# LiangZhaoPKUImperial/LinearSFM

Measured on AMD Instinct MI355X. Metric: hierarchical linear map-joining solve wall-clock, NC3500-like stereo (all transforms + joins), lower is better.
Workload: dtype f64

## Files before the change

### linearsfm_amd/csrc/lsfm_chol.hip

```cpp
#include <algorithm>
#include <climits>
#include <cmath>
#include <cstdlib>
#include <numeric>

#include "lsfm_device.hpp"
#include "lsfm_symbolic.hpp"
#include "lsfm_chol.hpp"

namespace lsfm {

#define FX_ONE 0x1p61
#define FX_INV 0x1p-61
__device__ __forceinline__ long long fx_from(double v) { return __double2ll_rn(fmin(fmax(v, -2.0), 2.0) * FX_ONE); }
__device__ __forceinline__ double fx_to(long long a) { return (double)a * FX_INV; }
__device__ __forceinline__ void fx_atomic_sub(double* slot, double t)
{
	__hip_atomic_fetch_add(reinterpret_cast<unsigned long long*>(slot), (unsigned long long)fx_from(-t), __ATOMIC_RELAXED, __HIP_MEMORY_SCOPE_AGENT);
}
__device__ __forceinline__ int scale_exp(double d)
{
	if (!(d > 0) || !(d < 1e300)) return 0;
	return (__builtin_amdgcn_frexp_exp(d) + 1) >> 1;
}
// ... 810 lines not shown
	__shared__ int spos[HB * HB];
	__shared__ int sCol[CHOL_GS];
	const int g = blockIdx.x, c0 = grp_c0[g], s = grp_s[g], nr = grp_nr[g];
	if (nr == 0 || of.skip(c0)) return;
	const int tid = threadIdx.x, nt = blockDim.x, lane = tid & 63, wave = __builtin_amdgcn_readfirstlane(tid >> 6);
	const int n6 = 6 * s, n6r = (n6 + 3) & ~3;
	const int xs = ((6 * smax + 3) & ~3) + 1;
	double* const XA = Ms;
	double* const XBs = Ms + 6 * HB * xs;
	const int nch = (nr + HB - 1) / HB, npairs = nch * (nch + 1) / 2;
	for (int t = tid; t < s; t += nt) sCol[t] = colptr[c0 + t];
	__syncthreads();
	const int rows0 = sCol[s - 1] + 1;
	for (int p = blockIdx.y; p < npairs; p += gridDim.y)
	{
		int ca = (int)((sqrtf(8.0f * p + 1.0f) - 1.0f) * 0.5f);
		while (ca * (ca + 1) / 2 > p) ca--;
		while ((ca + 1) * (ca + 2) / 2 <= p) ca++;
		const int cb = p - ca * (ca + 1) / 2;
		const bool two = ca != cb;
		if (tid < HB * HB)
		{
			const int a = tid / HB, b = tid - a * HB;
			const int ia = ca * HB + a, ib = cb * HB + b;
			int pos = -1;
			if (ia < nr && ib < nr && ia >= ib)
			{
				const int ra = rowidx[rows0 + ia], rb = rowidx[rows0 + ib];
				const int cbk = colptr[rb], nbk = colptr[rb + 1] - cbk;
				pos = cbk + (ia - ib);
				if (!(ia - ib < nbk && rowidx[pos] == ra)) pos = find_row(rowidx, cbk, cbk + nbk, ra);
			}
			spos[tid] = pos;
		}
		const int np2 = (two ? 2 : 1) * HB * s * 18;
		for (int base = 0; base < np2; base += nt * SN_LD)
		{
			double2 v[SN_LD];
#pragma unroll
			for (int i = 0; i < SN_LD; i++)
			{
				const int q = base + i * nt + tid;
				v[i] = make_double2(0.0, 0.0);
				if (q < np2)
				{
					const int blk = q / 18, il = blk / s, t = blk - il * s;
					const int row = (il < HB ? ca * HB + il : cb * HB + (il - HB));
					if (row < nr) v[i] = *reinterpret_cast<const double2*>(Lg + (size_t)(sCol[t] + (s - t) + row) * 36 + 2 * (q - blk * 18));
				}
			}
#pragma unroll
			for (int i = 0; i < SN_LD; i++)
			{
				const int q = base + i * nt + tid;
				if (q < np2)
				{
					const int blk = q / 18, w = 2 * (q - blk * 18), il = blk / s, t = blk - il * s;
					double* d = &Ms[(6 * il + w / 6) * xs + 6 * t + w % 6];
					d[0] = v[i].x; d[1] = v[i].y;
				}
			}
		}
		if (n6r > n6)
			for (int q = tid; q < (two ? 2 : 1) * 6 * HB * (n6r - n6); q += nt) Ms[(q / (n6r - n6)) * xs + n6 + q % (n6r - n6)] = 0.0;
		__syncthreads();
		const double* XB = two ? XBs : XA;
		sn_v4d acc[TPW];
#pragma unroll
		for (int i = 0; i < TPW; i++)
		{
			acc[i] = (sn_v4d){ 0.0, 0.0, 0.0, 0.0 };
			const int q = wave + (SN_THREADS / 64) * i;
			if (q < NTL * NTL)
			{
				const int ti = q / NTL, tj = q - ti * NTL;
				const double* pa = &XA[(16 * ti + (lane & 15)) * xs + (lane >> 4)];
				const double* pb = &XB[(16 * tj + (lane & 15)) * xs + (lane >> 4)];
				for (int ks = 0; ks < n6r; ks += 4) acc[i] = __builtin_amdgcn_mfma_f64_16x16x4f64(pa[ks], pb[ks], acc[i], 0, 0, 0);
			}
		}
		__syncthreads();
		double* sT = Ms;
#pragma unroll
		for (int i = 0; i < TPW; i++)
		{
			const int q = wave + (SN_THREADS / 64) * i;
			if (q < NTL * NTL)
			{
				const int ti = q / NTL, tj = q - ti * NTL;
#pragma unroll
				for (int e = 0; e < 4; e++) sT[(16 * ti + (lane >> 4) + 4 * e) * TS + 16 * tj + (lane & 15)] = acc[i][e];
			}
		}
		__syncthreads();
		for (int idx = tid; idx < HB * HB * 36; idx += nt)
		{
			const int pp = idx / 36, q = idx - pp * 36, ps = spos[pp];
			if (ps >= 0) fx_atomic_sub(L + (size_t)ps * 36 + q, sT[(6 * (pp / HB) + q / 6) * TS + 6 * (pp % HB) + q % 6]);
		}
		__syncthreads();
	}
}
static size_t sn_syrk_lds(int smax)
{
	const size_t xs = ((6 * (size_t)smax + 3) & ~(size_t)3) + 1;
	return std::max((size_t)(6 * SN_RB) * xs, (size_t)(6 * SN_RB / 2) * (6 * SN_RB / 2 + 1)) * sizeof(double);
}
static size_t sn_panel_lds(int smax)
{
	const size_t LD = 6 * (size_t)smax, xs = ((LD + 3) & ~(size_t)3) + 1;
	return std::max((LD + 6 * SN_RB + 1) * xs, (size_t)(6 * SN_RB / 2) * (6 * SN_RB / 2 + 1)) * sizeof(double);
}
__global__ void k_sn_merge(const int* __restrict__ grp_c0, const int* __restrict__ grp_s, const int* __restrict__ colptr, const double* __restrict__ Lg,
                           double* __restrict__ L)
{
	const int g = blockIdx.x, c0 = grp_c0[g], s = grp_s[g];
	const size_t b0 = (size_t)colptr[c0] * 36, b1 = (size_t)colptr[c0 + s] * 36;
	for (size_t q = b0 + threadIdx.x; q < b1; q += blockDim.x) L[q] = Lg[q];
}


template <class FT> struct SnPair;
template <> struct SnPair<double> { typedef double2 T; };
template <> struct SnPair<float> { typedef float2 T; };
template <class FT>
__device__ __forceinline__ void sn_load_diag(int s, int c0, const int* __restrict__ colptr, const FT* __restrict__ L, double* Ls, int* sSrc,
                                             int* sDst, int* sCol)
{
	const int tid = threadIdx.x, nt = blockDim.x, nb = s * (s + 1) / 2;
	for (int t = tid; t < s; t += nt) sCol[t] = colptr[c0 + t];
	__syncthreads();
	for (int e = tid; e < nb; e += nt)
	{
		int t = 0;
		while (sn_idx(s, s - 1, t) < e) t++;
		const int u = t + (e - sn_idx(s, t, t));
		sSrc[e] = (sCol[t] + (u - t)) * 36;
		sDst[e] = 6 * u * SN_XS + 6 * t;
	}
	__syncthreads();
	const int nd2 = nb * 18;
	for (int base = 0; base < nd2; base += nt * SN_LD)
	{
		typename SnPair<FT>::T v[SN_LD];
#pragma unroll
		for (int i = 0; i < SN_LD; i++)
		{
			const int q = base + i * nt + tid;
			if (q < nd2) { const int e = q / 18; v[i] = *reinterpret_cast<const typename SnPair<FT>::T*>(L + (size_t)sSrc[e] + 2 * (q - e * 18)); }
		}
#pragma unroll
		for (int i = 0; i < SN_LD; i++)
		{
			const int q = base + i * nt + tid;
			if (q < nd2) { const int e = q / 18, w = 2 * (q - e * 18); double* d = &Ls[sDst[e] + (w / 6) * SN_XS + w % 6]; d[0] = (double)v[i].x; d[1] = (double)v[i].y; }
		}
	}
	__syncthreads();
}

template <class FT>
__global__ void __launch_bounds__(SN_THREADS) k_sn_fwd(const int* __restrict__ grp_c0, const int* __restrict__ grp_s, const int* __restrict__ grp_nr,
                                                        const int* __restrict__ colptr, const int* __restrict__ rowidx, const FT* __restrict__ L,
                                                        const FT* __restrict__ Dinv, double* __restrict__ v, double* __restrict__ w, OwnFilter of)
{
	__shared__ double Ls[6 * CHOL_GS * SN_XS];
	__shared__ double sDi[CHOL_GS * 36];
	__shared__ double sA[6], sY[6 * CHOL_GS];
	__shared__ int sSrc[CHOL_GS * (CHOL_GS + 1) / 2], sDst[CHOL_GS * (CHOL_GS + 1) / 2], sCol[CHOL_GS];
	const int g = blockIdx.x, c0 = grp_c0[g], s = grp_s[g], nr = grp_nr[g];
	if (of.skip(c0)) return;
	const int tid = threadIdx.x, n6 = 6 * s;
	for (int q = tid; q < s * 36; q += SN_THREADS) sDi[q] = (double)Dinv[(size_t)c0 * 36 + q];
	double acc = tid < n6 ? v[(size_t)c0 * 6 + tid] : 0.0;
	sn_load_diag(s, c0, colptr, L, Ls, sSrc, sDst, sCol);
	for (int t = 0; t < s; t++)
	{
		const int k0 = 6 * t;
		if (tid >= k0 && tid < k0 + 6) sA[tid - k0] = acc;
		__syncthreads();
		if (tid >= k0 && tid < k0 + 6)
		{
			const int c = tid - k0;
			double y = 0.0;
			for (int k = 0; k <= c; k++) y = fma(sDi[t * 36 + c * 6 + k], sA[k], y);
			sY[tid] = y;
		}
		__syncthreads();
		if (tid >= k0 + 6 && tid < n6)
		{
			const double* lr = &Ls[tid * SN_XS + k0];
#pragma unroll
			for (int k = 0; k < 6; k++) acc = fma(-lr[k], sY[k0 + k], acc);
		}
	}
	if (tid < n6) w[(size_t)c0 * 6 + tid] = sY[tid];
	const int rows0 = colptr[c0 + s - 1] + 1;
	const int sub = tid & 3;
	for (int i = tid >> 2; i < nr; i += SN_THREADS / 4)
	{
		double o[6] = { 0, 0, 0, 0, 0, 0 };
		for (int t = sub; t < s; t += 4)
		{
			const FT* blk = L + ((size_t)sCol[t] + (s - t) + i) * 36;
			double b[36];
			ld<36>(b, blk);
#pragma unroll
			for (int r = 0; r < 6; r++)
#pragma unroll
				for (int k = 0; k < 6; k++) o[r] = fma(b[r * 6 + k], sY[6 * t + k], o[r]);
		}
#pragma unroll
		for (int r = 0; r < 6; r++)
		{
			o[r] += __shfl_xor(o[r], 1, LSFM_WAVE);
			o[r] += __shfl_xor(o[r], 2, LSFM_WAVE);
		}
		if (sub == 0)
		{
			double* dst = v + (size_t)rowidx[rows0 + i] * 6;
#pragma unroll
			for (int r = 0; r < 6; r++) atomic_add_f64(dst + r, -o[r]);
		}
	}
}

template <class FT>
__global__ void __launch_bounds__(SN_THREADS) k_sn_bwd(const int* __restrict__ grp_c0, const int* __restrict__ grp_s, const int* __restrict__ grp_nr,
                                                        const int* __restrict__ colptr, const int* __restrict__ rowidx, const FT* __restrict__ L,
                                                        const FT* __restrict__ Dinv, double* __restrict__ v, const double* __restrict__ w, OwnFilter of)
{
	__shared__ double Ls[6 * CHOL_GS * SN_XS];
	__shared__ double sDi[CHOL_GS * 36];
	__shared__ double sA[6], sZ[6 * CHOL_GS], sX[6 * CHOL_GS];
	__shared__ int sSrc[CHOL_GS * (CHOL_GS + 1) / 2], sDst[CHOL_GS * (CHOL_GS + 1) / 2], sCol[CHOL_GS];
	const int g = blockIdx.x, c0 = grp_c0[g], s = grp_s[g], nr = grp_nr[g];
	if (of.skip(c0)) return;
	const int tid = threadIdx.x, n6 = 6 * s;
	for (int q = tid; q < s * 36; q += SN_THREADS) sDi[q] = (double)Dinv[(size_t)c0 * 36 + q];
	if (tid < n6) sZ[tid] = w[(size_t)c0 * 6 + tid];
	sn_load_diag(s, c0, colptr, L, Ls, sSrc, sDst, sCol);
	const int rows0 = colptr[c0 + s - 1] + 1;
	const int sub = tid & 3;
	for (int i = tid >> 2; i < nr; i += SN_THREADS / 4)
	{
		const double* xr = v + (size_t)rowidx[rows0 + i] * 6;
		double x6[6];
		ld<6>(x6, xr);
		for (int t = sub; t < s; t += 4)
		{
			const FT* blk = L + ((size_t)sCol[t] + (s - t) + i) * 36;
			double b[36];
			ld<36>(b, blk);
#pragma unroll
			for (int c = 0; c < 6; c++)
			{
				double o = 0.0;
#pragma unroll
				for (int r = 0; r < 6; r++) o = fma(b[r * 6 + c], x6[r], o);
				lds_add_f64(&sZ[6 * t + c], -o);
			}
		}
	}
	__syncthreads();
	double acc = tid < n6 ? sZ[tid] : 0.0;
	for (int t = s - 1; t >= 0; t--)
	{
		const int k0 = 6 * t;
		if (tid >= k0 && tid < k0 + 6) sA[tid - k0] = acc;
		__syncthreads();
		if (tid >= k0 && tid < k0 + 6)
		{
			const int c = tid - k0;
			double x = 0.0;
			for (int k = c; k < 6; k++) x = fma(sDi[t * 36 + k * 6 + c], sA[k], x);
			sX[tid] = x;
		}
		__syncthreads();
		if (tid < k0)
		{
#pragma unroll
			for (int k = 0; k < 6; k++) acc = fma(-Ls[(k0 + k) * SN_XS + tid], sX[k0 + k], acc);
		}
	}
	if (tid < n6) v[(size_t)c0 * 6 + tid] = sX[tid];
}

__global__ void k_to_float(size_t n, const double* __restrict__ a, float* __restrict__ b)
{
	size_t i = (size_t)blockIdx.x * blockDim.x + threadIdx.x;
	if (i < n) b[i] = (float)a[i];
}

__global__ void k_perm_in(int M, const int* __restrict__ perm, const double* __restrict__ r, const unsigned char* __restrict__ fixed,
                          const double* __restrict__ dscale, double* __restrict__ v, int zero_from)
{
	size_t i = (size_t)blockIdx.x * blockDim.x + threadIdx.x;
	if (i >= (size_t)M * 6) return;
	const size_t src = (size_t)perm[i / 6] * 6 + i % 6;
	v[i] = ((fixed && fixed[src]) || (long)(i / 6) >= (long)zero_from) ? 0.0 : r[src] * dscale[i];
}
__global__ void k_perm_out_dot(int M, const int* __restrict__ pinv, const double* __restrict__ v, const double* __restrict__ r,
                               const unsigned char* __restrict__ fixed, const double* __restrict__ dscale, const int* __restrict__ pose_seg,
                               double* __restrict__ z, double* dot, int dot_stride, const int* __restrict__ col_owner, int rank)
{
	int row = blockIdx.x * blockDim.x + threadIdx.x;
	const bool ok = row < M;
	double acc = 0;
	int sg = 0;
	if (ok)
	{
		sg = pose_seg[row];
		const double* src = v + (size_t)pinv[row] * 6;
		const double* sc = dscale + (size_t)pinv[row] * 6;
		for (int i = 0; i < 6; i++)
		{
			double zz = src[i] * sc[i];
			if (fixed && fixed[(size_t)row * 6 + i]) zz = 0.0;
			if (col_owner) { const int ow = col_owner[pinv[row]]; if (!(ow == rank || (ow < 0 && rank == 0))) zz = 0.0; }
			z[(size_t)row * 6 + i] = zz;
			acc = fma(zz, r[(size_t)row * 6 + i], acc);
		}
	}
	if (dot) wave_scatter_add<1>(dot + (size_t)sg * dot_stride, &acc, ok);
}
__global__ void k_rz_dot(int M, const double* __restrict__ z, const double* __restrict__ r, const int* __restrict__ pose_seg, double* dot, int dot_stride)
{
	int row = blockIdx.x * blockDim.x + threadIdx.x;
	const bool ok = row < M;
	double acc = 0;
	int sg = 0;
	if (ok)
	{
		sg = pose_seg[row];
		for (int i = 0; i < 6; i++) acc = fma(z[(size_t)row * 6 + i], r[(size_t)row * 6 + i], acc);
	}
	wave_scatter_add<1>(dot + (size_t)sg * dot_stride, &acc, ok);
}

void chol_fetch(lsfm_context* ctx, const SchurSystem& sy, const int* d_origin, CholHostIn& in)
{
	const int M = sy.M, nnzb = sy.nnzb;
	in.keys.resize(nnzb);
	in.origin.resize(M);
	if (d_origin) LSFM_CHECK_HIP(hipMemcpyAsync(in.origin.data(), d_origin, (size_t)M * sizeof(int), hipMemcpyDeviceToHost, ctx->stream));
	else std::iota(in.origin.begin(), in.origin.end(), 0);
	d2h(ctx, in.keys.data(), sy.upper_keys, (size_t)nnzb * sizeof(unsigned long long));
}

void chol_alloc_values(lsfm_context* ctx, CholDev& ch)
{
	Arena& sc = ctx->scratch;
	ch.L = sc.alloc<double>((size_t)ch.nnzL * 36); ch.Dinv = sc.alloc<double>((size_t)ch.M * 36);
	ch.wv = sc.alloc<double>((size_t)ch.M * 6);
	ch.diag0 = sc.alloc<double>((size_t)ch.M * 6);
	ch.dscale = sc.alloc<double>((size_t)ch.M * 6);
	ch.Lg = ch.ngroups ? sc.alloc<double>((size_t)ch.nnzL * 36) : nullptr;
	dev_zero(ctx, ch.L, (size_t)ch.nnzL * 36 * sizeof(double));
	static const bool digest = getenv("LSFM_FACTOR_DIGEST") != nullptr;
	if (digest && ch.Lg) dev_zero(ctx, ch.Lg, (size_t)ch.nnzL * 36 * sizeof(double));
	ch.d_err = sc.alloc<int>(1);
	dev_zero(ctx, ch.d_err, sizeof(int));
}

static size_t chol_task_lds(const CholDev& ch) { return (size_t)ch.task0_maxsize * CHOL_TASK_LDS_PER_COL + 8; }
void chol_upload_index(lsfm_context* ctx, const CholSymbolic& sym, CholDev& ch)
{
	Arena& sc = ctx->scratch;
	ch.M = sym.M; ch.nnzL = sym.nnzL; ch.nlevels = sym.nlevels; ch.tail_begin = sym.tail_begin;
	ch.level_ptr = sym.level_ptr;
	if (!sym.tlevel_ptr.empty())
	{
		ch.ntask0 = sym.tlevel_ptr[1]; ch.ncol0 = sym.tlevel_col0[1];
		ch.task0_maxsize = sym.tlevel_maxsize[0]; ch.task0_lds = sym.tlevel_small_lds[0]; ch.task0_outer = sym.tlevel_outer[0];
		if (sym.tlevel_nsmall[0] != ch.ntask0 || chol_task_lds(ch) > CHOL_SOLVE_LDS)
			LSFM_FAIL(LSFM_ERR_INTERNAL, "a leaf task of the factorisation does not fit LDS (" + std::to_string(sym.tlevel_nsmall[0]) + " of " + std::to_string(ch.ntask0) +
			                                 " fit, " + std::to_string(ch.task0_maxsize) + " columns at most)");
	}
	ch.ngroups = sym.ngroups; ch.glevel_ptr = sym.glevel_ptr; ch.glevel_maxnr = sym.glevel_maxnr; ch.glevel_maxs = sym.glevel_maxs;
	ch.work_total = sym.work_total; ch.work_shared = sym.work_shared;
	ch.first_shared = sym.first_shared; ch.shared_blk0 = sym.colptr[sym.first_shared]; ch.glevel_owned = sym.glevel_owned; ch.glevel_shared = sym.glevel_shared;
	const struct { int** dst; const std::vector<int>* v; } parts[] = {
		{ &ch.grp_c0, &sym.grp_c0 }, { &ch.grp_s, &sym.grp_s }, { &ch.grp_nr, &sym.grp_nr }, { &ch.col_nin, &sym.col_nin }, { &ch.col_task, &sym.col_task },
		{ &ch.col_lpos, &sym.col_lpos }, { &ch.task_cols, &sym.task_cols }, { &ch.task_ptr, &sym.task_ptr }, { &ch.colptr, &sym.colptr },
		{ &ch.rowidx, &sym.rowidx }, { &ch.perm, &sym.perm }, { &ch.pinv, &sym.pinv }, { &ch.order, &sym.order }, { &ch.col_owner, &sym.col_owner } };
	size_t total = 0;
	for (const auto& pt : parts) total += pt.v->size();
	static thread_local std::vector<int> blob;
	blob.resize(total);
	int* d_blob = sc.alloc<int>(total);
	size_t off = 0;
	for (const auto& pt : parts)
	{
		if (!pt.v->empty()) memcpy(blob.data() + off, pt.v->data(), pt.v->size() * sizeof(int));
		*pt.dst = pt.v->empty() ? nullptr : d_blob + off;
		off += pt.v->size();
	}
	h2d(ctx, d_blob, blob.data(), total * sizeof(int));
	ch.blob = d_blob; ch.blob_ints = total;
}
void chol_upload_symbolic(lsfm_context* ctx, const CholSymbolic& sym, CholDev& ch)
{
	chol_upload_index(ctx, sym, ch);
	chol_alloc_values(ctx, ch);
	if (getenv("LSFM_DEBUG") && sym.ngroups > 50)
	{
		int hist[CHOL_GS + 1] = { 0 };
		for (int g = 0; g < sym.ngroups; g++) hist[sym.grp_s[g]]++;
		fprintf(stderr, "[lsfm] groups %d, group levels %d, sizes:", sym.ngroups, (int)sym.glevel_ptr.size() - 1);
		for (int q = 1; q <= CHOL_GS; q++) fprintf(stderr, " %d", hist[q]);
		fprintf(stderr, " | groups per level:");
		for (size_t l = 0; l + 1 < sym.glevel_ptr.size(); l++) fprintf(stderr, " %d", sym.glevel_ptr[l + 1] - sym.glevel_ptr[l]);
		fprintf(stderr, "\n");
	}
}
void chol_analyse(lsfm_context* ctx, const SchurSystem& sy, const CholHostIn& in, CholDev& ch)
{
	static thread_local CholSymbolic sym;
	chol_symbolic(in.keys.data(), sy.nnzb, in.origin.data(), sy.M, sym, ctx->comm ? ctx->comm->block_maps : 0);
	chol_upload_symbolic(ctx, sym, ch);
}

bool chol_distributed(const lsfm_context* ctx, const CholDev& ch)
{
	return ctx->comm && ctx->comm->world > 1 && ch.col_owner && ch.first_shared < ch.M;
}
static void comm_sum(lsfm_context* ctx, void* p, size_t count, int dtype)
{
	if (!count) return;
	Comm& cm = *ctx->comm;
	const size_t mk = cm.off;
	void* b = cm.alloc_bytes(count * 8);
	LSFM_CHECK_HIP(hipMemcpyAsync(b, p, count * 8, hipMemcpyDeviceToDevice, ctx->stream));
	cm.allreduce(ctx->stream, b, count, dtype);
	LSFM_CHECK_HIP(hipMemcpyAsync(p, b, count * 8, hipMemcpyDeviceToDevice, ctx->stream));
	cm.off = mk;
}
void comm_sum_host(lsfm_context* ctx, long long* h, int n)
{
	hipStream_t s = ctx->stream;
	Comm& cm = *ctx->comm;
	const size_t mk = cm.off;
	long long* d = cm.alloc<long long>(n);
	LSFM_CHECK_HIP(hipMemcpyAsync(d, h, n * sizeof(long long), hipMemcpyHostToDevice, s));
	LSFM_CHECK_HIP(hipStreamSynchronize(s));
	cm.allreduce(s, d, n, LSFM_DTYPE_I64);
	LSFM_CHECK_HIP(hipMemcpyAsync(h, d, n * sizeof(long long), hipMemcpyDeviceToHost, s));
	LSFM_CHECK_HIP(hipStreamSynchronize(s));
	cm.off = mk;
}

void chol_scatter(lsfm_context* ctx, const SchurSystem& sy, const unsigned char* fixed, CholDev& ch)
{
	const bool dist = chol_distributed(ctx, ch);
	if (sy.nnzb)
		hipLaunchKernelGGL(k_chol_scatter, dim3((sy.nnzb + 127) / 128), dim3(128), 0, ctx->stream, sy.nnzb, sy.upper_keys, sy.S, sy.rowptr, ch.pinv, ch.colptr, ch.rowidx,
		                   fixed, ch.col_task, ch.ntask0, ch.L, ch.diag0, ch.dscale, dist ? ch.col_owner : (const int*)nullptr, dist ? ctx->comm->rank : 0);
}
void chol_factor(lsfm_context* ctx, const SchurSystem& sy, const unsigned char* fixed, CholDev& ch, double* fwd_v)
{
	hipStream_t s = ctx->stream;
	const bool dist = chol_distributed(ctx, ch);
	const OwnFilter mine{ dist ? ch.col_owner : nullptr, dist ? ctx->comm->rank : 0 }, shared{ dist ? ch.col_owner : nullptr, -1 };
	ch.sn_fused_levels = ch.sn_split_levels = 0;
	if (ch.ntask0)
	{
		hipLaunchKernelGGL(k_chol_factor_level, dim3(ch.ntask0), dim3(128), (size_t)ch.task0_lds, s, ch.task_ptr, ch.task_cols, ch.col_nin, ch.colptr, ch.rowidx,
		                   ch.L, ch.Dinv, ch.d_err, mine);
		if (ch.task0_outer > 0)
		{
			const dim3 grid(ch.ncol0, std::min((ch.task0_outer + CHOL_OUT_THREADS - 1) / CHOL_OUT_THREADS, 64));
			hipLaunchKernelGGL(k_chol_update_outer, grid, dim3(CHOL_OUT_THREADS), 0, s, ch.task_cols, ch.col_nin, ch.colptr, ch.rowidx, ch.L, mine);
		}
		if (fwd_v)
			hipLaunchKernelGGL(k_chol_fwd_tasks<double>, dim3(ch.ntask0), dim3(128), chol_task_lds(ch), s, ch.task_ptr, ch.task_cols, ch.col_task, ch.col_lpos, 0, ch.colptr,
			                   ch.rowidx, (const double*)ch.L, (const double*)ch.Dinv, fwd_v, mine);
	}
	static const int fuse_max = getenv("LSFM_SN_FUSE_MAX") ? atoi(getenv("LSFM_SN_FUSE_MAX")) : 96;
	static const double piv_floor = getenv("LSFM_PIVOT_FLOOR") ? atof(getenv("LSFM_PIVOT_FLOOR")) : 1e-13;
	static const bool lds_set = []() {
		(void)hipFuncSetAttribute(reinterpret_cast<const void*>(&k_sn_panel<true>), hipFuncAttributeMaxDynamicSharedMemorySize, (int)sn_panel_lds(CHOL_GS));
		(void)hipFuncSetAttribute(reinterpret_cast<const void*>(&k_sn_panel<false>), hipFuncAttributeMaxDynamicSharedMemorySize, (int)sn_panel_lds(CHOL_GS));
		(void)hipFuncSetAttribute(reinterpret_cast<const void*>(&k_sn_syrk), hipFuncAttributeMaxDynamicSharedMemorySize, (int)sn_syrk_lds(CHOL_GS));
		return true;
	}();
	(void)lds_set;
	for (int phase = 0; phase < (dist ? 2 : 1); phase++)
	{
		const OwnFilter of = phase == 0 ? mine : shared;
		if (phase == 1)
		{
			comm_sum(ctx, ch.L + (size_t)ch.shared_blk0 * 36, ((size_t)ch.nnzL - ch.shared_blk0) * 36, LSFM_DTYPE_I64);
			if (fwd_v) comm_sum(ctx, fwd_v + (size_t)ch.first_shared * 6, ((size_t)ch.M - ch.first_shared) * 6, LSFM_DTYPE_F64);
		}
		for (size_t l = 0; l + 1 < ch.glevel_ptr.size(); l++)
		{
			const int g0 = ch.glevel_ptr[l], ng = ch.glevel_ptr[l + 1] - g0, mnr = ch.glevel_maxnr[l];
			if (!ng) continue;
			if (dist && !(phase == 0 ? ch.glevel_owned[l] : ch.glevel_shared[l])) continue;
			const int smax = l < ch.glevel_maxs.size() ? ch.glevel_maxs[l] : CHOL_GS;
			if (mnr <= fuse_max)
			{
				const int nch = (mnr + SN_RB / 2 - 1) / (SN_RB / 2);
				hipLaunchKernelGGL(k_sn_panel<true>, dim3(ng, std::max(1, nch * (nch + 1) / 2)), dim3(SN_PT), sn_panel_lds(smax), s, ch.grp_c0 + g0, ch.grp_s + g0, ch.grp_nr + g0,
				                   ch.colptr, ch.L, ch.Lg, ch.Dinv, ch.d_err, ch.rowidx, fwd_v, ch.wv, smax, ch.diag0, piv_floor, ctx->d_run ? &ctx->d_run->floored : nullptr, of);
				ch.sn_fused_levels++;
				continue;
			}
			hipLaunchKernelGGL(k_sn_panel<false>, dim3(ng, std::max(1, (mnr + SN_RB - 1) / SN_RB)), dim3(SN_PT), sn_panel_lds(smax), s, ch.grp_c0 + g0, ch.grp_s + g0, ch.grp_nr + g0,
			                   ch.colptr, ch.L, ch.Lg, ch.Dinv, ch.d_err, ch.rowidx, fwd_v, ch.wv, smax, ch.diag0, piv_floor, ctx->d_run ? &ctx->d_run->floored : nullptr, of);
			const long nch = (mnr + SN_RB / 2 - 1) / (SN_RB / 2), npair = nch * (nch + 1) / 2;
			hipLaunchKernelGGL(k_sn_syrk, dim3(ng, (unsigned)std::max<long>(1, std::min<long>(npair, 8192))), dim3(SN_THREADS), sn_syrk_lds(smax), s,
			                   ch.grp_c0 + g0, ch.grp_s + g0, ch.grp_nr + g0, ch.colptr, ch.rowidx, ch.L, ch.Lg, smax, of);
			ch.sn_split_levels++;
		}
	}
}

void chol_merge_groups(lsfm_context* ctx, const CholDev& ch)
{
	if (ch.ngroups)
		hipLaunchKernelGGL(k_sn_merge, dim3(ch.ngroups), dim3(256), 0, ctx->stream, ch.grp_c0, ch.grp_s, ch.colptr, ch.Lg, ch.L);
}
void chol_round_to_float(lsfm_context* ctx, CholDev& ch)
{
	hipStream_t s = ctx->stream;
	Arena& sc = ctx->scratch;
	const size_t nl = (size_t)ch.nnzL * 36, nd = (size_t)ch.M * 36;
	ch.Lf = sc.alloc<float>(nl); ch.Dinvf = sc.alloc<float>(nd);
	hipLaunchKernelGGL(k_to_float, dim3((unsigned)((nl + 255) / 256)), dim3(256), 0, s, nl, ch.L, ch.Lf);
	if (ch.Lg)
	{
		ch.Lgf = sc.alloc<float>(nl);
		hipLaunchKernelGGL(k_to_float, dim3((unsigned)((nl + 255) / 256)), dim3(256), 0, s, nl, ch.Lg, ch.Lgf);
	}
	hipLaunchKernelGGL(k_to_float, dim3((unsigned)((nd + 255) / 256)), dim3(256), 0, s, nd, ch.Dinv, ch.Dinvf);
}

void chol_perm_in(lsfm_context* ctx, const CholDev& ch, const double* r, const unsigned char* fixed, double* v)
{
	const size_t ns = (size_t)ch.M * 6;
	const int zero_from = (chol_distributed(ctx, ch) && ctx->comm->rank != 0) ? ch.first_shared : INT_MAX;
	hipLaunchKernelGGL(k_perm_in, dim3((unsigned)((ns + 255) / 256)), dim3(256), 0, ctx->stream, ch.M, ch.perm, r, fixed, ch.dscale, v, zero_from);
}

void chol_apply(lsfm_context* ctx, const CholDev& ch, const double* r, double* v, double* z, const unsigned char* fixed, const int* pose_seg,
                double* dot, int dot_stride, bool fwd_done)
{
	hipStream_t s = ctx->stream;
	if (!fwd_done) chol_perm_in(ctx, ch, r, fixed, v);
	const int ngl = (int)ch.glevel_ptr.size() - 1;
	const bool dist = chol_distributed(ctx, ch);
	const OwnFilter mine{ dist ? ch.col_owner : nullptr, dist ? ctx->comm->rank : 0 }, shared{ dist ? ch.col_owner : nullptr, -1 };
	auto sweep = [&](auto tag, const auto* Lx, const auto* Gx, const auto* Dx) {
		typedef decltype(tag) FT;
		if (!fwd_done)
		{
			if (ch.ntask0) hipLaunchKernelGGL(k_chol_fwd_tasks<FT>, dim3(ch.ntask0), dim3(128), chol_task_lds(ch), s, ch.task_ptr, ch.task_cols, ch.col_task, ch.col_lpos, 0, ch.colptr, ch.rowidx, Lx, Dx, v, mine);
			for (int phase = 0; phase < (dist ? 2 : 1); phase++)
			{
				if (phase == 1) comm_sum(ctx, v + (size_t)ch.first_shared * 6, ((size_t)ch.M - ch.first_shared) * 6, LSFM_DTYPE_F64);
				for (int l = 0; l < ngl; l++)
				{
					const int g0 = ch.glevel_ptr[l], ng = ch.glevel_ptr[l + 1] - g0;
					if (!ng || (dist && !(phase == 0 ? ch.glevel_owned[l] : ch.glevel_shared[l]))) continue;
					hipLaunchKernelGGL(k_sn_fwd<FT>, dim3(ng), dim3(SN_THREADS), 0, s, ch.grp_c0 + g0, ch.grp_s + g0, ch.grp_nr + g0, ch.colptr, ch.rowidx, Gx, Dx, v, ch.wv, phase == 0 ? mine : shared);
				}
			}
		}
		for (int phase = (dist ? 1 : 0); phase >= 0; phase--)
			for (int l = ngl - 1; l >= 0; l--)
			{
				const int g0 = ch.glevel_ptr[l], ng = ch.glevel_ptr[l + 1] - g0;
				if (!ng || (dist && !(phase == 0 ? ch.glevel_owned[l] : ch.glevel_shared[l]))) continue;
				hipLaunchKernelGGL(k_sn_bwd<FT>, dim3(ng), dim3(SN_THREADS), 0, s, ch.grp_c0 + g0, ch.grp_s + g0, ch.grp_nr + g0, ch.colptr, ch.rowidx, Gx, Dx, v, ch.wv, (dist && phase == 1) ? shared : mine);
			}
		if (ch.ntask0) hipLaunchKernelGGL(k_chol_bwd_tasks<FT>, dim3(ch.ntask0), dim3(128), chol_task_lds(ch), s, ch.task_ptr, ch.task_cols, ch.col_task, ch.col_lpos, 0, ch.colptr, ch.rowidx, Lx, Dx, v, mine);
	};
	if (ch.Lf) sweep(float(), (const float*)ch.Lf, (const float*)ch.Lgf, (const float*)ch.Dinvf);
	else sweep(double(), (const double*)ch.L, (const double*)ch.Lg, (const double*)ch.Dinv);
	if (dist)
	{
		hipLaunchKernelGGL(k_perm_out_dot, dim3((ch.M + 127) / 128), dim3(128), 0, s, ch.M, ch.pinv, v, r, fixed, ch.dscale, pose_seg, z, (double*)nullptr, dot_stride,
		                   ch.col_owner, ctx->comm->rank);
		ctx->comm->allreduce(s, z, (size_t)ch.M * 6, LSFM_DTYPE_F64);
		hipLaunchKernelGGL(k_rz_dot, dim3((ch.M + 127) / 128), dim3(128), 0, s, ch.M, z, r, pose_seg, dot, dot_stride);
	}
	else
		hipLaunchKernelGGL(k_perm_out_dot, dim3((ch.M + 127) / 128), dim3(128), 0, s, ch.M, ch.pinv, v, r, fixed, ch.dscale, pose_seg, z, dot, dot_stride, (const int*)nullptr, 0);
}

int chol_selftest(lsfm_context* ctx, int m, const int* rowptr, const int* colidx, const double* val, const int* origin, const unsigned char* fixed,
                  const int* pose_seg, int nseg, const double* r, int nrhs, int mode, double* z, double* dot, int* perm, int* colptr, int* rowidx,
                  double* L, double* Dinv, double* dscale, int cap_blocks, int* info)
{
	const int nnzb = rowptr[m];
	const size_t ns = (size_t)m * 6;
	CholHostIn hin;
	hin.keys.resize(nnzb);
	hin.origin.resize(m);
	for (int p = 0; p < m; p++)
	{
		hin.origin[p] = origin ? origin[p] : p;
		for (int k = rowptr[p]; k < rowptr[p + 1]; k++) hin.keys[k] = ((unsigned long long)(unsigned)p << 32) | (unsigned)colidx[k];
	}
	{
		CholSymbolic sym;
		chol_symbolic(hin.keys.data(), nnzb, hin.origin.data(), m, sym);
		info[0] = sym.nnzL;
		if (cap_blocks < sym.nnzL) LSFM_FAIL(LSFM_ERR_ARG, "rowidx / L too small for the factor (" + std::to_string(sym.nnzL) + " blocks)");
		ctx->ensure_arenas((size_t)sym.nnzL * 36 * 32 + (size_t)nnzb * 320 + ns * 8 * (16 + 2 * (size_t)nrhs) + ((size_t)64 << 20));
	}
	ctx->scratch.reset();
	Arena& sc = ctx->scratch;
	SchurSystem sy;
	sy.M = m; sy.nnzb = nnzb;
	unsigned long long* dk = sc.alloc<unsigned long long>(nnzb + 1);
	sy.S = sc.alloc<double>((size_t)nnzb * 36);
	sy.rowptr = sc.alloc<int>(m + 1);
	h2d(ctx, dk, hin.keys.data(), (size_t)nnzb * sizeof(unsigned long long));
	h2d(ctx, sy.S, val, (size_t)nnzb * 36 * sizeof(double));
	h2d(ctx, sy.rowptr, rowptr, (size_t)(m + 1) * sizeof(int));
	sy.upper_keys = dk;
	unsigned char* dfx = nullptr;
	if (fixed) { dfx = sc.alloc<unsigned char>(ns); h2d(ctx, dfx, fixed, ns); }
	int* dseg = sc.alloc<int>(m);
	h2d(ctx, dseg, pose_seg, (size_t)m * sizeof(int));
	double* dr = sc.alloc<double>(ns * nrhs);
	double* dz = sc.alloc<double>(ns * nrhs);
	double* ddot = sc.alloc<double>((size_t)nseg * nrhs);
	double* dv = sc.alloc<double>(ns);
	h2d(ctx, dr, r, ns * nrhs * sizeof(double));
	dev_zero(ctx, ddot, (size_t)nseg * nrhs * sizeof(double));
	CholDev ch;
	chol_analyse(ctx, sy, hin, ch);
	RunStatsDev* d_run = sc.alloc<RunStatsDev>(1);
	dev_zero(ctx, d_run, sizeof(RunStatsDev));
	const bool fused = (mode & 1) != 0;
	{
		struct Swap { lsfm_context* c; RunStatsDev* keep; ~Swap() { c->d_run = keep; } } swap{ ctx, ctx->d_run };
		ctx->d_run = d_run;
		chol_scatter(ctx, sy, dfx, ch);
		if (fused) chol_perm_in(ctx, ch, dr, dfx, dv);
		chol_factor(ctx, sy, dfx, ch, fused ? dv : nullptr);
	}
	if (mode & 2) chol_round_to_float(ctx, ch);
	for (int k = 0; k < nrhs; k++) chol_apply(ctx, ch, dr + ns * k, dv, dz + ns * k, dfx, dseg, ddot + (size_t)nseg * k, 1, fused && k == 0);
	chol_merge_groups(ctx, ch);
	LSFM_CHECK_HIP(hipGetLastError());
	RunStatsDev rs;
	d2h(ctx, &rs, d_run, sizeof rs);
	const int chol_err = d2h_int(ctx, ch.d_err);
	const int ngl = (int)ch.glevel_ptr.size() - 1;
	info[1] = ch.ntask0; info[2] = ch.ncol0; info[3] = ch.task0_outer; info[4] = ch.ngroups; info[5] = std::max(ngl, 0);
	info[6] = ch.sn_fused_levels; info[7] = ch.sn_split_levels;
	info[8] = ch.glevel_maxnr.empty() ? 0 : *std::max_element(ch.glevel_maxnr.begin(), ch.glevel_maxnr.end());
	info[9] = chol_err; info[10] = rs.floored;
	d2h(ctx, z, dz, ns * nrhs * sizeof(double));
	d2h(ctx, dot, ddot, (size_t)nseg * nrhs * sizeof(double));
	if (perm) d2h(ctx, perm, ch.perm, (size_t)m * sizeof(int));
	if (colptr) d2h(ctx, colptr, ch.colptr, (size_t)(m + 1) * sizeof(int));
	if (rowidx) d2h(ctx, rowidx, ch.rowidx, (size_t)ch.nnzL * sizeof(int));
	if (L) d2h(ctx, L, ch.L, (size_t)ch.nnzL * 36 * sizeof(double));
	if (Dinv) d2h(ctx, Dinv, ch.Dinv, (size_t)m * 36 * sizeof(double));
	if (dscale) d2h(ctx, dscale, ch.dscale, ns * sizeof(double));
	if (chol_err) LSFM_FAIL(LSFM_ERR_NOT_SPD, "the matrix is not positive definite (block column " + std::to_string(chol_err - 1) + " of the factor)");
	return LSFM_OK;
}

}
```

### linearsfm_amd/csrc/lsfm_chol.hpp

```cpp
#pragma once
#include <vector>

#include "lsfm_internal.hpp"
#include "lsfm_solve.hpp"

namespace lsfm {

struct CholDev {
	int M = 0, nnzL = 0, nlevels = 0, tail_begin = 0;
	int* colptr = nullptr;
	int* rowidx = nullptr;
	int* perm = nullptr;
	int* pinv = nullptr;
	int* order = nullptr;
	std::vector<int> level_ptr;
	int* task_cols = nullptr;
	int* task_ptr = nullptr;
	int* col_task = nullptr;
	int* col_lpos = nullptr;
	int* col_nin = nullptr;
	int ntask0 = 0, ncol0 = 0;
	int task0_maxsize = 0;
	int task0_lds = 0;
	int task0_outer = 0;
	int ngroups = 0;
	int *grp_c0 = nullptr, *grp_s = nullptr, *grp_nr = nullptr;
	std::vector<int> glevel_ptr;
	std::vector<int> glevel_maxnr;
	std::vector<int> glevel_maxs;
	int sn_fused_levels = 0, sn_split_levels = 0;
	int* col_owner = nullptr;
	int first_shared = 0, shared_blk0 = 0;
	double work_total = 0, work_shared = 0;
	std::vector<char> glevel_owned, glevel_shared;
	int* blob = nullptr;
	size_t blob_ints = 0;
	float *Lf = nullptr, *Dinvf = nullptr;
	double* wv = nullptr;
	double* Lg = nullptr;
	float* Lgf = nullptr;
	double* L = nullptr;
	double* Dinv = nullptr;
	double* diag0 = nullptr;
	double* dscale = nullptr;
	int* d_err = nullptr;
};

struct OwnFilter {
	const int* col_owner = nullptr;
	int want = 0;
	__device__ __forceinline__ bool skip(int col) const { return col_owner && col_owner[col] != want; }
};
__device__ __forceinline__ int find_row(const int* __restrict__ rowidx, int lo, int hi, int target)
{
	while (lo < hi) { int mid = (lo + hi) >> 1; if (rowidx[mid] < target) lo = mid + 1; else hi = mid; }
	return lo;
}


struct CholSymbolic;
struct CholHostIn {
	std::vector<unsigned long long> keys;
	std::vector<int> origin;
};

void chol_fetch(lsfm_context* ctx, const SchurSystem& sy, const int* d_origin, CholHostIn& in);
void chol_analyse(lsfm_context* ctx, const SchurSystem& sy, const CholHostIn& in, CholDev& ch);
void chol_upload_index(lsfm_context* ctx, const CholSymbolic& sym, CholDev& ch);
void chol_upload_symbolic(lsfm_context* ctx, const CholSymbolic& sym, CholDev& ch);
void chol_alloc_values(lsfm_context* ctx, CholDev& ch);
void chol_scatter(lsfm_context* ctx, const SchurSystem& sy, const unsigned char* fixed, CholDev& ch);
void chol_factor(lsfm_context* ctx, const SchurSystem& sy, const unsigned char* fixed, CholDev& ch, double* fwd_v = nullptr);
void chol_merge_groups(lsfm_context* ctx, const CholDev& ch);
void chol_round_to_float(lsfm_context* ctx, CholDev& ch);
void chol_perm_in(lsfm_context* ctx, const CholDev& ch, const double* r, const unsigned char* fixed, double* v);
void chol_apply(lsfm_context* ctx, const CholDev& ch, const double* r, double* v, double* z, const unsigned char* fixed, const int* pose_seg, double* dot, int dot_stride, bool fwd_done = false);
bool chol_distributed(const lsfm_context* ctx, const CholDev& ch);
void comm_sum_host(lsfm_context* ctx, long long* h, int n);

}
```

### linearsfm_amd/csrc/lsfm_internal.hpp

```cpp
#pragma once
#include <hip/hip_runtime.h>

#include <cstdint>
#include <cstdio>
#include <condition_variable>
#include <cstring>
#include <exception>
#include <functional>
#include <memory>
#include <mutex>
#include <thread>
#include <string>
#include <vector>

#include "../../include/lsfm.h"

namespace lsfm {

struct Error { int code; std::string msg; };
struct DevBatch;
struct IndexHold;
struct SolvePlan;
struct PreLevel;
struct EarlyPattern;

#define LSFM_CHECK_HIP(expr)                                                                                   \
	do {                                                                                                        \
		hipError_t e__ = (expr);                                                                                \
		if (e__ != hipSuccess)                                                                                  \
			throw ::lsfm::Error{ LSFM_ERR_HIP, std::string(#expr) + ": " + hipGetErrorString(e__) + " at " + __FILE__ + ":" + std::to_string(__LINE__) }; \
	} while (0)
#define LSFM_FAIL(code, m) throw ::lsfm::Error{ (code), std::string(m) + " at " + __FILE__ + ":" + std::to_string(__LINE__) }

struct Arena {
	char* base = nullptr;
	size_t cap = 0, off = 0, high = 0;
	void init(size_t bytes);
	void destroy();
	void* alloc_bytes(size_t bytes);
	template <class T> T* alloc(size_t n) { return static_cast<T*>(alloc_bytes(n * sizeof(T))); }
	void reset() { off = 0; }
	size_t mark() const { return off; }
	void release(size_t m) { off = m; }
};

struct ZeroSpan {
	Arena& ar;
	size_t from;
	explicit ZeroSpan(Arena& a) : ar(a), from((a.off + 255) & ~size_t(255)) {}
	void zero(hipStream_t s) const;
};

struct DevBatch {
	int B = 0, M = 0, NF = 0, NU = 0, NW = 0;
	std::vector<int> pose_off, feat_off, u_off, w_off;
	std::vector<int> Ref, FRef, ScaP, Fix, Sign, FScaP, FFix;
	int *d_pose_off = nullptr, *d_feat_off = nullptr;
	double* pose = nullptr;
	int* pose_id = nullptr;
	int* pose_map = nullptr;
	int* pose_origin = nullptr;
	double* feat = nullptr;
	int* feat_id = nullptr;
	int* feat_map = nullptr;
	double* U = nullptr; int *Ui = nullptr, *Uj = nullptr;
	double* W = nullptr; int *photo = nullptr, *feature = nullptr;
	int* fptr = nullptr;
	double* V = nullptr;
	const double* W_alias = nullptr;
	const int* d_alias = nullptr;
	const unsigned long long* s_keys = nullptr;
	int s_nnzb = 0;
};

struct PcgOptions { double rel_tol = 1e-12; int max_steps = 50; bool mixed = false; int spmv_variant = 0; };

struct LevelIndex {
	int NU = -1, NW = -1, NF = -1;
	const int *KU = nullptr, *KW = nullptr;
	const int *match = nullptr, *R = nullptr;
	std::shared_ptr<IndexHold> own;
};
const int* level_index_keep(lsfm_context* ctx, LevelIndex& li, const int* src, size_t n);

struct LevelPlan {
	bool valid = false;
	LevelIndex idx;
	std::vector<int> tr_cnt;
	std::vector<int> tr_sign;
	std::vector<int> join_rb;
	std::vector<int> join_uo, join_wo;
	std::shared_ptr<SolvePlan> solve;
};

struct RunStatsDev {
	int chol_err;
	int not_converged;
	int tr_err;
	int plan_stale;
	int undone;
	int floored;
	double max_rel_residual;
	unsigned long long s_digest, factor_digest;
	int refactor_mismatch;
	int s_rebuild_mismatch;
	unsigned long long k2;
};

struct Comm {
	int rank = 0, world = 1;
	lsfm_allreduce_fn fn = nullptr;
	void* user = nullptr;
	char* buf = nullptr;
	size_t cap = 0, off = 256;
	int block_maps = 0;
	enum { HDR_BYTES = 256, KIND_DATA = 0, KIND_FINAL = 1 };
	bool broken = false;
	void restart() { off = HDR_BYTES; }
	void* alloc_bytes(size_t bytes)
	{
		const size_t a = (off + 255) & ~size_t(255);
		if (a + bytes > cap)
			throw Error{ LSFM_ERR_ARG, "the buffer handed to lsfm_tree_set_comm is too small (" + std::to_string(a + bytes) + " bytes needed, " + std::to_string(cap) + " given)" };
		off = a + bytes;
		return buf + a;
	}
	template <class T> T* alloc(size_t n) { return static_cast<T*>(alloc_bytes(n * sizeof(T))); }
	void allreduce(hipStream_t s, void* p, size_t count, int dtype, int kind = KIND_DATA);
	void call(hipStream_t s, size_t offset, size_t count, int dtype)
	{
		const int rc = fn(user, offset, count, dtype, (void*)s);
		if (rc) { broken = true; throw Error{ LSFM_ERR_INTERNAL, "the caller's all-reduce failed with code " + std::to_string(rc) }; }
	}
	bool follow(hipStream_t s);
};

struct HostWorker {
	std::thread th;
	std::mutex m;
	std::condition_variable cv;
	std::function<void()> job;
	std::exception_ptr err;
	bool busy = false, quit = false;
	~HostWorker()
	{
		{ std::lock_guard<std::mutex> l(m); quit = true; }
		cv.notify_all();
		if (th.joinable()) th.join();
	}
	void run(std::function<void()> f)
	{
		std::unique_lock<std::mutex> l(m);
		cv.wait(l, [&] { return !busy; });
		job = std::move(f); busy = true; err = nullptr;
		if (!th.joinable())
			th = std::thread([this] {
				std::unique_lock<std::mutex> lk(m);
				for (;;)
				{
					cv.wait(lk, [&] { return quit || (busy && job); });
					if (quit) return;
					std::function<void()> j = std::move(job);
					job = nullptr;
					lk.unlock();
					std::exception_ptr e;
					try { j(); } catch (...) { e = std::current_exception(); }
					lk.lock();
					err = e; busy = false;
					cv.notify_all();
				}
			});
		cv.notify_all();
	}
	void wait()
	{
		std::unique_lock<std::mutex> l(m);
		cv.wait(l, [&] { return !busy; });
		if (err) { std::exception_ptr e = err; err = nullptr; std::rethrow_exception(e); }
	}
};

}

namespace lsfm {
struct Roctx {
	int (*push)(const char*) = nullptr;
	int (*pop)() = nullptr;
	void (*mark)(const char*) = nullptr;
	Roctx();
};
Roctx& roctx();
struct Range {
	bool on;
	explicit Range(const char* name) : on(roctx().push != nullptr) { if (on) roctx().push(name); }
	~Range() { if (on) roctx().pop(); }
	Range(const Range&) = delete;
	Range& operator=(const Range&) = delete;
};
}

namespace lsfm {
enum Ord {
	evA,
	evB,
	evC_pairs,
	evC_runs,
	evY,
	evP,
	evU,
	evG,
	evT,
	evK9_fork,
	evK9_done,
	evR_fork,
	evR_done,
	ORD_COUNT
};
}

struct lsfm_context {
	int device = 0;
	hipStream_t stream = nullptr;
	lsfm::Arena arena[3];
	lsfm::Arena scratch;
	int cur = 0;
	size_t arena_bytes = 0, arena_req = 0;
	lsfm::PcgOptions pcg;
	int covcols_panel = 0;
	int small_max = 5;
	std::string last_error;
	int* h_pinned = nullptr;
	char* h_stage = nullptr;
	char* d_stage = nullptr;
	size_t stage_size = 0, stage_off = 0;
	hipEvent_t ev_half[2] = { nullptr, nullptr };
	unsigned long long generation = 0;
	hipStream_t stream2 = nullptr;
	hipEvent_t ord[lsfm::ORD_COUNT] = {};
	void quiesce_side_streams();
	std::shared_ptr<lsfm::EarlyPattern> early;
	hipStream_t stream3 = nullptr;
	lsfm::Arena sarena[2];
	std::shared_ptr<lsfm::PreLevel> pre;
	lsfm::LevelPlan pre_plan;
	int pre_plan_level = -1;
	std::unique_ptr<lsfm::HostWorker> worker;
	void drop_prepared() { pre.reset(); pre_plan = lsfm::LevelPlan(); pre_plan_level = -1; }
	double dbg_gap_ms = 0.0;
	std::vector<std::pair<const char*, double>> timeline;
	bool timeline_on = false;
	void mark(const char* what);
	bool in_tree_run = false;
	lsfm_stats* stats = nullptr;
	lsfm::LevelPlan* plan = nullptr;
	bool warm() const { return plan && plan->valid; }
	lsfm::RunStatsDev* d_run = nullptr;
	lsfm::Comm* comm = nullptr;
	std::vector<hipEvent_t> ev_pool;
	size_t ev_next = 0;
	struct Timed { hipEvent_t a, b; double* sink; };
	std::vector<Timed> timed;
	hipEvent_t pool_event();
	void defer_time(hipEvent_t a, hipEvent_t b, double* sink) { timed.push_back(Timed{ a, b, sink }); }
	void flush_times();
	void ensure_arenas(size_t bytes_each, bool start_small = false);
	bool grow_arenas();
	bool arena_small = false;
	size_t arena_bound = 0;
};

namespace lsfm {

struct OnStream {
	lsfm_context* c; hipStream_t& s; Arena* a;
	OnStream(lsfm_context* ctx, hipStream_t& other, Arena* arena = nullptr) : c(ctx), s(other), a(arena) { std::swap(c->stream, s); if (a) std::swap(c->scratch, *a); }
	~OnStream() { if (a) std::swap(c->scratch, *a); std::swap(c->stream, s); }
	OnStream(const OnStream&) = delete;
	OnStream& operator=(const OnStream&) = delete;
};
inline void wait_for(lsfm_context* ctx, hipStream_t s, Ord e) { LSFM_CHECK_HIP(hipStreamWaitEvent(s, ctx->ord[e], 0)); }
struct Fork {
	lsfm_context* c; hipStream_t main; OnStream on;
	Fork(lsfm_context* ctx, hipStream_t& side, Arena* arena = nullptr) : c(ctx), main(ctx->stream), on(ctx, side, arena) {}
	Fork(lsfm_context* ctx, hipStream_t& side, Ord start, bool record = true, Arena* arena = nullptr) : Fork(ctx, side, arena)
	{
		if (record) LSFM_CHECK_HIP(hipEventRecord(c->ord[start], main));
		wait_for(c, c->stream, start);
	}
	void done(Ord e) { LSFM_CHECK_HIP(hipEventRecord(c->ord[e], c->stream)); }
	void join(Ord e) { done(e); wait_for(c, main, e); }
};

void dev_exclusive_scan(lsfm_context* ctx, const int* in, int* out, size_t n);
void dev_sort_pairs_u64(lsfm_context* ctx, unsigned long long* keys, int* vals, size_t n, int end_bit, int begin_bit = 0);
void dev_sort_keys_u64(lsfm_context* ctx, const unsigned long long* keys, unsigned long long* sorted, size_t n, int begin_bit, int end_bit);
int d2h_int(lsfm_context* ctx, const int* dptr);
void d2h_ints(lsfm_context* ctx, const int* dptr, int* h, size_t n);
void h2d(lsfm_context* ctx, void* d, const void* h, size_t bytes);
struct HostPiece { const void* p; size_t bytes; };
void h2d_gather(lsfm_context* ctx, void* d, const std::vector<HostPiece>& pieces);
struct CopyBatch {
	lsfm_context* ctx;
	struct Item { void* dst; const void* src; size_t bytes; bool host; };
	std::vector<Item> items;
	explicit CopyBatch(lsfm_context* c) : ctx(c) {}
	void h2d(void* d, const void* h, size_t bytes) { if (bytes) items.push_back(Item{ d, h, bytes, true }); }
	void d2d(void* d, const void* s, size_t bytes) { if (bytes) items.push_back(Item{ d, s, bytes, false }); }
	void flush();
};
void d2h(lsfm_context* ctx, void* h, const void* d, size_t bytes);
void dev_zero(lsfm_context* ctx, void* d, size_t bytes);
void fill_async(hipStream_t s, void* d, int byte, size_t bytes);

void batch_upload(lsfm_context* ctx, Arena& ar, const lsfm_map* maps, int N, bool mono, DevBatch& out);
void batch_download_map(lsfm_context* ctx, const DevBatch& b, int k, bool mono, lsfm_map* out);
template <class T> inline T* host_alloc(size_t n) { return static_cast<T*>(malloc((n ? n : 1) * sizeof(T))); }
struct CopyBatch;
void batch_set_offsets(lsfm_context* ctx, Arena& ar, DevBatch& b, CopyBatch* cb = nullptr);
void batch_fill_maps(lsfm_context* ctx, DevBatch& b);
struct PackHeader {
	int magic, version, mono, m, n, nU, nW, Ref, FRef, ScaP, Fix, Sign, FScaP, FFix, pad0, pad1;
	unsigned long long total;
	unsigned long long off[12];
	unsigned long long pad[11];
};
static_assert(sizeof(PackHeader) == 256, "the header is the first 256 bytes of a pack");
#define LSFM_PACK_MAGIC 0x4d46534c
size_t pack_layout(PackHeader& h);
void batch_pack_map(lsfm_context* ctx, const DevBatch& b, int k, bool mono, void* dst, size_t cap);
void batch_slice_counts(lsfm_context* ctx, const DevBatch& b, int nslices, std::vector<int>& nf, std::vector<int>& nw);
void batch_pack_slice(lsfm_context* ctx, const DevBatch& b, bool mono, int nslices, int slice, int nf, int nw, void* dst, size_t cap);
void batch_unpack_maps(lsfm_context* ctx, Arena& ar, const void* const* packed, const PackHeader* hdr, int N, bool mono, DevBatch& out);
unsigned long long batch_structure_digest(lsfm_context* ctx, const DevBatch& b);

inline bool map_in_frame(const DevBatch& X, int b, int tref, int tscap, bool mono) { return X.Ref[b] == tref && (!mono || X.ScaP[b] == tscap); }
int level_targets(const DevBatch& X, bool mono, std::vector<int>& tref, std::vector<int>& tscap, std::vector<int>& tfix);
struct TrRedirect {
	const int* wbase = nullptr;
	const int* newf = nullptr;
	double* W = nullptr;
	int *photo = nullptr, *feature = nullptr, *srcf = nullptr;
};
using TrHook = std::function<TrRedirect(DevBatch& mid, const int* hub)>;
void transform_batch(lsfm_context* ctx, Arena& ar, const DevBatch& in, const std::vector<int>& target_ref,
                     const std::vector<int>& target_scap, const std::vector<int>& target_fix, bool mono, DevBatch& out,
                     bool alias_passthrough = false, const TrHook* hook = nullptr);

struct JoinWork;
struct SolveIO {
	int M = 0, NF = 0, NU = 0, NW = 0, nseg = 0;
	const int* d_pose_seg = nullptr;
	const int* d_feat_seg = nullptr;
	const unsigned char* d_seg_active = nullptr;
	const double* U = nullptr; const int *Ui = nullptr, *Uj = nullptr;
	const double* W = nullptr; const int *photo = nullptr, *fptr = nullptr;
	const double* V = nullptr;
	const double* ea = nullptr;
	const double* eb = nullptr;
	const double* x0 = nullptr;
	const unsigned char* d_fixed = nullptr;
	const int* d_pose_origin = nullptr;
	double* x_pose = nullptr;
	double* x_feat = nullptr;
	std::vector<int> seg_rows;
	const int *d_pose_off = nullptr, *d_feat_off = nullptr, *d_u_off = nullptr;
	const struct RhsFused* rhs = nullptr;
	const struct PatternSeed* seed = nullptr;
	bool index_arrays_at_evA = false;
	int step_hint = 0;
	bool caller_syncs = false;
};
struct SolveOutcome {
	int not_converged = 0;
	int steps_used = 0;
	const unsigned long long* keys = nullptr;
	int nnzb = 0;
	hipEvent_t end = nullptr;
};
int small_level_strips(const lsfm_context* ctx, int most_rows);
inline int most_rows(const std::vector<int>& seg_rows) { int most = 0; for (int r : seg_rows) most = r > most ? r : most; return most; }
inline int small_level_strips(const lsfm_context* ctx, const std::vector<int>& seg_rows) { return small_level_strips(ctx, most_rows(seg_rows)); }
void small_level_offsets(lsfm_context* ctx, const DevBatch& out, SolveIO& io);
void small_solve_launch(lsfm_context* ctx, const SolveIO& io, int strips, int* status, double* max_rel);
struct HostSystem;
int small_selftest(lsfm_context* ctx, int G, const int* pose_off, const int* feat_off, const int* u_off, const unsigned char* active, const HostSystem& h,
                   const unsigned char* fixed, int strips, double* x_pose, double* x_feat, int* status, double* max_rel);
SolveOutcome solve_batch(lsfm_context* ctx, const SolveIO& io);
SolveOutcome join_batch_stereo(lsfm_context* ctx, Arena& ar, const DevBatch& in, DevBatch& out, double* eP_out, double* eF_out, int step_hint = 0);
SolveOutcome join_batch_mono(lsfm_context* ctx, Arena& ar, const DevBatch& in, DevBatch& out, double* eP_out, double* eF_out, int step_hint = 0);
int gn_polish(lsfm_context* ctx, const lsfm_map* maps, int N, bool mono, lsfm_map* x, int iters, int kind, double c, double* obj, double* gnorm,
              int* halvings, double* chi2, double* weight, bool feat = false);
int map_feature_chi2(lsfm_context* ctx, const lsfm_map* maps, int N, bool mono, const lsfm_map* x, double* fchi2, double* pose_chi2);
int gn_polish_features(lsfm_context* ctx, const lsfm_map* maps, int N, bool mono, lsfm_map* x, int iters, int kind, double c, double* obj, double* gnorm,
                       int* halvings, double* fchi2, double* fweight);
int map_chi2(lsfm_context* ctx, const lsfm_map* maps, int N, bool mono, const lsfm_map* x, double* chi2, int* dof);
int gn_linearise(lsfm_context* ctx, const lsfm_map* maps, int N, bool mono, const lsfm_map* x, const double* weight, lsfm_map* out, double* obj,
                 double* b, double* times, int* counts);
int map_covariance(lsfm_context* ctx, const lsfm_map* map, bool mono, double* pose_cov, double* feat_cov, double* pair_cov, int cap_blocks, int* nnzb,
                   double* times);
int map_covariance_columns(lsfm_context* ctx, const lsfm_map* map, bool mono, const int* poses, int k, double* pose_cols, double* feat_cols, double* joint,
                           int* steps, double* last_corr, double* times);
int inverse_v(lsfm_context* ctx, double* V, int n);
int solve_features(lsfm_context* ctx, const double* W, const double* IV, const double* eb, const double* dpa, double* dpb, int m, int n, const int* mapCor,
                   const int* photo);
bool no_timing_events();
#define LSFM_REC_T(e, s) do { if (!lsfm::no_timing_events()) LSFM_CHECK_HIP(hipEventRecord(e, s)); } while (0)
unsigned timing_event_flags();
unsigned order_event_flags();
void prefetch_next_level(lsfm_context* ctx, const DevBatch& Y, const std::vector<int>& target_ref, int next_level, int step_hint,
                         const unsigned long long* level_keys, int level_nnzb);
int spmv_external(lsfm_context* ctx, int m, const int* rowptr, const int* colidx, const double* val, const double* x, double* y, int reps,
                  double* avg_ms, double* bytes);
int chol_selftest(lsfm_context* ctx, int m, const int* rowptr, const int* colidx, const double* val, const int* origin, const unsigned char* fixed,
                  const int* pose_seg, int nseg, const double* r, int nrhs, int mode, double* z, double* dot, int* perm, int* colptr, int* rowidx,
                  double* L, double* Dinv, double* dscale, int cap_blocks, int* info);

int wstream_bench(lsfm_context* ctx, long long nblocks, int mode, int reps, double* avg_ms);
int prims_selftest(lsfm_context* ctx, int cases, unsigned seed);
}
```

### linearsfm_amd/csrc/lsfm_level.hip

```cpp
#include <algorithm>
#include <chrono>
#include <cmath>
#include <cstdlib>

#include "lsfm_device.hpp"
#include "lsfm_symbolic.hpp"
#include "lsfm_pcg.hpp"

namespace lsfm {

struct SolvePlan {
	SchurSystem sy;
	CholDev ch;
	int its = 1;
	bool mixed = false;
	double rel_tol = 0;
	bool small = false;
	char* mem = nullptr;
	~SolvePlan() { if (mem) (void)hipFree(mem); }
};
static std::shared_ptr<SolvePlan> solve_plan_store(lsfm_context* ctx, const SchurSystem& sy, const CholDev& ch, int its)
{
	auto sp = std::make_shared<SolvePlan>();
	const size_t M = sy.M, nnzb = sy.nnzb, cap = (size_t)sy.mask + 1;
	if (getenv("LSFM_DEBUG") && sy.k9.ns && sy.k9_tiles > 0)
	{
		std::vector<int> h(sy.k9_tiles);
		d2h(ctx, h.data(), sy.k9.ns, sizeof(int) * h.size());
		int b16 = 0, b32 = 0, b48 = 0, b64 = 0, b96 = 0, more = 0;
		for (int v : h) { const int n = v < 0 ? -v : v; (n <= 16 ? b16 : n <= 32 ? b32 : n <= 48 ? b48 : n <= 64 ? b64 : n <= 96 ? b96 : more)++; }
		fprintf(stderr, "[lsfm] Schur tiles by poses: <=16 %d, <=32 %d, <=48 %d, <=64 %d, <=96 %d, more (or > 64 distinct: hash full) %d\n", b16, b32, b48, b64, b96, more);
	}
	struct Item { const void* src; size_t bytes; void** dst; };
	SolvePlan& P = *sp;
	P.sy = sy; P.ch = ch; P.its = its; P.mixed = ch.Lf != nullptr; P.rel_tol = ctx->pcg.rel_tol;
	P.sy.S = nullptr; P.sy.E = nullptr; P.sy.IV = nullptr;
	P.ch.L = nullptr; P.ch.Dinv = nullptr; P.ch.diag0 = nullptr; P.ch.dscale = nullptr; P.ch.Lg = nullptr; P.ch.Lgf = nullptr; P.ch.d_err = nullptr; P.ch.wv = nullptr; P.ch.Lf = nullptr; P.ch.Dinvf = nullptr;
	std::vector<Item> items = {
		{ sy.rowptr, (M + 1) * 4, (void**)&P.sy.rowptr }, { sy.colidx, (nnzb + 1) * 4, (void**)&P.sy.colidx },
		{ sy.upper_keys, nnzb * 8, (void**)&P.sy.upper_keys }, { sy.longrows, (M + 1) * 4, (void**)&P.sy.longrows },
		{ sy.d_nlong, 4, (void**)&P.sy.d_nlong }, { sy.tab, cap * 8, (void**)&P.sy.tab }, { sy.hval, cap * 4, (void**)&P.sy.hval },
		{ ch.blob, ch.blob_ints * 4, (void**)&P.ch.blob },
		{ sy.gent, sy.gent ? nnzb * 16 : 0, (void**)&P.sy.gent }, { sy.goth, sy.goth ? nnzb * 8 : 0, (void**)&P.sy.goth },
		{ sy.k9.ns, sy.k9.ns ? (size_t)sy.k9_tiles * 4 : 0, (void**)&P.sy.k9.ns }, { sy.k9.pose, sy.k9.pose ? (size_t)sy.k9_tiles * 64 * 4 : 0, (void**)&P.sy.k9.pose },
		{ sy.k9.eslot, sy.k9.eslot ? (size_t)sy.k9_NW : 0, (void**)&P.sy.k9.eslot },
		{ sy.k9.wlist, sy.k9.wlist ? (size_t)sy.k9_tiles * 3 * 4 : 0, (void**)&P.sy.k9.wlist }, { sy.k9.wcnt, sy.k9.wcnt ? (size_t)32 : (size_t)0, (void**)&P.sy.k9.wcnt },
	};
	size_t total = 0;
	for (const Item& it : items) total += (it.bytes + 255) & ~(size_t)255;
	LSFM_CHECK_HIP(hipMalloc((void**)&P.mem, total + 256));
	size_t off = 0;
	for (const Item& it : items)
	{
		if (it.bytes) LSFM_CHECK_HIP(hipMemcpyAsync(P.mem + off, it.src, it.bytes, hipMemcpyDeviceToDevice, ctx->stream));
		*it.dst = it.src ? P.mem + off : nullptr;
		off += (it.bytes + 255) & ~(size_t)255;
	}
	const ptrdiff_t shift = (char*)P.ch.blob - (char*)ch.blob;
	auto rebase = [&](int*& p) { if (p) p = (int*)((char*)p + shift); };
	rebase(P.ch.colptr); rebase(P.ch.rowidx); rebase(P.ch.perm); rebase(P.ch.pinv); rebase(P.ch.order); rebase(P.ch.task_cols);
	rebase(P.ch.task_ptr); rebase(P.ch.col_task); rebase(P.ch.col_lpos); rebase(P.ch.col_nin); rebase(P.ch.grp_c0); rebase(P.ch.grp_s);
	rebase(P.ch.grp_nr); rebase(P.ch.col_owner);
	LSFM_CHECK_HIP(hipStreamSynchronize(ctx->stream));
	return sp;
}

struct PreLevel {
	SchurSystem sy;
	CholSymbolic sym;
	CholHostIn hin;
	int M = 0;
	HostWorker* worker = nullptr;
	bool whole = false;
	int level = -1, its = 0;
	void wait()
	{
		HostWorker* w = worker;
		worker = nullptr;
		if (w) w->wait();
	}
	~PreLevel() { try { wait(); } catch (...) {} }
};
void prefetch_next_level(lsfm_context* ctx, const DevBatch& Y, const std::vector<int>& target_ref, int next_level, int step_hint,
                         const unsigned long long* level_keys, int level_nnzb)
{
	ctx->drop_prepared();
	if (!Y.M || Y.B < 2) return;
	int most_next = 0;
	for (int b = 0; b < Y.B; b += 2) most_next = std::max(most_next, Y.pose_off[std::min(b + 2, Y.B)] - Y.pose_off[b]);
	const bool next_small = small_level_strips(ctx, most_next) > 0;
	const bool whole = step_hint > 0 && !getenv("LSFM_CHECK_EARLY_PATTERN");
	if (next_small && !whole) return;
	ctx->mark("pre_start");
	auto pl = std::make_shared<PreLevel>();
	pl->M = Y.M;
	Arena& sa = ctx->sarena[next_level & 1];
	sa.reset();
	std::vector<int> counts;
	LevelIndex kept;
	bool ok = false;
	{
		Fork side(ctx, ctx->stream3, evY, false, &sa);
		if (ctx->timeline_on) { (void)hipEventSynchronize(ctx->ord[evY]); ctx->mark("pre_evY"); }
		int* d_tref = ctx->scratch.alloc<int>(Y.B);
		h2d(ctx, d_tref, target_ref.data(), sizeof(int) * (size_t)Y.B);
		ok = schur_pattern_prefetch(ctx, Y, d_tref, level_keys, level_nnzb, pl->sy, whole ? &counts : nullptr, !next_small, whole ? &kept : nullptr);
		if (ok)
		{
			if (!next_small) chol_fetch(ctx, pl->sy, Y.pose_origin, pl->hin);
			side.done(evP);
		}
	}
	ctx->mark("pre_pat");
	if (!ok) return;
	if (!next_small)
	{
		if (!ctx->worker) ctx->worker.reset(new HostWorker());
		PreLevel* raw = pl.get();
		ctx->worker->run([raw]() { chol_symbolic(raw->hin.keys.data(), raw->sy.nnzb, raw->hin.origin.data(), raw->sy.M, raw->sym); });
		pl->worker = ctx->worker.get();
		ctx->mark("pre_sym");
		pl->whole = whole; pl->level = next_level; pl->its = step_hint;
		ctx->pre = pl;
	}
	if (!whole) return;
	const int B = Y.B;
	ctx->pre_plan.tr_cnt.assign(counts.begin(), counts.begin() + 2 * (B + 1));
	ctx->pre_plan.join_rb.assign(counts.begin() + 2 * (B + 1), counts.end());
	ctx->pre_plan.solve.reset();
	ctx->pre_plan.idx = kept;
	ctx->pre_plan.valid = true;
	ctx->pre_plan_level = next_level;
	ctx->mark("pre_plan");
}
static std::shared_ptr<SolvePlan> pre_plan_complete(lsfm_context* ctx, PreLevel& pl)
{
	pl.wait();
	auto sp = std::make_shared<SolvePlan>();
	sp->sy = pl.sy;
	sp->its = pl.its; sp->mixed = ctx->pcg.mixed; sp->rel_tol = ctx->pcg.rel_tol;
	{
		Fork side(ctx, ctx->stream3, &ctx->sarena[pl.level & 1]);
		chol_upload_index(ctx, pl.sym, sp->ch);
		side.join(evP);
	}
	return sp;
}

__global__ void k_dbg_absstats(size_t n, const double* __restrict__ a, double* __restrict__ out)
{
	double s = 0.0, m = 0.0;
	for (size_t i = (size_t)blockIdx.x * blockDim.x + threadIdx.x; i < n; i += (size_t)gridDim.x * blockDim.x)
	{
		const double v = fabs(a[i]);
		s += v; if (v > m || !(v == v)) m = v == v ? v : 1e300;
	}
	atomic_add_f64(out, s);
	atomicMax(reinterpret_cast<unsigned long long*>(out + 1), (unsigned long long)__double_as_longlong(m));
}
__global__ void k_dbg_dinv(int M, const double* __restrict__ Dinv, const double* __restrict__ diag0, const int* __restrict__ colptr, int first_group_col)
{
	int j = blockIdx.x * blockDim.x + threadIdx.x;
	if (j >= M) return;
	double m = 0.0;
	for (int q = 0; q < 36; q++) m = fmax(m, fabs(Dinv[(size_t)j * 36 + q]));
	if (m > 1e3 || !(m == m))
		printf("[lsfm conv] column %d (%s, %d blocks): max |Dinv| %.3e, Dinv diag %.3e %.3e %.3e %.3e %.3e %.3e, diag0 %.3e %.3e %.3e %.3e %.3e %.3e\n", j,
		       j >= first_group_col ? "group" : "leaf", colptr[j + 1] - colptr[j], m, Dinv[(size_t)j * 36], Dinv[(size_t)j * 36 + 7], Dinv[(size_t)j * 36 + 14],
		       Dinv[(size_t)j * 36 + 21], Dinv[(size_t)j * 36 + 28], Dinv[(size_t)j * 36 + 35], diag0[j * 6], diag0[j * 6 + 1], diag0[j * 6 + 2], diag0[j * 6 + 3],
		       diag0[j * 6 + 4], diag0[j * 6 + 5]);
}
__global__ void k_digest(size_t n, const unsigned long long* __restrict__ a, unsigned long long* out)
{
	unsigned long long h = 0;
	for (size_t i = (size_t)blockIdx.x * blockDim.x + threadIdx.x; i < n; i += (size_t)gridDim.x * blockDim.x)
	{
		unsigned long long b = a[i];
		if (b == 0x8000000000000000ull) b = 0;
		b ^= b >> 31; b *= 0x9E3779B97F4A7C15ull * (2 * (unsigned long long)i + 1); b ^= b >> 29;
		h += b;
	}
	atomicAdd(out, h);
}
__global__ void k_digest_compare(const unsigned long long* d, int* mismatch)
{
	if (d[0] != d[1]) atomicAdd(mismatch, 1);
}
__global__ void k_chol_err_to_run(const int* err, RunStatsDev* run)
{
	if (*err && !run->chol_err) run->chol_err = *err;
}

struct LevelStructure {
	SchurSystem sy;
	CholDev ch;
	SolvePlan* sp = nullptr;
	double tw0 = 0, tw1 = 0;
};
static double wall_ms() { return std::chrono::duration<double, std::milli>(std::chrono::steady_clock::now().time_since_epoch()).count(); }
static LevelStructure level_structure(lsfm_context* ctx, const SolveIO& io, SolvePlan* sp, PreLevel* pre, bool pending, hipEvent_t eb)
{
	hipStream_t s = ctx->stream;
	LevelStructure ls;
	SchurSystem& sy = ls.sy;
	CholDev& ch = ls.ch;
	auto assemble = [&]() {
		build_schur_values(ctx, io, sy);
		LSFM_REC_T(eb, s); if (roctx().mark) roctx().mark("lsfm factor + refine: begin");
	};
	if (sp || pending)
	{
		sy = pending ? pre->sy : sp->sy;
		schur_vinv(ctx, io, sy);
		assemble();
		if (pending)
		{
			ctx->mark("k9_enq");
			ctx->plan->solve = pre_plan_complete(ctx, *pre);
			sp = ctx->plan->solve.get();
			ctx->mark("sym_wait");
		}
		ls.sp = sp;
		ch = sp->ch;
		chol_alloc_values(ctx, ch);
		return ls;
	}
	schur_vinv(ctx, io, sy);
	CholHostIn hin;
	bool have = false;
	if (pre && !(pre->M == io.M && !ctx->comm)) pre = nullptr;
	if (pre)
	{
		schur_pattern_early_drop(ctx);
		SchurSystem prepared = pre->sy;
		prepared.IV = sy.IV; prepared.LY = sy.LY; prepared.ymax = sy.ymax; prepared.uu = sy.uu;
		sy = prepared;
		have = true;
		wait_for(ctx, s, evP);
		if (getenv("LSFM_CHECK_EARLY_PATTERN")) schur_pattern_check(ctx, io, sy, "prefetched");
	}
	else if (ctx->early && !ctx->comm)
	{
		{
			Fork side(ctx, ctx->stream3, evC_runs, false);
			ctx->mark("sv_start");
			have = schur_pattern_early_finish(ctx, io, sy);
			ctx->mark("pat_fin");
			if (have)
			{
				if (getenv("LSFM_CHECK_EARLY_PATTERN")) schur_pattern_check(ctx, io, sy, "early");
				chol_fetch(ctx, sy, io.d_pose_origin, hin);
				ctx->mark("fetch");
				schur_pattern_early_extras(ctx, sy);
				side.join(evB);
			}
		}
	}
	else if (io.index_arrays_at_evA && !ctx->comm)
	{
		Fork side(ctx, ctx->stream2, evA, false);
		build_schur_pattern(ctx, io, sy);
		chol_fetch(ctx, sy, io.d_pose_origin, hin);
		side.join(evB);
		have = true;
	}
	if (!have)
	{
		build_schur_pattern(ctx, io, sy);
		chol_fetch(ctx, sy, io.d_pose_origin, hin);
	}
	assemble();
	ls.tw0 = wall_ms();
	ctx->mark("k9_enq");
	if (pre) { pre->wait(); chol_upload_symbolic(ctx, pre->sym, ch); }
	else chol_analyse(ctx, sy, hin, ch);
	ctx->mark("analyse");
	ls.tw1 = wall_ms();
	return ls;
}

static SolveOutcome solve_level_dense(lsfm_context* ctx, const SolveIO& io, int strips, bool warm, hipEvent_t eb, hipEvent_t ec, hipEvent_t ed)
{
	hipStream_t s = ctx->stream;
	LevelPlan* lp = ctx->plan;
	if (!warm) schur_pattern_early_drop(ctx);
	int* d_small = nullptr;
	auto enqueue = [&]() {
		d_small = ctx->scratch.alloc<int>(4);
		dev_zero(ctx, d_small, 4 * sizeof(int));
		hipEvent_t esm0 = nullptr, esm1 = nullptr;
		if (ctx->stats) { esm0 = ctx->pool_event(); esm1 = ctx->pool_event(); LSFM_REC_T(esm0, s); }
		small_solve_launch(ctx, io, strips, d_small, reinterpret_cast<double*>(d_small + 2));
		if (ctx->stats) { LSFM_REC_T(esm1, s); ctx->defer_time(esm0, esm1, &ctx->stats->t_small_ms); ctx->stats->small_levels++; }
	};
	if (!warm) enqueue();
	LSFM_REC_T(eb, s); if (warm && roctx().mark) roctx().mark("lsfm factor + refine: begin");
	if (warm) enqueue();
	LSFM_REC_T(ec, s);
	LSFM_REC_T(ed, s); if (roctx().mark) roctx().mark("lsfm solve: end");
	SolveOutcome oc;
	oc.end = ed;
	oc.steps_used = 1;
	if (ctx->stats) ctx->stats->pcg_iterations += 1;
	const bool deferred = ctx->in_tree_run && ctx->d_run && (warm || !lp || lp == &ctx->pre_plan);
	if (deferred) return oc;
	int hs[4];
	d2h_ints(ctx, d_small, hs, 4);
	if (hs[1]) LSFM_FAIL(LSFM_ERR_NOT_SPD, "Schur system is not positive definite (system " + std::to_string(hs[1] - 1) + " of the level)");
	double mr;
	memcpy(&mr, hs + 2, sizeof mr);
	if (ctx->stats) ctx->stats->max_rel_residual = std::max(ctx->stats->max_rel_residual, mr);
	if (lp && !lp->solve && hs[0] == 0)
	{
		auto small_plan = std::make_shared<SolvePlan>();
		small_plan->its = 1; small_plan->mixed = false; small_plan->rel_tol = ctx->pcg.rel_tol; small_plan->small = true;
		lp->solve = small_plan;
	}
	oc.not_converged = hs[0];
	return oc;
}

static void factor_digest_check(lsfm_context* ctx, const SolveIO& io, const SchurSystem& sy, CholDev& ch)
{
	static const bool digest = getenv("LSFM_FACTOR_DIGEST") != nullptr;
	if (!digest || !ctx->d_run) return;
	hipStream_t s = ctx->stream;
	Arena& sc = ctx->scratch;
	const int M = io.M;
	auto dg = [&](const double* a, size_t n, unsigned long long* out) {
		if (a && n) hipLaunchKernelGGL(k_digest, dim3(256), dim3(256), 0, s, n, reinterpret_cast<const unsigned long long*>(a), out);
	};
	dg(sy.S, (size_t)sy.nnzb * 36, &ctx->d_run->s_digest);
	if (!ctx->comm)
	{
		SchurSystem sy2 = sy;
		build_schur_values(ctx, io, sy2);
		unsigned long long* d = sc.alloc<unsigned long long>(2);
		dev_zero(ctx, d, 2 * sizeof(unsigned long long));
		dg(sy.S, (size_t)sy.nnzb * 36, d); dg(sy.E, (size_t)M * 6, d);
		dg(sy2.S, (size_t)sy.nnzb * 36, d + 1); dg(sy2.E, (size_t)M * 6, d + 1);
		hipLaunchKernelGGL(k_digest_compare, dim3(1), dim3(1), 0, s, d, &ctx->d_run->s_rebuild_mismatch);
	}
	auto factor_digest = [&](unsigned long long* out) {
		dg(ch.Dinv, (size_t)ch.M * 36, out);
		dg(ch.L, (size_t)ch.nnzL * 36, out);
		if (ch.Lg) dg(ch.Lg, (size_t)ch.nnzL * 36, out);
	};
	factor_digest(&ctx->d_run->factor_digest);
	if (!ctx->comm)
	{
		unsigned long long* d = sc.alloc<unsigned long long>(2);
		dev_zero(ctx, d, 2 * sizeof(unsigned long long));
		factor_digest(d);
		dev_zero(ctx, ch.L, (size_t)ch.nnzL * 36 * sizeof(double));
		if (ch.Lg) dev_zero(ctx, ch.Lg, (size_t)ch.nnzL * 36 * sizeof(double));
		chol_scatter(ctx, sy, io.d_fixed, ch);
		chol_factor(ctx, sy, io.d_fixed, ch, nullptr);
		factor_digest(d + 1);
		hipLaunchKernelGGL(k_digest_compare, dim3(1), dim3(1), 0, s, d, &ctx->d_run->refactor_mismatch);
	}
}

static void debug_conv(lsfm_context* ctx, const SolveIO& io, const SchurSystem& sy, const CholDev& ch, const PcgSeg* seg)
{
	hipStream_t s = ctx->stream;
	const int M = io.M;
	hipLaunchKernelGGL(k_pcg_debug, dim3((io.nseg + 127) / 128), dim3(128), 0, s, io.nseg, M, seg);
	if (!(M > 10000 && io.nseg == 1)) return;
	double* d = ctx->scratch.alloc<double>(12);
	dev_zero(ctx, d, 12 * sizeof(double));
	auto st = [&](const double* a, size_t n, int k) { if (a && n) hipLaunchKernelGGL(k_dbg_absstats, dim3(512), dim3(256), 0, s, n, a, d + 2 * k); };
	st(sy.S, (size_t)sy.nnzb * 36, 0); st(sy.E, (size_t)M * 6, 1); st(ch.L, (size_t)ch.nnzL * 36, 2); st(ch.Lg, (size_t)ch.nnzL * 36, 3);
	st(ch.Dinv, (size_t)ch.M * 36, 4); st(io.x_pose, (size_t)M * 6, 5);
	hipLaunchKernelGGL(k_dbg_dinv, dim3((ch.M + 255) / 256), dim3(256), 0, s, ch.M, ch.Dinv, ch.diag0, ch.colptr, 0);
	double h[12];
	d2h(ctx, h, d, sizeof h);
	fprintf(stderr, "[lsfm conv] root M=%d: |S| sum %.15e max %.6e  |E| sum %.15e  |L| sum %.12e max %.3e  |Lg| sum %.12e max %.3e  |Dinv| sum %.6e max %.3e  |x| sum %.12e max %.3e\n",
	        M, h[0], h[1], h[2], h[4], h[5], h[6], h[7], h[8], h[9], h[10], h[11]);
}

SolveOutcome solve_batch(lsfm_context* ctx, const SolveIO& io)
{
	hipStream_t s = ctx->stream;
	const int M = io.M;
	LevelPlan* lp = ctx->plan;
	const int strips = (io.d_pose_off && io.d_feat_off && io.d_u_off) ? small_level_strips(ctx, io.seg_rows) : 0;
	SolvePlan* sp = lp ? lp->solve.get() : nullptr;
	if (sp && sp->small != (strips > 0)) { lp->solve.reset(); sp = nullptr; }
	std::shared_ptr<PreLevel> pre = std::move(ctx->pre);
	const bool pending = !strips && !sp && pre && pre->whole && lp == &ctx->pre_plan;
	if (pre && !pending && (strips || sp || pre->whole || pre->M != M || ctx->comm)) pre.reset();
	const bool warm = sp != nullptr || pending;
	hipEvent_t ea = ctx->pool_event(), eb = ctx->pool_event(), ec = ctx->pool_event(), ed = ctx->pool_event();
	LSFM_REC_T(ea, s); if (roctx().mark) roctx().mark("lsfm schur: begin");
	if (strips) return solve_level_dense(ctx, io, strips, warm, eb, ec, ed);
	LevelStructure ls = level_structure(ctx, io, sp, pre.get(), pending, eb);
	pre.reset();
	const SchurSystem& sy = ls.sy;
	CholDev& ch = ls.ch;
	sp = ls.sp;
	const bool dbg = getenv("LSFM_DEBUG") != nullptr;
	PcgWork w = pcg_begin(ctx, io, sy, ch);
	if (ctx->stats && chol_distributed(ctx, ch)) { ctx->stats->dist_solves++; ctx->stats->dist_work_total += ch.work_total; ctx->stats->dist_work_shared += ch.work_shared; }
	chol_scatter(ctx, sy, io.d_fixed, ch);
	if (w.fused_fwd) chol_perm_in(ctx, ch, w.r, io.d_fixed, w.v);
	chol_factor(ctx, sy, io.d_fixed, ch, w.fused_fwd ? w.v : nullptr);
	if (ctx->pcg.mixed) chol_round_to_float(ctx, ch);
	factor_digest_check(ctx, io, sy, ch);
	if (dbg) { LSFM_CHECK_HIP(hipStreamSynchronize(s)); }
	const double tw2 = wall_ms();
	const bool deferred = warm || (ctx->in_tree_run && ctx->d_run && !lp);
	const PcgSteps steps{ warm, deferred, sp ? sp->its : 0, sp ? sp->mixed : false, sp ? sp->rel_tol : 0.0 };
	const PcgResult res = pcg_run(ctx, io, sy, ch, w, steps);
	if (dbg)
	{
		LSFM_CHECK_HIP(hipStreamSynchronize(s));
		fprintf(stderr, "[lsfm] solve M=%d nseg=%d nnzb=%d nnzL=%d etree levels=%d tail=%d leaf tasks=%d group levels=%d %s| analyse %.2f ms, factor %.2f ms, cg(%d its) %.2f ms\n", M, io.nseg,
		        sy.nnzb, ch.nnzL, ch.nlevels, ch.M - ch.tail_begin, ch.ntask0, (int)ch.glevel_ptr.size() - 1, warm ? "(plan) " : "", ls.tw1 - ls.tw0, tw2 - ls.tw1, res.its, wall_ms() - tw2);
	}
	if (ctx->comm)
	{
		Comm& cm = *ctx->comm;
		const size_t nscal = (size_t)M * 6;
		double *x = io.x_pose, *xb = cm.alloc<double>(nscal);
		if (cm.rank == 0) LSFM_CHECK_HIP(hipMemcpyAsync(xb, x, nscal * sizeof(double), hipMemcpyDeviceToDevice, s));
		else fill_async(s, xb, 0, nscal * sizeof(double));
		cm.allreduce(s, xb, nscal, LSFM_DTYPE_F64);
		LSFM_CHECK_HIP(hipMemcpyAsync(x, xb, nscal * sizeof(double), hipMemcpyDeviceToDevice, s));
	}
	pcg_final_residual(ctx, io, sy, w);
	LSFM_REC_T(ec, s); if (roctx().mark) roctx().mark("lsfm back-substitution: begin");
	launch_backsub(ctx, io, sy, io.x_pose);
	LSFM_CHECK_HIP(hipGetLastError());
	LSFM_REC_T(ed, s); if (roctx().mark) roctx().mark("lsfm solve: end");
	SolveOutcome oc;
	oc.keys = sy.upper_keys; oc.nnzb = sy.nnzb;
	oc.end = ed;
	if (ctx->stats)
	{
		lsfm_stats* st = ctx->stats;
		ctx->defer_time(ea, eb, &st->t_schur_ms);
		ctx->defer_time(eb, ec, &st->t_pcg_ms);
		ctx->defer_time(ec, ed, &st->t_backsub_ms);
		ctx->defer_time(w.es0, w.es1, &st->spmv_ms);
		st->pcg_iterations += res.its;
		st->spmv_launches += 1;
		st->spmv_bytes += spmv_bytes(sy);
		st->spmv_nnzb_upper_last = sy.nnzb; st->spmv_rows_last = M;
	}
	oc.steps_used = res.planned ? 0 : std::max(res.its, 1);
	if (deferred)
	{
		if (warm && !res.planned) { sp->its = std::max(res.its, 1); sp->mixed = ctx->pcg.mixed; sp->rel_tol = ctx->pcg.rel_tol; }
		static const bool dbg_conv = getenv("LSFM_DEBUG_CONV") != nullptr;
		if (dbg_conv) debug_conv(ctx, io, sy, ch, w.seg);
		hipLaunchKernelGGL(k_pcg_run_stats, dim3((io.nseg + 127) / 128), dim3(128), 0, s, io.nseg, w.seg, ctx->d_run);
		return oc;
	}
	double maxrel = 0;
	int notconv = pcg_read_verdict(ctx, io, w, &maxrel);
	if (ctx->stats) ctx->stats->max_rel_residual = std::max(ctx->stats->max_rel_residual, maxrel);
	if (ctx->comm)
	{
		long long hv[2] = { notconv, 0 };
		comm_sum_host(ctx, hv, 2);
		notconv = (int)((hv[0] + ctx->comm->world - 1) / ctx->comm->world);
	}
	if (lp && !lp->solve && notconv == 0) lp->solve = solve_plan_store(ctx, sy, ch, std::max(res.its, 1));
	oc.not_converged = notconv;
	return oc;
}

}
```

### linearsfm_amd/csrc/lsfm_pcg.hip

```cpp
#include <algorithm>
#include <cmath>
#include <cstdlib>

#include "lsfm_device.hpp"
#include "lsfm_pcg.hpp"

namespace lsfm {

struct PcgSeg {
	double rz[2];
	double pAp;
	double rr, ee, thresh, rr_prev;
	int done, its, row0, active;
	int slow, pad;
};
static_assert(sizeof(PcgSeg) % sizeof(double) == 0, "PcgSeg is strided in doubles by the fused dot products");
#define SEG_STRIDE ((int)(sizeof(PcgSeg) / sizeof(double)))

__global__ void k_x_init(int M, const double* __restrict__ x0, const unsigned char* __restrict__ fixed, double* __restrict__ x, double* __restrict__ y, int* __restrict__ misc)
{
	size_t i = (size_t)blockIdx.x * blockDim.x + threadIdx.x;
	if (i < 4) misc[i] = 0;
	if (i >= (size_t)M * 6) return;
	y[i] = 0.0;
	double v = x0 ? x0[i] : 0.0;
	if (fixed && fixed[i]) v = 0.0;
	x[i] = v;
}

__global__ void k_pcg_resid(int M, const double* __restrict__ E, double* __restrict__ y, const int* __restrict__ pose_seg,
                            const unsigned char* __restrict__ fixed, double* __restrict__ r, PcgSeg* seg, int with_ee)
{
	int row = blockIdx.x * blockDim.x + threadIdx.x;
	bool v = row < M;
	double a[2] = { 0, 0 };
	int sg = 0;
	if (v)
	{
		sg = pose_seg[row];
		for (int i = 0; i < 6; i++)
		{
			const size_t o = (size_t)row * 6 + i;
			double e = E[o], d = e - y[o];
			y[o] = 0.0;
			if (fixed && fixed[o]) { e = 0; d = 0; }
			if (r) r[o] = d;
			a[0] += d * d; a[1] += e * e;
		}
		if (seg[sg].done) v = false;
	}
	if (!with_ee) a[1] = 0.0;
	wave_scatter_add<2>(&seg[sg].rr, a, v);
}

__global__ void k_pcg_start(int nseg, PcgSeg* seg, const unsigned char* __restrict__ active, double rel_tol, int* ndone, const int* __restrict__ err, RunStatsDev* run)
{
	int s = blockIdx.x * blockDim.x + threadIdx.x;
	if (s == 0 && run && *err && !run->chol_err) run->chol_err = *err;
	if (s >= nseg) return;
	PcgSeg& g = seg[s];
	g.thresh = rel_tol * rel_tol * g.ee;
	g.pAp = 0; g.rz[1] = 0; g.its = 0;
	g.active = active ? active[s] : 1;
	g.done = (!g.active || !(g.rr > g.thresh)) ? 1 : 0;
	g.rr_prev = g.rr;
	seg[nseg + s].rr = g.rr; seg[nseg + s].ee = g.ee;
	g.rr = 0;
	if (g.done) atomicAdd(ndone, 1);
}
__global__ void k_copy(size_t n, const double* __restrict__ a, double* __restrict__ b)
{
	size_t i = (size_t)blockIdx.x * blockDim.x + threadIdx.x;
	if (i < n) b[i] = a[i];
}

__global__ void k_pcg_update1(int M, int cur, const int* __restrict__ pose_seg, double* __restrict__ x, const double* __restrict__ p,
                              double* __restrict__ y, const PcgSeg* __restrict__ seg)
{
	int row = blockIdx.x * blockDim.x + threadIdx.x;
	if (row >= M) return;
	const PcgSeg& g = seg[pose_seg[row]];
	for (int i = 0; i < 6; i++) y[(size_t)row * 6 + i] = 0.0;
	if (g.done) return;
	const double alpha = g.rz[cur] / g.pAp;
	for (int i = 0; i < 6; i++) { const size_t o = (size_t)row * 6 + i; x[o] += alpha * p[o]; }
}

__global__ void k_pcg_update2(int M, int cur, const double* __restrict__ z, const int* __restrict__ pose_seg, double* __restrict__ p,
                              double* __restrict__ Ap, PcgSeg* seg, int* ndone)
{
	int row = blockIdx.x * blockDim.x + threadIdx.x;
	if (row >= M) return;
	const int sg = pose_seg[row];
	PcgSeg& g = seg[sg];
	const bool done = g.done;
	const double rzn = g.rz[cur ^ 1], rzc = g.rz[cur];
	for (int i = 0; i < 6; i++) Ap[(size_t)row * 6 + i] = 0.0;
	if (!done)
	{
		const double beta = rzn / rzc;
		for (int i = 0; i < 6; i++) { const size_t o = (size_t)row * 6 + i; p[o] = z[o] + beta * p[o]; }
	}
}
__global__ void k_pcg_check(int nseg, PcgSeg* seg, int* ndone)
{
	int s = blockIdx.x * blockDim.x + threadIdx.x;
	if (s >= nseg) return;
	PcgSeg& g = seg[s];
	if (g.done) return;
	const double rr = g.rr;
	g.its++;
	seg[nseg + s].rr = rr;
	const bool slow = !(rr < 0.25 * g.rr_prev);
	g.slow = slow ? g.slow + 1 : 0;
	if (!(rr > g.thresh) || !(rr == rr) || (slow && (!(rr > 1e-16 * g.ee) || g.slow >= 10))) { g.done = (rr == rr) ? 1 : 2; atomicAdd(ndone, 1); }
	g.rr_prev = rr;
}
__global__ void k_pcg_reset(int nseg, int cur, PcgSeg* seg)
{
	int s = blockIdx.x * blockDim.x + threadIdx.x;
	if (s >= nseg) return;
	PcgSeg& g = seg[s];
	if (g.done) return;
	g.pAp = 0; g.rr = 0; g.rz[cur] = 0;
}

__global__ void k_pcg_final_zero(int nseg, PcgSeg* fin)
{
	int s = blockIdx.x * blockDim.x + threadIdx.x;
	if (s < nseg) { fin[s].rr = 0.0; fin[s].ee = 0.0; }
}
__global__ void k_pcg_run_stats(int nseg, const PcgSeg* __restrict__ seg, RunStatsDev* run)
{
	int g = blockIdx.x * blockDim.x + threadIdx.x;
	if (g >= nseg || !seg[g].active) return;
	const PcgSeg& fin = seg[nseg + g];
	const double rel = fin.ee > 0 ? sqrt(fin.rr / fin.ee) : 0.0;
	if (!(rel < 1e-8) || (seg[g].done != 1 && !(rel < 1e-9))) atomicAdd(&run->not_converged, 1);
	if (seg[g].done == 0 && !(rel < 1e-10)) atomicAdd(&run->undone, 1);
	atomicMax(reinterpret_cast<unsigned long long*>(&run->max_rel_residual), (unsigned long long)__double_as_longlong(rel == rel ? rel : 1e300));
}
__global__ void k_pcg_debug(int nseg, int M, const PcgSeg* __restrict__ seg)
{
	int g = blockIdx.x * blockDim.x + threadIdx.x;
	if (g >= nseg || !seg[g].active) return;
	const PcgSeg& fin = seg[nseg + g];
	const double rel = fin.ee > 0 ? sqrt(fin.rr / fin.ee) : 0.0;
	if (!(rel < 1e-9))
		printf("[lsfm conv] M=%d nseg=%d system %d: rel %.3e its %d done %d slow %d rr_prev/ee %.3e thresh/ee %.3e ee %.3e pAp %.3e rz %.3e %.3e\n", M, nseg, g, rel, seg[g].its,
		       seg[g].done, seg[g].slow, seg[g].rr_prev / fin.ee, seg[g].thresh / fin.ee, fin.ee, seg[g].pAp, seg[g].rz[0], seg[g].rz[1]);
}

PcgWork pcg_begin(lsfm_context* ctx, const SolveIO& io, const SchurSystem& sy, const CholDev& ch)
{
	hipStream_t s = ctx->stream;
	Arena& sc = ctx->scratch;
	const int M = io.M, nseg = io.nseg;
	PcgWork w;
	w.d_misc = sc.alloc<int>(4);
	std::vector<PcgSeg> hseg(2 * (size_t)nseg);
	memset(hseg.data(), 0, sizeof(PcgSeg) * hseg.size());
	for (int g = 0, row = 0; g < nseg; g++) { hseg[g].row0 = hseg[nseg + g].row0 = row; row += io.seg_rows[g]; }
	w.seg = sc.alloc<PcgSeg>(hseg.size());
	h2d(ctx, w.seg, hseg.data(), sizeof(PcgSeg) * hseg.size());
	const size_t nscal = (size_t)M * 6;
	w.r = sc.alloc<double>(nscal); w.z = ctx->comm ? ctx->comm->alloc<double>(nscal) : sc.alloc<double>(nscal); w.p = sc.alloc<double>(nscal);
	w.Ap = sc.alloc<double>(nscal); w.v = sc.alloc<double>(nscal);
	const unsigned nbe = (unsigned)((nscal + 255) / 256);
	hipLaunchKernelGGL(k_x_init, dim3(std::max(1u, nbe)), dim3(256), 0, s, M, io.x0, io.d_fixed, io.x_pose, w.Ap, w.d_misc);
	launch_spmv(ctx, sy, io.x_pose, w.Ap, io.d_fixed, nullptr, nullptr, nullptr, 1);
	hipLaunchKernelGGL(k_pcg_resid, dim3((M + 127) / 128), dim3(128), 0, s, M, sy.E, w.Ap, io.d_pose_seg, io.d_fixed, w.r, w.seg, 1);
	static const bool no_fused_fwd = getenv("LSFM_NO_FUSED_FWD") != nullptr;
	w.fused_fwd = !ctx->pcg.mixed && !no_fused_fwd && ch.M > 0;
	return w;
}

PcgResult pcg_run(lsfm_context* ctx, const SolveIO& io, const SchurSystem& sy, const CholDev& ch, PcgWork& w, const PcgSteps& steps)
{
	hipStream_t s = ctx->stream;
	const int M = io.M, nseg = io.nseg;
	const size_t nscal = (size_t)M * 6;
	const int nbr = (M + 127) / 128, nbs = (nseg + 127) / 128;
	const unsigned nbe = (unsigned)((nscal + 255) / 256);
	double *x = io.x_pose, *r = w.r, *z = w.z, *p = w.p, *Ap = w.Ap, *v = w.v;
	PcgSeg* seg = w.seg;
	int* d_misc = w.d_misc;
	const bool mixed = ctx->pcg.mixed;
	chol_apply(ctx, ch, r, v, z, io.d_fixed, io.d_pose_seg, &seg[0].rz[0], SEG_STRIDE, w.fused_fwd);
	hipLaunchKernelGGL(k_copy, dim3(nbe), dim3(256), 0, s, nscal, z, p);
	const bool err_to_run = steps.deferred || (ctx->comm && ctx->d_run);
	hipLaunchKernelGGL(k_pcg_start, dim3(nbs), dim3(128), 0, s, nseg, seg, io.d_seg_active, ctx->pcg.rel_tol, d_misc + 1, ch.d_err, err_to_run ? ctx->d_run : (RunStatsDev*)nullptr);

	const int maxit = std::max(1, std::min(50, ctx->pcg.max_steps));
	const bool hinted = !steps.warm && steps.deferred && io.step_hint > 0 && io.step_hint <= maxit;
	const bool planned_run = hinted || (steps.warm && steps.mixed == mixed && steps.rel_tol == ctx->pcg.rel_tol && steps.its <= maxit);
	int its = 0, ndone = 0;
	w.es0 = ctx->pool_event(); w.es1 = ctx->pool_event();
	const bool ask_after = hinted && io.caller_syncs && !ctx->comm;
	const int base_steps = hinted ? io.step_hint : (planned_run ? steps.its : maxit);
	const int planned = (planned_run && !ask_after && base_steps >= (mixed ? 3 : 2)) ? std::min(base_steps + 1, maxit) : base_steps;
	bool counting = planned_run;
	int cap = maxit;
	while ((counting ? its < planned : (ndone < nseg && its < cap)))
	{
		const int cur = its & 1;
		launch_spmv(ctx, sy, p, Ap, io.d_fixed, p, io.d_pose_seg, &seg[0].pAp, SEG_STRIDE);
		hipLaunchKernelGGL(k_pcg_update1, dim3(nbr), dim3(128), 0, s, M, cur, io.d_pose_seg, x, p, Ap, seg);
		if (!w.es_done) LSFM_REC_T(w.es0, s);
		launch_spmv(ctx, sy, x, Ap, io.d_fixed, nullptr, nullptr, nullptr, 1);
		if (!w.es_done) { LSFM_REC_T(w.es1, s); w.es_done = true; }
		hipLaunchKernelGGL(k_pcg_resid, dim3(nbr), dim3(128), 0, s, M, sy.E, Ap, io.d_pose_seg, io.d_fixed, r, seg, 0);
		hipLaunchKernelGGL(k_pcg_check, dim3(nbs), dim3(128), 0, s, nseg, seg, d_misc + 1);
		its++;
		if (counting)
		{
			if (its >= planned)
			{
				if (!ask_after) break;
				ndone = d2h_int(ctx, d_misc + 1);
				if (ndone >= nseg || its >= maxit) break;
				counting = false;
				cap = std::min(maxit, planned + 3);
			}
		}
		else
		{
			ctx->mark("cg_enq");
			ndone = d2h_int(ctx, d_misc + 1);
			ctx->mark("cg_sync");
			const int cerr = (its == 1 && !err_to_run) ? d2h_int(ctx, ch.d_err) : 0;
			if (cerr) LSFM_FAIL(LSFM_ERR_NOT_SPD, "Schur system is not positive definite (block column " + std::to_string(cerr - 1) + " of the factor)");
			if (ctx->comm && ctx->comm->world > 1)
			{
				long long more = ndone >= nseg ? 0 : 1;
				comm_sum_host(ctx, &more, 1);
				if (!more) break;
				ndone = std::min(ndone, nseg - 1);
			}
			else if (ndone >= nseg) break;
		}
		chol_apply(ctx, ch, r, v, z, io.d_fixed, io.d_pose_seg, &seg[0].rz[cur ^ 1], SEG_STRIDE);
		hipLaunchKernelGGL(k_pcg_update2, dim3(nbr), dim3(128), 0, s, M, cur, z, io.d_pose_seg, p, Ap, seg, d_misc + 1);
		hipLaunchKernelGGL(k_pcg_reset, dim3(nbs), dim3(128), 0, s, nseg, cur, seg);
	}
	return PcgResult{ its, planned_run };
}

void pcg_final_residual(lsfm_context* ctx, const SolveIO& io, const SchurSystem& sy, PcgWork& w)
{
	if (!ctx->comm && w.es_done) return;
	hipStream_t s = ctx->stream;
	const int M = io.M, nseg = io.nseg, nbr = (M + 127) / 128, nbs = (nseg + 127) / 128;
	PcgSeg* seg2 = w.seg + nseg;
	if (!w.es_done) LSFM_REC_T(w.es0, s);
	launch_spmv(ctx, sy, io.x_pose, w.Ap, io.d_fixed, nullptr, nullptr, nullptr, 1);
	if (!w.es_done) { LSFM_REC_T(w.es1, s); w.es_done = true; }
	hipLaunchKernelGGL(k_pcg_final_zero, dim3(nbs), dim3(128), 0, s, nseg, seg2);
	hipLaunchKernelGGL(k_pcg_resid, dim3(nbr), dim3(128), 0, s, M, sy.E, w.Ap, io.d_pose_seg, io.d_fixed, (double*)nullptr, seg2, 1);
}

int pcg_read_verdict(lsfm_context* ctx, const SolveIO& io, const PcgWork& w, double* maxrel)
{
	const int nseg = io.nseg;
	std::vector<PcgSeg> hs2(2 * (size_t)nseg);
	d2h(ctx, hs2.data(), w.seg, sizeof(PcgSeg) * 2 * nseg);
	int notconv = 0;
	*maxrel = 0;
	for (int g = 0; g < nseg; g++)
	{
		if (!hs2[g].active) continue;
		const PcgSeg& fin = hs2[nseg + g];
		const double rel = fin.ee > 0 ? sqrt(fin.rr / fin.ee) : 0.0;
		*maxrel = std::max(*maxrel, rel);
		if (!(rel < 1e-8) || (hs2[g].done != 1 && !(rel < 1e-9))) notconv++;
	}
	return notconv;
}

}
```

### linearsfm_amd/csrc/lsfm_pcg.hpp

```cpp
#pragma once
#include "lsfm_chol.hpp"

namespace lsfm {

struct PcgSeg;

struct PcgWork {
	double *r = nullptr, *z = nullptr, *p = nullptr, *Ap = nullptr, *v = nullptr;
	PcgSeg* seg = nullptr;
	int* d_misc = nullptr;
	bool fused_fwd = false;
	hipEvent_t es0 = nullptr, es1 = nullptr;
	bool es_done = false;
};
struct PcgSteps { bool warm, deferred; int its; bool mixed; double rel_tol; };
struct PcgResult { int its; bool planned; };

PcgWork pcg_begin(lsfm_context* ctx, const SolveIO& io, const SchurSystem& sy, const CholDev& ch);
PcgResult pcg_run(lsfm_context* ctx, const SolveIO& io, const SchurSystem& sy, const CholDev& ch, PcgWork& w, const PcgSteps& steps);
void pcg_final_residual(lsfm_context* ctx, const SolveIO& io, const SchurSystem& sy, PcgWork& w);
__global__ void k_pcg_run_stats(int nseg, const PcgSeg* __restrict__ seg, RunStatsDev* run);
__global__ void k_pcg_debug(int nseg, int M, const PcgSeg* __restrict__ seg);
int pcg_read_verdict(lsfm_context* ctx, const SolveIO& io, const PcgWork& w, double* maxrel);

}
```

### linearsfm_amd/csrc/lsfm_solve.hip

```cpp
#include <algorithm>
#include <cmath>

#include "lsfm_device.hpp"
#include "lsfm_internal.hpp"
#include "lsfm_solve.hpp"

namespace lsfm {

__global__ void __launch_bounds__(256) k_vinv(int NF, const double* __restrict__ V, const double* __restrict__ eb, double* __restrict__ IV, double* __restrict__ LY,
                                               double* __restrict__ ymax, RhsFused rhs, double* __restrict__ uu)
{
	__shared__ double wmax[4];
	int f = blockIdx.x * blockDim.x + threadIdx.x;
	double y2 = 0.0;
	if (f < NF)
	{
	double a[9], o[9];
	ld<9>(a, V + (size_t)f * 9);
	inv3_sym(a, o);
	st<9>(IV + (size_t)f * 9, o);
	const double* e = eb + (size_t)f * 3;
	double l[9];
	const double d0 = o[0];
	l[0] = sqrt(d0);
	l[1] = o[3] / l[0];
	l[3] = o[6] / l[0];
	const double d1 = o[4] - l[1] * l[1];
	l[2] = sqrt(d1);
	l[4] = (o[7] - l[3] * l[1]) / l[2];
	const double d2 = o[8] - l[3] * l[3] - l[4] * l[4];
	l[5] = sqrt(d2);
	l[6] = l[0] * e[0] + l[1] * e[1] + l[3] * e[2];
	l[7] = l[2] * e[1] + l[4] * e[2];
	l[8] = l[5] * e[2];
	if (!(d0 > 0.0) || !(d1 > 0.0) || !(d2 > 0.0)) l[0] = __builtin_nan("");
	st<9>(LY + (size_t)f * 9, l);
	y2 = l[6] * l[6] + l[7] * l[7] + l[8] * l[8];
	if (uu)
	{
#pragma unroll
		for (int sd = 0; sd < 2; sd++)
		{
			const int fs = sd ? rhs.srcC[f] : rhs.srcE[f];
			double u0 = 0.0, u1 = 0.0, u2 = 0.0;
			if (fs >= 0)
			{
				const double* x = rhs.feat_src + (size_t)fs * 3;
				u0 = x[0] / l[0];
				u1 = (x[1] - l[1] * u0) / l[2];
				u2 = (x[2] - l[3] * u0 - l[4] * u1) / l[5];
			}
			uu[(size_t)f * 6 + 3 * sd] = u0; uu[(size_t)f * 6 + 3 * sd + 1] = u1; uu[(size_t)f * 6 + 3 * sd + 2] = u2;
			y2 = fmax(y2, u0 * u0 + u1 * u1 + u2 * u2);
		}
	}
	if (!(y2 == y2)) y2 = 0.0;
	}
	if (!ymax) return;
#pragma unroll
	for (int off = 32; off > 0; off >>= 1) y2 = fmax(y2, __shfl_xor(y2, off, LSFM_WAVE));
	if ((threadIdx.x & (LSFM_WAVE - 1)) == 0) wmax[threadIdx.x >> 6] = y2;
	__syncthreads();
	if (threadIdx.x == 0) ymax[blockIdx.x] = fmax(fmax(wmax[0], wmax[1]), fmax(wmax[2], wmax[3]));
}

__device__ __forceinline__ int half_exponent(double d)
{
	if (!(d > 0.0) || !(d < 1e300)) return 0;
	int k;
	(void)frexp(d, &k);
	return ((k + 1) >> 1) + 1;
}
__global__ void __launch_bounds__(256) k_schur_scale(int M, const int* __restrict__ rowptr, const double* __restrict__ S, int NF, int nymax,
                                                      const double* __restrict__ ymax, const unsigned char* __restrict__ fixed, int* __restrict__ sexp,
                                                      const double* __restrict__ ea, double* __restrict__ E)
{
	const int i = blockIdx.x * blockDim.x + threadIdx.x;
	if (i < 6 * M)
	{
		E[i] = ea[i];
		const int p = i / 6, r = i - 6 * p;
		sexp[i] = (fixed && fixed[i]) ? 400 : half_exponent(S[(size_t)rowptr[p] * 36 + 7 * r]);
	}
	if (blockIdx.x == 0)
	{
		__shared__ double wmax[4];
		double m = 0.0;
		for (int b = threadIdx.x; b < nymax; b += 256) m = fmax(m, ymax[b]);
#pragma unroll
		for (int off = 32; off > 0; off >>= 1) m = fmax(m, __shfl_xor(m, off, LSFM_WAVE));
		if ((threadIdx.x & (LSFM_WAVE - 1)) == 0) wmax[threadIdx.x >> 6] = m;
		__syncthreads();
		if (threadIdx.x == 0) sexp[6 * (size_t)M] = half_exponent((double)NF * fmax(fmax(wmax[0], wmax[1]), fmax(wmax[2], wmax[3]))) + 20;
	}
}
__global__ void k_schur_finish(int nnzb, int M, const unsigned long long* __restrict__ keys, const long long* __restrict__ acc, const int* __restrict__ sexp,
                               double* __restrict__ S, double* __restrict__ E)
{
	const size_t i = (size_t)blockIdx.x * blockDim.x + threadIdx.x;
	const size_t ns = (size_t)nnzb * 36, ne = (size_t)M * 6;
	const bool poison = acc[0] != 0;
	acc += 1;
	if (i < ns)
	{
		const unsigned long long key = keys[i / 36];
		const int p = (int)(key >> 32), q = (int)(key & 0xffffffffull), rc = (int)(i % 36);
		const double v = ldexp((double)acc[i], sexp[6 * (size_t)p + rc / 6] + sexp[6 * (size_t)q + rc % 6] - 60);
		S[i] = poison ? __builtin_nan("") : S[i] - v;
	}
	else if (i < ns + ne)
	{
		const size_t k = i - ns;
		const int e = sexp[k] + sexp[ne] - 62;
		const double v = ldexp((double)acc[ns + k], e) + ldexp((double)acc[ns + ne + k], e - 40);
		E[k] = poison ? __builtin_nan("") : E[k] + v;
	}
}

__global__ void __launch_bounds__(256) k_sum_run_squares(int NF, const int* __restrict__ fptr, unsigned long long* out)
{
	__shared__ unsigned long long part[4];
	unsigned long long v = 0;
	for (int f = blockIdx.x * blockDim.x + threadIdx.x; f < NF; f += gridDim.x * blockDim.x)
	{
		const unsigned long long k = (unsigned long long)(fptr[f + 1] - fptr[f]);
		v += k * k;
	}
#pragma unroll
	for (int off = 32; off > 0; off >>= 1) v += __shfl_xor(v, off, LSFM_WAVE);
	if ((threadIdx.x & (LSFM_WAVE - 1)) == 0) part[threadIdx.x >> 6] = v;
	__syncthreads();
	if (threadIdx.x == 0) { v = part[0] + part[1] + part[2] + part[3]; if (v) atomicAdd(out, v); }
}

#define SCHUR_U_BLOCKS 256
__global__ void __launch_bounds__(SCHUR_U_BLOCKS) k_schur_u(int NU, const double* __restrict__ U, const int* __restrict__ Ui, const int* __restrict__ Uj,
                                                          const unsigned long long* __restrict__ tab, const int* __restrict__ val, unsigned long long mask,
                                                          double* __restrict__ S)
{
	__shared__ int s_slot[SCHUR_U_BLOCKS];
	const int i0 = blockIdx.x * SCHUR_U_BLOCKS, nb = min(SCHUR_U_BLOCKS, NU - i0);
	if ((int)threadIdx.x < nb)
	{
		const int a = Ui[i0 + threadIdx.x], b = Uj[i0 + threadIdx.x];
		const int slot = hash_find(tab, val, mask, pair_key(a, b));
		s_slot[threadIdx.x] = slot < 0 ? -1 : (slot | (a <= b ? 0 : (1 << 30)));
	}
	__syncthreads();
	const double* u = U + (size_t)i0 * 36;
	for (int p = threadIdx.x; p < nb * 36; p += SCHUR_U_BLOCKS)
	{
		const int blk = p / 36, q = p - 36 * blk, sl = s_slot[blk];
		if (sl < 0) continue;
		const int slot = sl & ((1 << 30) - 1);
		const int qq = (sl >> 30) ? (q % 6) * 6 + q / 6 : q;
		atomic_add_f64(S + (size_t)slot * 36 + qq, u[p]);
	}
}

#define SCHUR_TILE 128
#define SCHUR_CAP 256
#define SCHUR_ECAP 64

__global__ void __launch_bounds__(SCHUR_TILE)
k_schur_w(int NF, const int* __restrict__ fptr, const int* __restrict__ photo, const double* __restrict__ W, const double* __restrict__ IV,
          const double* __restrict__ eb, const unsigned long long* __restrict__ tab, const int* __restrict__ val, unsigned long long mask,
          K9Out o, const unsigned char* __restrict__ only, const double* __restrict__ LY)
{
	if (only && !only[blockIdx.x / (LSFM_PM_TILE / SCHUR_TILE)]) return;
	__shared__ int skey[SCHUR_CAP];
	__shared__ int ekey[SCHUR_ECAP];
	__shared__ long long sval[SCHUR_CAP * 36];
	__shared__ long long evalv[SCHUR_ECAP * 12];
	const int tid = threadIdx.x;
	for (int i = tid; i < SCHUR_CAP; i += SCHUR_TILE) skey[i] = -1;
	for (int i = tid; i < SCHUR_ECAP; i += SCHUR_TILE) ekey[i] = -1;
	for (int i = tid; i < SCHUR_CAP * 36; i += SCHUR_TILE) sval[i] = 0;
	for (int i = tid; i < SCHUR_ECAP * 12; i += SCHUR_TILE) evalv[i] = 0;
	__syncthreads();
	const int f = blockIdx.x * SCHUR_TILE + tid;
	bool bad = false;
	const int ey = *o.ey;
	if (f < NF)
	{
		const int j0 = fptr[f], len = fptr[f + 1] - j0;
		double iv[9];
		ld<9>(iv, IV + (size_t)f * 9);
		double eb0 = eb[(size_t)f * 3], eb1 = eb[(size_t)f * 3 + 1], eb2 = eb[(size_t)f * 3 + 2];
		double xfs[2][3] = { { 0.0, 0.0, 0.0 }, { 0.0, 0.0, 0.0 } };
		if (o.xpose)
		{
			for (int a = 0; a < len; a++)
			{
				const double* wa = W + (size_t)(j0 + a) * 18;
				const double* xp = o.xpose + (size_t)photo[j0 + a] * 6;
#pragma unroll
				for (int r = 0; r < 6; r++) { eb0 = fma(wa[3 * r], xp[r], eb0); eb1 = fma(wa[3 * r + 1], xp[r], eb1); eb2 = fma(wa[3 * r + 2], xp[r], eb2); }
			}
			const double* l = LY + (size_t)f * 9;
			if (!(l[0] == l[0])) bad = true;
#pragma unroll
			for (int sd = 0; sd < 2; sd++)
			{
				const double* u = o.uu + (size_t)f * 6 + 3 * sd;
				xfs[sd][0] = l[0] * u[0]; xfs[sd][1] = l[1] * u[0] + l[2] * u[1]; xfs[sd][2] = l[3] * u[0] + l[4] * u[1] + l[5] * u[2];
			}
		}
		for (int a = 0; a < len; a++)
		{
			double WV[18], Wa[18];
			const int pa = photo[j0 + a];
			ld<18>(Wa, W + (size_t)(j0 + a) * 18);
			mm<6, 3, 3, false>(Wa, iv, WV);
			int ea6[6];
#pragma unroll
			for (int r = 0; r < 6; r++) ea6[r] = o.sexp[(size_t)pa * 6 + r];
			{
				const int es = lds_slot(ekey, SCHUR_ECAP, pa);
#pragma unroll
				for (int r = 0; r < 6; r++)
				{
					double e = -(WV[3 * r] * eb0 + WV[3 * r + 1] * eb1 + WV[3 * r + 2] * eb2);
					if (o.xpose) { const double* xf = xfs[o.pside[pa] & 1]; e += Wa[3 * r] * xf[0] + Wa[3 * r + 1] * xf[1] + Wa[3 * r + 2] * xf[2]; }
					long long hi, lo;
					to_fixed2(e, 62 - ea6[r] - ey, hi, lo, bad);
					if (es >= 0) { lds_add_i64(&evalv[es * 6 + r], hi); lds_add_i64(&evalv[SCHUR_ECAP * 6 + es * 6 + r], lo); }
					else { atomic_add_i64(o.Ehi + (size_t)pa * 6 + r, hi); atomic_add_i64(o.Elo + (size_t)pa * 6 + r, lo); }
				}
			}
			for (int b = a; b < len; b++)
			{
				double Wb[18], T[36];
				const int pb = photo[j0 + b];
				ld<18>(Wb, W + (size_t)(j0 + b) * 18);
				mmt<6, 3, 6, false>(WV, Wb, T);
				const int slot = hash_find(tab, val, mask, pair_key(pa, pb));
				const int ls = lds_slot(skey, SCHUR_CAP, slot);
				long long* dl = ls >= 0 ? &sval[ls * 36] : nullptr;
				long long* dg = o.S + (size_t)slot * 36;
				int eb6[6];
#pragma unroll
				for (int c = 0; c < 6; c++) eb6[c] = o.sexp[(size_t)pb * 6 + c];
				const bool same = (pa == pb), tr = pa > pb, twice = same && a != b;
#pragma unroll
				for (int r = 0; r < 6; r++)
#pragma unroll
					for (int c = 0; c < 6; c++)
					{
						double x = T[r * 6 + c];
						if (twice) x += T[c * 6 + r];
						const int at = tr ? c * 6 + r : r * 6 + c;
						const long long q = to_fixed(x, 60 - ea6[r] - eb6[c], bad);
						if (dl) lds_add_i64(dl + at, q); else atomic_add_i64(dg + at, q);
					}
			}
		}
	}
	if (bad) atomic_add_i64(o.poison, 1);
	__syncthreads();
	for (int i = tid; i < SCHUR_CAP * 36; i += SCHUR_TILE)
	{
		const int k = skey[i / 36];
		if (k >= 0 && sval[i]) atomic_add_i64(o.S + (size_t)k * 36 + i % 36, sval[i]);
	}
	for (int i = tid; i < SCHUR_ECAP * 6; i += SCHUR_TILE)
	{
		const int k = ekey[i / 6];
		if (k >= 0)
		{
			if (evalv[i]) atomic_add_i64(o.Ehi + (size_t)k * 6 + i % 6, evalv[i]);
			if (evalv[SCHUR_ECAP * 6 + i]) atomic_add_i64(o.Elo + (size_t)k * 6 + i % 6, evalv[SCHUR_ECAP * 6 + i]);
		}
	}
}

#define SPT 16
#define SPW 64
#define SP_LONG 256
#define SP_FAR 64
#define SPMV_CACHED_BYTES ((size_t)96 << 20)
__global__ void k_spmv_long_rows(int M, const int* __restrict__ rowptr, int* __restrict__ nlong, int* __restrict__ longrows)
{
	int r = blockIdx.x * blockDim.x + threadIdx.x;
	if (r < M && rowptr[r + 1] - rowptr[r] > SP_LONG) longrows[atomicAdd(nlong, 1)] = r;
}
__global__ void __launch_bounds__(256)
k_spmv(int M, const int* __restrict__ rowptr, const int* __restrict__ colidx, const int* __restrict__ nlong_p, const int* __restrict__ longrows,
       const double* __restrict__ S, const double* __restrict__ x, double* __restrict__ y, const unsigned char* __restrict__ fixed,
       const double* __restrict__ dotw, const int* __restrict__ pose_seg, double* __restrict__ dot, int dot_stride)
{
	__shared__ int pre[SPT + 1];
	__shared__ int rp[SPT + 1];
	__shared__ double ywin[(SPT + SPW) * 6];
	__shared__ int fkeys[SP_FAR];
	__shared__ double fvals[SP_FAR * 6];
	const int tid = threadIdx.x, g = tid >> 3, r = tid & 7, ng = blockDim.x >> 3;
	const int r0 = blockIdx.x * SPT, r1 = min(r0 + SPT, M), nr = r1 - r0;
	for (int i = tid; i < (SPT + SPW) * 6; i += blockDim.x) ywin[i] = 0.0;
	for (int i = tid; i < SP_FAR; i += blockDim.x) fkeys[i] = -1;
	for (int i = tid; i < SP_FAR * 6; i += blockDim.x) fvals[i] = 0.0;
	for (int i = tid; i <= nr; i += blockDim.x) rp[i] = rowptr[r0 + i];
	__syncthreads();
	if (tid == 0)
	{
		int acc = 0;
		for (int i = 0; i < nr; i++) { pre[i] = acc; const int len = rp[i + 1] - rp[i]; acc += len > SP_LONG ? 0 : len; }
		pre[nr] = acc;
	}
	__syncthreads();
	auto add = [&](int t, double v) {
		const int w = t - r0;
		if (w >= 0 && w < SPT + SPW) { lds_add_f64(&ywin[w * 6 + r], v); return; }
		const int sl = lds_slot(fkeys, SP_FAR, t);
		if (sl >= 0) { lds_add_f64(&fvals[sl * 6 + r], v); return; }
		if (fixed && fixed[(size_t)t * 6 + r]) return;
		atomic_add_f64(y + (size_t)t * 6 + r, v);
		if (dotw) atomic_add_f64(dot + (size_t)pose_seg[t] * dot_stride, dotw[(size_t)t * 6 + r] * v);
	};
	auto block = [&](int k, int p) {
		const int q = colidx[k];
		const double* blk = S + (size_t)k * 36;
		const double* xq = x + (size_t)q * 6;
		double sum = 0.0;
#pragma unroll
		for (int j = 0; j < 6; j++) sum = fma(blk[r * 6 + j], xq[j], sum);
		add(p, sum);
		if (q != p)
		{
			const double* xp = x + (size_t)p * 6;
			double t = 0.0;
#pragma unroll
			for (int j = 0; j < 6; j++) t = fma(blk[j * 6 + r], xp[j], t);
			add(q, t);
		}
	};
	const int nb = pre[nr];
	if (r < 6)
		for (int i = g; i < nb; i += ng)
		{
			int lo = 0, hi = nr - 1;
			while (lo < hi) { const int mid = (lo + hi + 1) >> 1; if (pre[mid] <= i) lo = mid; else hi = mid - 1; }
			block(rp[lo] + (i - pre[lo]), r0 + lo);
		}
	__shared__ int lstart[SP_FAR];
	const int nlong = *nlong_p;
	for (int l0 = 0; l0 < nlong; l0 += SP_FAR)
	{
		const int nl = min(SP_FAR, nlong - l0);
		__syncthreads();
		if (tid < nl)
		{
			const int h = longrows[l0 + tid];
			int lo = rowptr[h], hi = rowptr[h + 1];
			const int guess = lo + max(r0 - h, 0);
			if (guess < hi && colidx[guess] >= r0 && (guess == lo || colidx[guess - 1] < r0)) lo = guess;
			else
				while (lo < hi) { const int mid = (lo + hi) >> 1; if (colidx[mid] < r0) lo = mid + 1; else hi = mid; }
			lstart[tid] = lo;
		}
		__syncthreads();
		if (r < 6)
			for (int li = 0; li < nl; li++)
			{
				const int h = longrows[l0 + li], he = rowptr[h + 1];
				for (int k = lstart[li] + g; k < he && colidx[k] < r1; k += ng) block(k, h);
			}
	}
	__syncthreads();
	double w = 0.0;
	int seg = 0;
	bool any = false;
	for (int i = tid; i < (SPT + SPW) * 6; i += blockDim.x)
	{
		const int t = r0 + i / 6;
		const double v = ywin[i];
		if (t < M && v != 0.0 && !(fixed && fixed[(size_t)t * 6 + i % 6]))
		{
			atomic_add_f64(y + (size_t)t * 6 + i % 6, v);
			if (dotw)
			{
				const int sg = pose_seg[t];
				if (any && sg != seg) { atomic_add_f64(dot + (size_t)seg * dot_stride, w); w = 0.0; }
				seg = sg; any = true;
				w = fma(dotw[(size_t)t * 6 + i % 6], v, w);
			}
		}
	}
	for (int i = tid; i < SP_FAR * 6; i += blockDim.x)
	{
		const int t = fkeys[i / 6];
		const double v = fvals[i];
		if (t >= 0 && v != 0.0 && !(fixed && fixed[(size_t)t * 6 + i % 6]))
		{
			atomic_add_f64(y + (size_t)t * 6 + i % 6, v);
			if (dotw)
			{
				const int sg = pose_seg[t];
				if (any && sg != seg) { atomic_add_f64(dot + (size_t)seg * dot_stride, w); w = 0.0; }
				seg = sg; any = true;
				w = fma(dotw[(size_t)t * 6 + i % 6], v, w);
			}
		}
	}
	if (dotw) wave_scatter_add<1>(dot + (size_t)seg * dot_stride, &w, any);
}

#define SPG_EPG 8
#define SPG_ENT (32 * SPG_EPG)
__global__ void k_spmv_gather_keys(int nnzb, const unsigned long long* __restrict__ upper_keys, unsigned long long* __restrict__ ent,
                                   int* __restrict__ oth)
{
	const int k = blockIdx.x * blockDim.x + threadIdx.x;
	if (k >= nnzb) return;
	const unsigned long long key = upper_keys[k];
	const unsigned p = (unsigned)(key >> 32), q = (unsigned)(key & 0xffffffffull);
	ent[k] = ((unsigned long long)p << 32) | ((unsigned)k << 1);
	oth[k] = (int)q;
	ent[(size_t)nnzb + k] = p != q ? (((unsigned long long)q << 32) | ((unsigned)k << 1) | 1u) : ~0ull;
	oth[(size_t)nnzb + k] = (int)p;
}
__global__ void __launch_bounds__(256)
k_spmv_gather(int M, int nent, const unsigned long long* __restrict__ ent, const int* __restrict__ oth, const double* __restrict__ S,
              const double* __restrict__ x, double* __restrict__ y, const unsigned char* __restrict__ fixed, const double* __restrict__ dotw,
              const int* __restrict__ pose_seg, double* __restrict__ dot, int dot_stride)
{
	__shared__ double ywin[SPG_ENT * 6];
	const int tid = threadIdx.x, g = tid >> 3, r = tid & 7;
	const int eb = blockIdx.x * SPG_ENT;
	const int row0 = (int)(ent[eb] >> 32);
	for (int i = tid; i < SPG_ENT * 6; i += 256) ywin[i] = 0.0;
	__syncthreads();
	const int e0 = eb + g * SPG_EPG;
	if (r < 6 && e0 < nent && row0 >= 0)
	{
		unsigned long long key[SPG_EPG];
		int ot[SPG_EPG];
#pragma unroll
		for (int i = 0; i < SPG_EPG; i++)
		{
			const bool in = e0 + i < nent;
			key[i] = in ? ent[e0 + i] : ~0ull;
			ot[i] = in ? oth[e0 + i] : 0;
		}
		double sum[SPG_EPG];
#pragma unroll
		for (int i = 0; i < SPG_EPG; i++)
		{
			sum[i] = 0.0;
			if (key[i] == ~0ull) continue;
			const unsigned kk = (unsigned)(key[i] & 0xffffffffull);
			const double* blk = S + (size_t)(kk >> 1) * 36;
			const double* xo = x + (size_t)ot[i] * 6;
			double s = 0.0;
			if (kk & 1u)
			{
#pragma unroll
				for (int j = 0; j < 6; j++) s = fma(blk[j * 6 + r], xo[j], s);
			}
			else
			{
#pragma unroll
				for (int j = 0; j < 6; j++) s = fma(blk[r * 6 + j], xo[j], s);
			}
			sum[i] = s;
		}
		auto put = [&](int row, double v) {
			if (row - row0 < SPG_ENT) { lds_add_f64(&ywin[(row - row0) * 6 + r], v); return; }
			if (fixed && fixed[(size_t)row * 6 + r]) return;
			atomic_add_f64(y + (size_t)row * 6 + r, v);
			if (dotw) atomic_add_f64(dot + (size_t)pose_seg[row] * dot_stride, dotw[(size_t)row * 6 + r] * v);
		};
		int cur = -1;
		double acc = 0.0;
#pragma unroll
		for (int i = 0; i < SPG_EPG; i++)
		{
			if (key[i] == ~0ull) continue;
			const int row = (int)(key[i] >> 32);
			if (row != cur)
			{
				if (cur >= 0) put(cur, acc);
				cur = row; acc = 0.0;
			}
			acc += sum[i];
		}
		if (cur >= 0) put(cur, acc);
	}
	__syncthreads();
	double w = 0.0;
	int seg = 0;
	bool any = false;
	if (row0 >= 0)
		for (int i = tid; i < SPG_ENT * 6; i += 256)
		{
			const int t = row0 + i / 6;
			const double v = ywin[i];
			if (t < M && v != 0.0 && !(fixed && fixed[(size_t)t * 6 + i % 6]))
			{
				atomic_add_f64(y + (size_t)t * 6 + i % 6, v);
				if (dotw)
				{
					const int sg = pose_seg[t];
					if (any && sg != seg) { atomic_add_f64(dot + (size_t)seg * dot_stride, w); w = 0.0; }
					seg = sg; any = true;
					w = fma(dotw[(size_t)t * 6 + i % 6], v, w);
				}
			}
		}
	if (dotw) wave_scatter_add<1>(dot + (size_t)seg * dot_stride, &w, any);
}

#define BSUB_TILE 128
__global__ void __launch_bounds__(256)
k_backsub(int NF, const int* __restrict__ fptr, const int* __restrict__ photo, const double* __restrict__ W,
          const double* __restrict__ IV, const double* __restrict__ eb, const double* __restrict__ xp,
          const int* __restrict__ feat_seg, const unsigned char* __restrict__ active, double* __restrict__ xf,
          const double* __restrict__ LY, const double* __restrict__ xhat)
{
	__shared__ int sFp[BSUB_TILE + 1];
	__shared__ double sT[256 * 3];
	__shared__ double sS[BSUB_TILE * 3];
	const int f0 = blockIdx.x * BSUB_TILE, nft = min(BSUB_TILE, NF - f0);
	for (int i = threadIdx.x; i <= nft; i += blockDim.x) sFp[i] = fptr[f0 + i];
	for (int i = threadIdx.x; i < nft * 3; i += blockDim.x) sS[i] = 0.0;
	__syncthreads();
	tile_runs<3>(nft, sFp, sT,
		[&](int j, int, double* out) {
			double w[18];
			ld<18>(w, W + (size_t)j * 18);
			const double* a = xp + (size_t)photo[j] * 6;
			double a6[6];
			ld<6>(a6, a);
			if (xhat)
			{
				const double* h = xhat + (size_t)photo[j] * 6;
#pragma unroll
				for (int r = 0; r < 6; r++) a6[r] -= h[r];
			}
#pragma unroll
			for (int c = 0; c < 3; c++)
			{
				double sacc = 0.0;
#pragma unroll
				for (int r = 0; r < 6; r++) sacc = fma(w[3 * r + c], a6[r], sacc);
				out[c] = sacc;
			}
		},
		[&](int fl, int q, double sum, bool) { sS[fl * 3 + q] += sum; });
	for (int fl = threadIdx.x; fl < nft; fl += blockDim.x)
	{
		const int f = f0 + fl;
		if (active && !active[feat_seg[f]]) continue;
		if (xhat)
		{
			const double* l = LY + (size_t)f * 9;
			const double s0 = sS[fl * 3], s1 = sS[fl * 3 + 1], s2 = sS[fl * 3 + 2];
			const double d0 = l[6] - (l[0] * s0 + l[1] * s1 + l[3] * s2), d1 = l[7] - (l[2] * s1 + l[4] * s2),
			             d2 = l[8] - l[5] * s2;
			xf[(size_t)f * 3] = l[0] * d0; xf[(size_t)f * 3 + 1] = l[1] * d0 + l[2] * d1; xf[(size_t)f * 3 + 2] = l[3] * d0 + l[4] * d1 + l[5] * d2;
			continue;
		}
		const double* iv = IV + (size_t)f * 9;
		const double d[3] = { eb[(size_t)f * 3] - sS[fl * 3], eb[(size_t)f * 3 + 1] - sS[fl * 3 + 1], eb[(size_t)f * 3 + 2] - sS[fl * 3 + 2] };
		for (int r = 0; r < 3; r++) xf[(size_t)f * 3 + r] = iv[3 * r] * d[0] + iv[3 * r + 1] * d[1] + iv[3 * r + 2] * d[2];
	}
}

__global__ void k_low_words(int n, const unsigned long long* __restrict__ keys, int* __restrict__ out)
{
	int i = blockIdx.x * blockDim.x + threadIdx.x;
	if (i < n) out[i] = (int)(keys[i] & 0xffffffffull);
}

void build_spmv_index(lsfm_context* ctx, SchurSystem& sy, const unsigned long long* sorted_upper)
{
	hipStream_t s = ctx->stream;
	Arena& sc = ctx->scratch;
	const int M = sy.M, cnt = sy.nnzb;
	if (!sy.rowptr)
	{
		sy.rowptr = sc.alloc<int>(M + 1);
		rowptr_from_keys(ctx, M, cnt, sorted_upper, sy.rowptr);
	}
	if (!sy.colidx)
	{
		sy.colidx = sc.alloc<int>(cnt + 1);
		if (cnt) hipLaunchKernelGGL(k_low_words, dim3((cnt + 255) / 256), dim3(256), 0, s, cnt, sorted_upper, sy.colidx);
	}
	int* nl = sc.alloc<int>(1);
	sy.longrows = sc.alloc<int>(M + 1);
	dev_zero(ctx, nl, sizeof(int));
	if (M) hipLaunchKernelGGL(k_spmv_long_rows, dim3((M + 255) / 256), dim3(256), 0, s, M, sy.rowptr, nl, sy.longrows);
	sy.d_nlong = nl;
	sy.gent = nullptr; sy.goth = nullptr;
	const int variant = ctx->pcg.spmv_variant;
	if (cnt && variant != 1 && (variant == 2 || (size_t)cnt * 288 <= SPMV_CACHED_BYTES))
	{
		unsigned long long* ent = sc.alloc<unsigned long long>((size_t)2 * cnt);
		int* oth = sc.alloc<int>((size_t)2 * cnt);
		hipLaunchKernelGGL(k_spmv_gather_keys, dim3((cnt + 255) / 256), dim3(256), 0, s, cnt, sorted_upper, ent, oth);
		int rb = 1;
		while ((1 << rb) <= M) rb++;
		dev_sort_pairs_u64(ctx, ent, oth, (size_t)2 * cnt, 32 + rb, 32);
		sy.gent = ent; sy.goth = oth;
	}
}

void schur_vinv(lsfm_context* ctx, const SolveIO& io, SchurSystem& sy)
{
	sy.IV = ctx->scratch.alloc<double>((size_t)io.NF * 9);
	sy.LY = ctx->scratch.alloc<double>((size_t)io.NF * 9);
	sy.ymax = ctx->scratch.alloc<double>((size_t)(io.NF + 255) / 256 + 1);
	sy.uu = nullptr;
	if (io.rhs) sy.uu = ctx->scratch.alloc<double>((size_t)io.NF * 6);
	if (io.NF) hipLaunchKernelGGL(k_vinv, dim3((io.NF + 255) / 256), dim3(256), 0, ctx->stream, io.NF, io.V, io.eb, sy.IV, sy.LY, sy.ymax, io.rhs ? *io.rhs : RhsFused(), sy.uu);
}

void build_schur_values(lsfm_context* ctx, const SolveIO& io, SchurSystem& sy)
{
	hipStream_t s = ctx->stream;
	Arena& sc = ctx->scratch;
	const int M = io.M, NF = io.NF, cnt = sy.nnzb;
	const unsigned long long* tab = sy.tab;
	const int* hval = sy.hval;
	const unsigned long long mask = sy.mask;
	const int ntiles = (NF + SCHUR_TILE - 1) / SCHUR_TILE;
	unsigned char* fb;
	const size_t nacc = 1 + (size_t)cnt * 36 + (size_t)M * 12;
	if (ctx->comm)
	{
		ctx->comm->restart();
		sy.acc = ctx->comm->alloc<long long>(nacc);
		sy.E = ctx->comm->alloc<double>((size_t)M * 6);
		fill_async(s, sy.acc, 0, nacc * sizeof(long long));
		ZeroSpan zs(sc);
		sy.S = sc.alloc<double>((size_t)cnt * 36);
		fb = sc.alloc<unsigned char>(ntiles + 1);
		zs.zero(s);
	}
	else
	{
		ZeroSpan zs(sc);
		sy.S = sc.alloc<double>((size_t)cnt * 36);
		fb = sc.alloc<unsigned char>(ntiles + 1);
		sy.acc = sc.alloc<long long>(nacc);
		zs.zero(s);
		sy.E = sc.alloc<double>((size_t)M * 6);
	}
	sy.sexp = sc.alloc<int>((size_t)M * 6 + 1);
	if (io.NU) hipLaunchKernelGGL(k_schur_u, dim3((io.NU + 255) / 256), dim3(256), 0, s, io.NU, io.U, io.Ui, io.Uj, tab, hval, mask, sy.S);
	hipLaunchKernelGGL(k_schur_scale, dim3((6 * M + 255) / 256 + 1), dim3(256), 0, s, M, sy.rowptr, sy.S, NF, NF ? (NF + 255) / 256 : 0, sy.ymax, io.d_fixed, sy.sexp, io.ea, sy.E);
	K9Out ko;
	ko.poison = sy.acc; ko.S = sy.acc + 1; ko.Ehi = ko.S + (size_t)cnt * 36; ko.Elo = ko.Ehi + (size_t)M * 6;
	ko.sexp = sy.sexp; ko.ey = sy.sexp + (size_t)M * 6;
	if (io.rhs) { ko.xpose = io.rhs->pose_src; ko.pside = io.rhs->pose_map_src; ko.uu = sy.uu; }
	if (NF)
	{
		hipEvent_t e2 = nullptr, e3 = nullptr;
		if (ctx->stats) { e2 = ctx->pool_event(); e3 = ctx->pool_event(); LSFM_REC_T(e2, s); }
		static_assert(LSFM_PM_TILE % SCHUR_TILE == 0, "a tile of the panel kernel must be whole tiles of the fallback kernel");
		bool fresh_lists = false;
		if (!sy.k9.ns)
		{
			fresh_lists = true;
			sy.k9.ns = sc.alloc<int>(ntiles + 1);
			sy.k9.pose = sc.alloc<int>((size_t)ntiles * 64 + 1);
			sy.k9.eslot = sc.alloc<unsigned char>((size_t)io.NW + 1);
			sy.k9.wlist = sc.alloc<int>((size_t)3 * ntiles + 1);
			sy.k9.wcnt = sc.alloc<int>(8);
			sy.k9_tiles = ntiles; sy.k9_NW = io.NW;
			launch_schur_slots(ctx, NF, io.fptr, io.photo, fb, sy.k9);
		}
		launch_schur_panel(ctx, NF, io.fptr, io.photo, io.W, sy.LY, tab, hval, mask, ko, fb, most_rows(io.seg_rows), sy.k9, fresh_lists);
		hipLaunchKernelGGL(k_schur_w, dim3(ntiles), dim3(SCHUR_TILE), 0, s, NF, io.fptr, io.photo, io.W, sy.IV, io.eb, tab, hval, mask, ko, fb, sy.LY);
		if (ctx->stats)
		{
			LSFM_REC_T(e3, s);
			ctx->defer_time(e2, e3, &ctx->stats->schur_ms);
			ctx->stats->schur_launches++;
			ctx->stats->schur_bytes += (double)io.NW * (144 + 4) + (double)io.NF * (72 + 24 + 4) + (double)sy.nnzb * 288 + (double)io.M * 48;
			ctx->stats->schur_flops += (double)io.NW * (144.0 + 108.0);
			if (io.rhs) { ctx->stats->schur_flops += (double)io.NW * 72.0; ctx->stats->schur_bytes += (double)io.NF * (48 + 24) + (double)io.M * 48; }
			if (ctx->in_tree_run && ctx->d_run)
			{
				Fork side(ctx, ctx->stream2, evR_fork);
				hipLaunchKernelGGL(k_sum_run_squares, dim3(std::min((NF + 255) / 256, 512)), dim3(256), 0, ctx->stream, NF, io.fptr, &ctx->d_run->k2);
				side.done(evR_done);
			}
		}
	}
	if (ctx->comm) ctx->comm->allreduce(s, sy.acc, 1 + (size_t)cnt * 36, LSFM_DTYPE_I64);
	{
		const size_t n = (size_t)cnt * 36 + (size_t)M * 6;
		hipLaunchKernelGGL(k_schur_finish, dim3((unsigned)((n + 255) / 256)), dim3(256), 0, s, cnt, M, sy.upper_keys, sy.acc, sy.sexp, sy.S, sy.E);
	}
	if (ctx->comm) ctx->comm->allreduce(s, sy.E, (size_t)M * 6, LSFM_DTYPE_F64);
	LSFM_CHECK_HIP(hipGetLastError());
}

void launch_spmv(lsfm_context* ctx, const SchurSystem& sy, const double* x, double* y, const unsigned char* fixed,
                 const double* dotw, const int* pose_seg, double* dot, int dot_stride)
{
	if (!sy.M) return;
	if (sy.gent)
	{
		const int nent = 2 * sy.nnzb;
		hipLaunchKernelGGL(k_spmv_gather, dim3((nent + SPG_ENT - 1) / SPG_ENT), dim3(256), 0, ctx->stream, sy.M, nent, sy.gent, sy.goth, sy.S, x, y, fixed,
		                   dotw, pose_seg, dot, dot_stride);
		return;
	}
	hipLaunchKernelGGL(k_spmv, dim3((sy.M + SPT - 1) / SPT), dim3(256), 0, ctx->stream, sy.M, sy.rowptr, sy.colidx, sy.d_nlong, sy.longrows, sy.S, x, y,
	                   fixed, dotw, pose_seg, dot, dot_stride);
}

double spmv_bytes(const SchurSystem& sy) { return (double)sy.nnzb * (288 + 4) + 4.0 * (sy.M + 1) + 2.0 * 48 * sy.M; }

void launch_backsub(lsfm_context* ctx, const SolveIO& io, const SchurSystem& sy, const double* x)
{
	if (io.NF)
		hipLaunchKernelGGL(k_backsub, dim3((io.NF + BSUB_TILE - 1) / BSUB_TILE), dim3(256), 0, ctx->stream, io.NF, io.fptr, io.photo, io.W, sy.IV, io.eb, x,
		                   io.d_feat_seg, io.d_seg_active, io.x_feat, sy.LY, io.rhs ? io.rhs->pose_src : (const double*)nullptr);
}

int inverse_v(lsfm_context* ctx, double* V, int n)
{
	ctx->ensure_arenas((size_t)n * 400 + ((size_t)64 << 20));
	ctx->arena[0].reset(); ctx->scratch.reset();
	double* dV = ctx->arena[0].alloc<double>((size_t)n * 9);
	double* dIV = ctx->arena[0].alloc<double>((size_t)n * 9);
	h2d(ctx, dV, V, (size_t)n * 9 * sizeof(double));
	if (n)
	{
		double* LY = ctx->scratch.alloc<double>((size_t)n * 9);
		double* eb = ctx->scratch.alloc<double>((size_t)n * 3);
		dev_zero(ctx, eb, (size_t)n * 3 * sizeof(double));
		hipLaunchKernelGGL(k_vinv, dim3((n + 255) / 256), dim3(256), 0, ctx->stream, n, dV, eb, dIV, LY, (double*)nullptr, RhsFused(), (double*)nullptr);
		LSFM_CHECK_HIP(hipStreamSynchronize(ctx->stream));
	}
	d2h(ctx, V, dIV, (size_t)n * 9 * sizeof(double));
	return LSFM_OK;
}
int solve_features(lsfm_context* ctx, const double* W, const double* IV, const double* eb, const double* dpa, double* dpb, int m, int n, const int* mapCor,
                   const int* photo)
{
	std::vector<int> fptr((size_t)n + 1, 0);
	for (int f = 0; f < n; f++)
	{
		if (mapCor[f] < 0) LSFM_FAIL(LSFM_ERR_ARG, "negative block count of a feature");
		fptr[f + 1] = fptr[f] + mapCor[f];
	}
	const int nW = fptr[n];
	for (int j = 0; j < nW; j++) if (photo[j] < 0 || photo[j] >= m) LSFM_FAIL(LSFM_ERR_ARG, "photo index out of range");
	ctx->ensure_arenas((size_t)nW * 200 + (size_t)n * 300 + (size_t)m * 100 + ((size_t)64 << 20));
	ctx->arena[0].reset(); ctx->scratch.reset();
	Arena& ar = ctx->arena[0];
	double* dW = ar.alloc<double>((size_t)nW * 18); int* dph = ar.alloc<int>(nW); int* dfp = ar.alloc<int>((size_t)n + 1);
	double* dIV = ar.alloc<double>((size_t)n * 9); double* deb = ar.alloc<double>((size_t)n * 3);
	double* dxp = ar.alloc<double>((size_t)m * 6); double* dxf = ar.alloc<double>((size_t)n * 3);
	h2d(ctx, dW, W, (size_t)nW * 18 * sizeof(double)); h2d(ctx, dph, photo, (size_t)nW * sizeof(int));
	h2d(ctx, dfp, fptr.data(), ((size_t)n + 1) * sizeof(int)); h2d(ctx, dIV, IV, (size_t)n * 9 * sizeof(double));
	h2d(ctx, deb, eb, (size_t)n * 3 * sizeof(double)); h2d(ctx, dxp, dpa, (size_t)m * 6 * sizeof(double));
	if (n)
		hipLaunchKernelGGL(k_backsub, dim3((n + BSUB_TILE - 1) / BSUB_TILE), dim3(256), 0, ctx->stream, n, dfp, dph, dW, dIV, deb, dxp,
		                   (const int*)nullptr, (const unsigned char*)nullptr, dxf, (const double*)nullptr, (const double*)nullptr);
	d2h(ctx, dpb, dxf, (size_t)n * 3 * sizeof(double));
	return LSFM_OK;
}

int spmv_external(lsfm_context* ctx, int m, const int* rowptr, const int* colidx, const double* val, const double* x, double* y, int reps,
                  double* avg_ms, double* bytes)
{
	hipStream_t s = ctx->stream;
	Arena& sc = ctx->scratch;
	size_t mk = sc.mark();
	const int nnzb = rowptr[m];
	SchurSystem sy;
	sy.M = m; sy.nnzb = nnzb;
	std::vector<unsigned long long> keys(nnzb);
	for (int p = 0; p < m; p++)
		for (int k = rowptr[p]; k < rowptr[p + 1]; k++) keys[k] = ((unsigned long long)(unsigned)p << 32) | (unsigned)colidx[k];
	unsigned long long* dk = sc.alloc<unsigned long long>(nnzb + 1);
	sy.S = sc.alloc<double>((size_t)nnzb * 36);
	double* dx = sc.alloc<double>((size_t)m * 6);
	double* dy = sc.alloc<double>((size_t)m * 6);
	h2d(ctx, dk, keys.data(), (size_t)nnzb * sizeof(unsigned long long));
	h2d(ctx, sy.S, val, (size_t)nnzb * 36 * sizeof(double));
	h2d(ctx, dx, x, (size_t)m * 6 * sizeof(double));
	build_spmv_index(ctx, sy, dk);
	float total = 0;
	hipEvent_t e0 = ctx->pool_event(), e1 = ctx->pool_event();
	for (int k = 0; k < reps + 2; k++)
	{
		dev_zero(ctx, dy, (size_t)m * 6 * sizeof(double));
		LSFM_CHECK_HIP(hipEventRecord(e0, s));
		launch_spmv(ctx, sy, dx, dy, nullptr, nullptr, nullptr, nullptr, 1);
		LSFM_CHECK_HIP(hipEventRecord(e1, s));
		LSFM_CHECK_HIP(hipEventSynchronize(e1));
		float t = 0;
		LSFM_CHECK_HIP(hipEventElapsedTime(&t, e0, e1));
		if (k >= 2) total += t;
	}
	d2h(ctx, y, dy, (size_t)m * 6 * sizeof(double));
	if (avg_ms) *avg_ms = reps > 0 ? total / reps : 0;
	if (bytes) *bytes = spmv_bytes(sy);
	sc.release(mk);
	return 0;
}

}
```

### linearsfm_amd/csrc/lsfm_solve.hpp

```cpp
#pragma once
#include "lsfm_device.hpp"
#include "lsfm_internal.hpp"

#ifndef LSFM_PM_TILE
#define LSFM_PM_TILE 128
#endif

namespace lsfm {

struct K9Cache {
	int* ns = nullptr;
	int* pose = nullptr;
	unsigned char* eslot = nullptr;
	int* wlist = nullptr;
	int* wcnt = nullptr;
};

struct SchurSystem {
	int M = 0, nnzb = 0;
	int *rowptr = nullptr, *colidx = nullptr;
	const unsigned long long* upper_keys = nullptr;
	double* S = nullptr;
	double* E = nullptr;
	double* IV = nullptr;
	double* LY = nullptr;
	int* longrows = nullptr;
	const int* d_nlong = nullptr;
	const unsigned long long* gent = nullptr;
	const int* goth = nullptr;
	const unsigned long long* tab = nullptr;
	const int* hval = nullptr;
	unsigned long long mask = 0;
	long long* acc = nullptr;
	int* sexp = nullptr;
	double* uu = nullptr;
	double* ymax = nullptr;
	K9Cache k9;
	int k9_tiles = 0, k9_NW = 0;
	double k9_flops = 0;
};

struct PatternSeed {
	const unsigned long long* prev_keys = nullptr;
	int prev_nnzb = 0;
	const int* pnew = nullptr;
	const unsigned char* dropped = nullptr;
	int NFY = 0;
	const int *srcE = nullptr, *srcC = nullptr;
	const int *fptr_in = nullptr, *photo_in = nullptr;
};
struct EarlyPatternIn {
	int M = 0, NFY = 0, NU = 0;
	const int *Ui = nullptr, *Uj = nullptr, *pose_map = nullptr, *hub = nullptr;
	const int *fptr = nullptr, *photo = nullptr, *feat_map = nullptr, *srcE = nullptr, *srcC = nullptr;
};
void build_schur_pattern(lsfm_context* ctx, const SolveIO& io, SchurSystem& sy);
void schur_pattern_only(lsfm_context* ctx, const SolveIO& io, int* nnzb, const int** rowptr, const int** colidx);
void schur_pattern_early_issue(lsfm_context* ctx, const EarlyPatternIn& in);
void schur_pattern_early_drop(lsfm_context* ctx);
bool schur_pattern_early_finish(lsfm_context* ctx, const SolveIO& io, SchurSystem& sy);
void schur_pattern_early_extras(lsfm_context* ctx, SchurSystem& sy);
bool schur_pattern_prefetch(lsfm_context* ctx, const DevBatch& Y, const int* d_tref, const unsigned long long* prev_keys, int prev_nnzb, SchurSystem& sy,
                            std::vector<int>* counts = nullptr, bool want_pattern = true, LevelIndex* keep = nullptr);
void schur_pattern_check(lsfm_context* ctx, const SolveIO& io, const SchurSystem& sy, const char* what);
void rowptr_from_keys(lsfm_context* ctx, int M, int cnt, const unsigned long long* sorted_upper, int* rowptr);

void build_schur_values(lsfm_context* ctx, const SolveIO& io, SchurSystem& sy);
void schur_vinv(lsfm_context* ctx, const SolveIO& io, SchurSystem& sy);
void build_spmv_index(lsfm_context* ctx, SchurSystem& sy, const unsigned long long* sorted_upper);
void launch_spmv(lsfm_context* ctx, const SchurSystem& sy, const double* x, double* y, const unsigned char* fixed, const double* dotw,
                 const int* pose_seg, double* dot, int dot_stride);
double spmv_bytes(const SchurSystem& sy);
void launch_schur_slots(lsfm_context* ctx, int NF, const int* fptr, const int* photo, unsigned char* fallback, K9Cache kc);
struct K9Out {
	long long* S = nullptr;
	long long *Ehi = nullptr, *Elo = nullptr;
	long long* poison = nullptr;
	const int* sexp = nullptr;
	const int* ey = nullptr;
	const double* xpose = nullptr;
	const int* pside = nullptr;
	const double* uu = nullptr;
};
struct RhsFused {
	const int *srcE = nullptr, *srcC = nullptr;
	const double* feat_src = nullptr;
	const double* pose_src = nullptr;
	const int* pose_map_src = nullptr;
};
void launch_schur_panel(lsfm_context* ctx, int NF, const int* fptr, const int* photo, const double* W, const double* LY,
                        const unsigned long long* tab, const int* val, unsigned long long mask, K9Out out, unsigned char* fallback,
                        int max_poses_per_system, K9Cache kc, bool fresh_lists = false);
void launch_backsub(lsfm_context* ctx, const SolveIO& io, const SchurSystem& sy, const double* x);

static const unsigned long long HEMPTY = ~0ull;
__device__ __forceinline__ unsigned long long mix64(unsigned long long x)
{
	x ^= x >> 33; x *= 0xff51afd7ed558ccdull; x ^= x >> 33; x *= 0xc4ceb9fe1a85ec53ull; x ^= x >> 33;
	return x;
}
__device__ __forceinline__ void hash_insert_mixed(unsigned long long* tab, unsigned long long mask, unsigned long long key, unsigned long long hm, int* overflow)
{
	unsigned long long h = hm & mask;
	for (int probe = 0; probe < 4096; probe++)
	{
		unsigned long long cur = tab[h];
		if (cur == key) return;
		if (cur == HEMPTY)
		{
			unsigned long long old = atomicCAS(&tab[h], HEMPTY, key);
			if (old == HEMPTY || old == key) return;
		}
		h = (h + 1) & mask;
	}
	*overflow = 1;
}
__device__ __forceinline__ void hash_insert(unsigned long long* tab, unsigned long long mask, unsigned long long key, int* overflow)
{
	hash_insert_mixed(tab, mask, key, mix64(key), overflow);
}
constexpr int PAIRSET_SLOTS = 2048;
constexpr int PAIRSET_PROBES = 8;
__device__ __forceinline__ void pairset_clear(unsigned long long* set)
{
	for (int i = threadIdx.x; i < PAIRSET_SLOTS; i += blockDim.x) set[i] = HEMPTY;
}
__device__ __forceinline__ void pairset_insert(unsigned long long* set, unsigned long long* tab, unsigned long long mask, unsigned long long key, int* overflow)
{
	const unsigned long long hm = mix64(key);
	unsigned s = (unsigned)(hm >> 40) & (PAIRSET_SLOTS - 1);
	for (int probe = 0; probe < PAIRSET_PROBES; probe++)
	{
		unsigned long long cur = set[s];
		if (cur == HEMPTY) cur = atomicCAS(&set[s], HEMPTY, key);
		if (cur == key) return;
		if (cur == HEMPTY) break;
		s = (s + 1) & (PAIRSET_SLOTS - 1);
	}
	hash_insert_mixed(tab, mask, key, hm, overflow);
}
__device__ __forceinline__ int hash_find(const unsigned long long* __restrict__ tab, const int* __restrict__ val, unsigned long long mask,
                                         unsigned long long key)
{
	unsigned long long h = mix64(key) & mask;
	for (int probe = 0; probe < 4096; probe++)
	{
		unsigned long long cur = tab[h];
		if (cur == key) return val[h];
		if (cur == HEMPTY) return -1;
		h = (h + 1) & mask;
	}
	return -1;
}
__device__ __forceinline__ unsigned long long pair_key(int p, int q)
{
	return p <= q ? (((unsigned long long)(unsigned)p << 32) | (unsigned)q) : (((unsigned long long)(unsigned)q << 32) | (unsigned)p);
}

}
```

Baseline: 31.66.

## Fold PCG setup into Schur assembly and overlap vinv/slots on side stream

Restructures the start of each level solve: PCG vector and record allocation, x/y initialisation, and factor buffer zeroing are merged into the Schur assembly's single zeroing span and its k_schur_scale kernel. k_vinv and the U-scatter now run on a second stream alongside slot building. Residual and perm-in are fused into one kernel, and run-stat accounting moves into the check kernel. The aim is fewer kernel launches, fewer memsets and less serialisation, at the cost of callback-based control flow and new stream synchronisation.

New measurement: 31.67. Within noise of the previous version (+0.0%).

```diff
diff --git a/linearsfm_amd/csrc/lsfm_chol.hip b/linearsfm_amd/csrc/lsfm_chol.hip
--- a/linearsfm_amd/csrc/lsfm_chol.hip
+++ b/linearsfm_amd/csrc/lsfm_chol.hip
@@ -1136,7 +1136,8 @@
 }
 __global__ void k_perm_out_dot(int M, const int* __restrict__ pinv, const double* __restrict__ v, const double* __restrict__ r,
                                const unsigned char* __restrict__ fixed, const double* __restrict__ dscale, const int* __restrict__ pose_seg,
-                               double* __restrict__ z, double* dot, int dot_stride, const int* __restrict__ col_owner, int rank)
+                               double* __restrict__ z, double* dot, int dot_stride, const int* __restrict__ col_owner, int rank,
+                               double* __restrict__ z_copy, double* __restrict__ clear)
 {
 	int row = blockIdx.x * blockDim.x + threadIdx.x;
 	const bool ok = row < M;
@@ -1153,6 +1154,8 @@
 			if (fixed && fixed[(size_t)row * 6 + i]) zz = 0.0;
 			if (col_owner) { const int ow = col_owner[pinv[row]]; if (!(ow == rank || (ow < 0 && rank == 0))) zz = 0.0; }
 			z[(size_t)row * 6 + i] = zz;
+			if (z_copy) z_copy[(size_t)row * 6 + i] = zz;
+			if (clear) clear[(size_t)row * 6 + i] = 0.0;
 			acc = fma(zz, r[(size_t)row * 6 + i], acc);
 		}
 	}
@@ -1182,19 +1185,30 @@
 	d2h(ctx, in.keys.data(), sy.upper_keys, (size_t)nnzb * sizeof(unsigned long long));
 }
 
-void chol_alloc_values(lsfm_context* ctx, CholDev& ch)
+void chol_alloc_zeroed(lsfm_context* ctx, CholDev& ch)
 {
 	Arena& sc = ctx->scratch;
-	ch.L = sc.alloc<double>((size_t)ch.nnzL * 36); ch.Dinv = sc.alloc<double>((size_t)ch.M * 36);
+	static const bool digest = getenv("LSFM_FACTOR_DIGEST") != nullptr;
+	ch.Lg = nullptr;
+	ch.L = sc.alloc<double>((size_t)ch.nnzL * 36);
+	if (digest && ch.ngroups) ch.Lg = sc.alloc<double>((size_t)ch.nnzL * 36);
+	ch.d_err = sc.alloc<int>(1);
+}
+void chol_alloc_rest(lsfm_context* ctx, CholDev& ch)
+{
+	Arena& sc = ctx->scratch;
+	ch.Dinv = sc.alloc<double>((size_t)ch.M * 36);
 	ch.wv = sc.alloc<double>((size_t)ch.M * 6);
 	ch.diag0 = sc.alloc<double>((size_t)ch.M * 6);
 	ch.dscale = sc.alloc<double>((size_t)ch.M * 6);
-	ch.Lg = ch.ngroups ? sc.alloc<double>((size_t)ch.nnzL * 36) : nullptr;
-	dev_zero(ctx, ch.L, (size_t)ch.nnzL * 36 * sizeof(double));
-	static const bool digest = getenv("LSFM_FACTOR_DIGEST") != nullptr;
-	if (digest && ch.Lg) dev_zero(ctx, ch.Lg, (size_t)ch.nnzL * 36 * sizeof(double));
-	ch.d_err = sc.alloc<int>(1);
-	dev_zero(ctx, ch.d_err, sizeof(int));
+	if (ch.ngroups && !ch.Lg) ch.Lg = sc.alloc<double>((size_t)ch.nnzL * 36);
+}
+void chol_alloc_values(lsfm_context* ctx, CholDev& ch)
+{
+	ZeroSpan zs(ctx->scratch);
+	chol_alloc_zeroed(ctx, ch);
+	zs.zero(ctx->stream);
+	chol_alloc_rest(ctx, ch);
 }
 
 static size_t chol_task_lds(const CholDev& ch) { return (size_t)ch.task0_maxsize * CHOL_TASK_LDS_PER_COL + 8; }
@@ -1379,9 +1393,10 @@
 }
 
 void chol_apply(lsfm_context* ctx, const CholDev& ch, const double* r, double* v, double* z, const unsigned char* fixed, const int* pose_seg,
-                double* dot, int dot_stride, bool fwd_done)
+                double* dot, int dot_stride, bool fwd_done, double* z_copy, double* clear)
 {
 	hipStream_t s = ctx->stream;
+	if ((z_copy || clear) && chol_distributed(ctx, ch)) LSFM_FAIL(LSFM_ERR_INTERNAL, "chol_apply: z_copy / clear with a distributed factorisation");
 	if (!fwd_done) chol_perm_in(ctx, ch, r, fixed, v);
 	const int ngl = (int)ch.glevel_ptr.size() - 1;
 	const bool dist = chol_distributed(ctx, ch);
@@ -1416,12 +1431,13 @@
 	if (dist)
 	{
 		hipLaunchKernelGGL(k_perm_out_dot, dim3((ch.M + 127) / 128), dim3(128), 0, s, ch.M, ch.pinv, v, r, fixed, ch.dscale, pose_seg, z, (double*)nullptr, dot_stride,
-		                   ch.col_owner, ctx->comm->rank);
+		                   ch.col_owner, ctx->comm->rank, (double*)nullptr, (double*)nullptr);
 		ctx->comm->allreduce(s, z, (size_t)ch.M * 6, LSFM_DTYPE_F64);
 		hipLaunchKernelGGL(k_rz_dot, dim3((ch.M + 127) / 128), dim3(128), 0, s, ch.M, z, r, pose_seg, dot, dot_stride);
 	}
 	else
-		hipLaunchKernelGGL(k_perm_out_dot, dim3((ch.M + 127) / 128), dim3(128), 0, s, ch.M, ch.pinv, v, r, fixed, ch.dscale, pose_seg, z, dot, dot_stride, (const int*)nullptr, 0);
+		hipLaunchKernelGGL(k_perm_out_dot, dim3((ch.M + 127) / 128), dim3(128), 0, s, ch.M, ch.pinv, v, r, fixed, ch.dscale, pose_seg, z, dot, dot_stride, (const int*)nullptr, 0,
+		                   z_copy, clear);
 }
 
 int chol_selftest(lsfm_context* ctx, int m, const int* rowptr, const int* colidx, const double* val, const int* origin, const unsigned char* fixed,
diff --git a/linearsfm_amd/csrc/lsfm_chol.hpp b/linearsfm_amd/csrc/lsfm_chol.hpp
--- a/linearsfm_amd/csrc/lsfm_chol.hpp
+++ b/linearsfm_amd/csrc/lsfm_chol.hpp
@@ -69,12 +69,15 @@
 void chol_upload_index(lsfm_context* ctx, const CholSymbolic& sym, CholDev& ch);
 void chol_upload_symbolic(lsfm_context* ctx, const CholSymbolic& sym, CholDev& ch);
 void chol_alloc_values(lsfm_context* ctx, CholDev& ch);
+void chol_alloc_zeroed(lsfm_context* ctx, CholDev& ch);
+void chol_alloc_rest(lsfm_context* ctx, CholDev& ch);
 void chol_scatter(lsfm_context* ctx, const SchurSystem& sy, const unsigned char* fixed, CholDev& ch);
 void chol_factor(lsfm_context* ctx, const SchurSystem& sy, const unsigned char* fixed, CholDev& ch, double* fwd_v = nullptr);
 void chol_merge_groups(lsfm_context* ctx, const CholDev& ch);
 void chol_round_to_float(lsfm_context* ctx, CholDev& ch);
 void chol_perm_in(lsfm_context* ctx, const CholDev& ch, const double* r, const unsigned char* fixed, double* v);
-void chol_apply(lsfm_context* ctx, const CholDev& ch, const double* r, double* v, double* z, const unsigned char* fixed, const int* pose_seg, double* dot, int dot_stride, bool fwd_done = false);
+void chol_apply(lsfm_context* ctx, const CholDev& ch, const double* r, double* v, double* z, const unsigned char* fixed, const int* pose_seg, double* dot, int dot_stride, bool fwd_done = false,
+                double* z_copy = nullptr, double* clear = nullptr);
 bool chol_distributed(const lsfm_context* ctx, const CholDev& ch);
 void comm_sum_host(lsfm_context* ctx, long long* h, int n);
 
diff --git a/linearsfm_amd/csrc/lsfm_internal.hpp b/linearsfm_amd/csrc/lsfm_internal.hpp
--- a/linearsfm_amd/csrc/lsfm_internal.hpp
+++ b/linearsfm_amd/csrc/lsfm_internal.hpp
@@ -210,6 +210,8 @@
 	evU,
 	evG,
 	evT,
+	evS_fork,
+	evS_done,
 	evK9_fork,
 	evK9_done,
 	evR_fork,
diff --git a/linearsfm_amd/csrc/lsfm_level.hip b/linearsfm_amd/csrc/lsfm_level.hip
--- a/linearsfm_amd/csrc/lsfm_level.hip
+++ b/linearsfm_amd/csrc/lsfm_level.hip
@@ -198,20 +198,27 @@
 	double tw0 = 0, tw1 = 0;
 };
 static double wall_ms() { return std::chrono::duration<double, std::milli>(std::chrono::steady_clock::now().time_since_epoch()).count(); }
-static LevelStructure level_structure(lsfm_context* ctx, const SolveIO& io, SolvePlan* sp, PreLevel* pre, bool pending, hipEvent_t eb)
+static LevelStructure level_structure(lsfm_context* ctx, const SolveIO& io, SolvePlan* sp, PreLevel* pre, bool pending, hipEvent_t eb, SolveStart start)
 {
 	hipStream_t s = ctx->stream;
 	LevelStructure ls;
 	SchurSystem& sy = ls.sy;
 	CholDev& ch = ls.ch;
 	auto assemble = [&]() {
-		build_schur_values(ctx, io, sy);
+		build_schur_values(ctx, io, sy, &start);
 		LSFM_REC_T(eb, s); if (roctx().mark) roctx().mark("lsfm factor + refine: begin");
 	};
 	if (sp || pending)
 	{
 		sy = pending ? pre->sy : sp->sy;
-		schur_vinv(ctx, io, sy);
+		start.vinv = true;
+		const bool factor_with_s = sp && (level_overlap(ctx) & 2);
+		if (factor_with_s)
+		{
+			ch = sp->ch;
+			const std::function<void()> before = start.zeroed;
+			start.zeroed = [ctx, &ch, before]() { if (before) before(); chol_alloc_zeroed(ctx, ch); };
+		}
 		assemble();
 		if (pending)
 		{
@@ -221,20 +228,19 @@
 			ctx->mark("sym_wait");
 		}
 		ls.sp = sp;
-		ch = sp->ch;
-		chol_alloc_values(ctx, ch);
+		if (factor_with_s) chol_alloc_rest(ctx, ch);
+		else { ch = sp->ch; chol_alloc_values(ctx, ch); }
 		return ls;
 	}
-	schur_vinv(ctx, io, sy);
+	if (pre && !(pre->M == io.M && !ctx->comm)) pre = nullptr;
+	if (pre) start.vinv = true;
+	else schur_vinv(ctx, io, sy);
 	CholHostIn hin;
 	bool have = false;
-	if (pre && !(pre->M == io.M && !ctx->comm)) pre = nullptr;
 	if (pre)
 	{
 		schur_pattern_early_drop(ctx);
-		SchurSystem prepared = pre->sy;
-		prepared.IV = sy.IV; prepared.LY = sy.LY; prepared.ymax = sy.ymax; prepared.uu = sy.uu;
-		sy = prepared;
+		sy = pre->sy;
 		have = true;
 		wait_for(ctx, s, evP);
 		if (getenv("LSFM_CHECK_EARLY_PATTERN")) schur_pattern_check(ctx, io, sy, "prefetched");
@@ -394,16 +400,20 @@
 	hipEvent_t ea = ctx->pool_event(), eb = ctx->pool_event(), ec = ctx->pool_event(), ed = ctx->pool_event();
 	LSFM_REC_T(ea, s); if (roctx().mark) roctx().mark("lsfm schur: begin");
 	if (strips) return solve_level_dense(ctx, io, strips, warm, eb, ec, ed);
-	LevelStructure ls = level_structure(ctx, io, sp, pre.get(), pending, eb);
+	PcgWork w;
+	SolveStart start;
+	if (level_overlap(ctx) & 2) pcg_start_with_assembly(ctx, io, w, start);
+	LevelStructure ls = level_structure(ctx, io, sp, pre.get(), pending, eb, start);
 	pre.reset();
 	const SchurSystem& sy = ls.sy;
 	CholDev& ch = ls.ch;
 	sp = ls.sp;
 	const bool dbg = getenv("LSFM_DEBUG") != nullptr;
-	PcgWork w = pcg_begin(ctx, io, sy, ch);
+	w = pcg_begin(ctx, io, sy, ch, w);
 	if (ctx->stats && chol_distributed(ctx, ch)) { ctx->stats->dist_solves++; ctx->stats->dist_work_total += ch.work_total; ctx->stats->dist_work_shared += ch.work_shared; }
 	chol_scatter(ctx, sy, io.d_fixed, ch);
-	if (w.fused_fwd) chol_perm_in(ctx, ch, w.r, io.d_fixed, w.v);
+	if (w.pairs) pcg_resid_perm_in(ctx, io, sy, ch, w);
+	else if (w.fused_fwd) chol_perm_in(ctx, ch, w.r, io.d_fixed, w.v);
 	chol_factor(ctx, sy, io.d_fixed, ch, w.fused_fwd ? w.v : nullptr);
 	if (ctx->pcg.mixed) chol_round_to_float(ctx, ch);
 	factor_digest_check(ctx, io, sy, ch);
@@ -454,7 +464,7 @@
 		if (warm && !res.planned) { sp->its = std::max(res.its, 1); sp->mixed = ctx->pcg.mixed; sp->rel_tol = ctx->pcg.rel_tol; }
 		static const bool dbg_conv = getenv("LSFM_DEBUG_CONV") != nullptr;
 		if (dbg_conv) debug_conv(ctx, io, sy, ch, w.seg);
-		hipLaunchKernelGGL(k_pcg_run_stats, dim3((io.nseg + 127) / 128), dim3(128), 0, s, io.nseg, w.seg, ctx->d_run);
+		if (!res.stats_left) hipLaunchKernelGGL(k_pcg_run_stats, dim3((io.nseg + 127) / 128), dim3(128), 0, s, io.nseg, w.seg, ctx->d_run);
 		return oc;
 	}
 	double maxrel = 0;
diff --git a/linearsfm_amd/csrc/lsfm_pcg.hip b/linearsfm_amd/csrc/lsfm_pcg.hip
--- a/linearsfm_amd/csrc/lsfm_pcg.hip
+++ b/linearsfm_amd/csrc/lsfm_pcg.hip
@@ -11,16 +11,15 @@
 	double rz[2];
 	double pAp;
 	double rr, ee, thresh, rr_prev;
-	int done, its, row0, active;
+	int done, its, pad0, active;
 	int slow, pad;
 };
 static_assert(sizeof(PcgSeg) % sizeof(double) == 0, "PcgSeg is strided in doubles by the fused dot products");
 #define SEG_STRIDE ((int)(sizeof(PcgSeg) / sizeof(double)))
 
-__global__ void k_x_init(int M, const double* __restrict__ x0, const unsigned char* __restrict__ fixed, double* __restrict__ x, double* __restrict__ y, int* __restrict__ misc)
+__global__ void k_x_init(int M, const double* __restrict__ x0, const unsigned char* __restrict__ fixed, double* __restrict__ x, double* __restrict__ y)
 {
 	size_t i = (size_t)blockIdx.x * blockDim.x + threadIdx.x;
-	if (i < 4) misc[i] = 0;
 	if (i >= (size_t)M * 6) return;
 	y[i] = 0.0;
 	double v = x0 ? x0[i] : 0.0;
@@ -51,6 +50,31 @@
 	}
 	if (!with_ee) a[1] = 0.0;
 	wave_scatter_add<2>(&seg[sg].rr, a, v);
+}
+
+__global__ void k_pcg_resid_perm(int M, const double* __restrict__ E, const double* __restrict__ y, const int* __restrict__ pose_seg,
+                                 const unsigned char* __restrict__ fixed, const int* __restrict__ perm, const double* __restrict__ dscale,
+                                 double* __restrict__ r, double* __restrict__ v, PcgSeg* seg)
+{
+	int row = blockIdx.x * blockDim.x + threadIdx.x;
+	const bool ok = row < M;
+	double a[2] = { 0, 0 };
+	int sg = 0;
+	if (ok)
+	{
+		sg = pose_seg[row];
+		const size_t src = (size_t)perm[row] * 6;
+		for (int i = 0; i < 6; i++)
+		{
+			const size_t o = (size_t)row * 6 + i, q = src + i;
+			double e = E[o], d = e - y[o];
+			if (fixed && fixed[o]) { e = 0; d = 0; }
+			r[o] = d;
+			a[0] += d * d; a[1] += e * e;
+			v[o] = (fixed && fixed[q]) ? 0.0 : (E[q] - y[q]) * dscale[o];
+		}
+	}
+	wave_scatter_add<2>(&seg[sg].rr, a, ok);
 }
 
 __global__ void k_pcg_start(int nseg, PcgSeg* seg, const unsigned char* __restrict__ active, double rel_tol, int* ndone, const int* __restrict__ err, RunStatsDev* run)
@@ -102,12 +126,18 @@
 		for (int i = 0; i < 6; i++) { const size_t o = (size_t)row * 6 + i; p[o] = z[o] + beta * p[o]; }
 	}
 }
-__global__ void k_pcg_check(int nseg, PcgSeg* seg, int* ndone)
-{
-	int s = blockIdx.x * blockDim.x + threadIdx.x;
-	if (s >= nseg) return;
+__device__ __forceinline__ void pcg_outcome_to_run(int g, int nseg, const PcgSeg* seg, RunStatsDev* run)
+{
+	if (!seg[g].active) return;
+	const PcgSeg& fin = seg[nseg + g];
+	const double rel = fin.ee > 0 ? sqrt(fin.rr / fin.ee) : 0.0;
+	if (!(rel < 1e-8) || (seg[g].done != 1 && !(rel < 1e-9))) atomicAdd(&run->not_converged, 1);
+	if (seg[g].done == 0 && !(rel < 1e-10)) atomicAdd(&run->undone, 1);
+	atomicMax(reinterpret_cast<unsigned long long*>(&run->max_rel_residual), (unsigned long long)__double_as_longlong(rel == rel ? rel : 1e300));
+}
+__device__ __forceinline__ void pcg_check_system(int s, int nseg, PcgSeg* seg, int* ndone)
+{
 	PcgSeg& g = seg[s];
-	if (g.done) return;
 	const double rr = g.rr;
 	g.its++;
 	seg[nseg + s].rr = rr;
@@ -116,6 +146,13 @@
 	if (!(rr > g.thresh) || !(rr == rr) || (slow && (!(rr > 1e-16 * g.ee) || g.slow >= 10))) { g.done = (rr == rr) ? 1 : 2; atomicAdd(ndone, 1); }
 	g.rr_prev = rr;
 }
+__global__ void k_pcg_check(int nseg, PcgSeg* seg, int* ndone, RunStatsDev* run)
+{
+	int s = blockIdx.x * blockDim.x + threadIdx.x;
+	if (s >= nseg) return;
+	if (!seg[s].done) pcg_check_system(s, nseg, seg, ndone);
+	if (run) pcg_outcome_to_run(s, nseg, seg, run);
+}
 __global__ void k_pcg_reset(int nseg, int cur, PcgSeg* seg)
 {
 	int s = blockIdx.x * blockDim.x + threadIdx.x;
@@ -133,12 +170,7 @@
 __global__ void k_pcg_run_stats(int nseg, const PcgSeg* __restrict__ seg, RunStatsDev* run)
 {
 	int g = blockIdx.x * blockDim.x + threadIdx.x;
-	if (g >= nseg || !seg[g].active) return;
-	const PcgSeg& fin = seg[nseg + g];
-	const double rel = fin.ee > 0 ? sqrt(fin.rr / fin.ee) : 0.0;
-	if (!(rel < 1e-8) || (seg[g].done != 1 && !(rel < 1e-9))) atomicAdd(&run->not_converged, 1);
-	if (seg[g].done == 0 && !(rel < 1e-10)) atomicAdd(&run->undone, 1);
-	atomicMax(reinterpret_cast<unsigned long long*>(&run->max_rel_residual), (unsigned long long)__double_as_longlong(rel == rel ? rel : 1e300));
+	if (g < nseg) pcg_outcome_to_run(g, nseg, seg, run);
 }
 __global__ void k_pcg_debug(int nseg, int M, const PcgSeg* __restrict__ seg)
 {
@@ -151,28 +183,51 @@
 		       seg[g].done, seg[g].slow, seg[g].rr_prev / fin.ee, seg[g].thresh / fin.ee, fin.ee, seg[g].pAp, seg[g].rz[0], seg[g].rz[1]);
 }
 
-PcgWork pcg_begin(lsfm_context* ctx, const SolveIO& io, const SchurSystem& sy, const CholDev& ch)
-{
-	hipStream_t s = ctx->stream;
+static void pcg_alloc_vectors(lsfm_context* ctx, const SolveIO& io, PcgWork& w)
+{
 	Arena& sc = ctx->scratch;
-	const int M = io.M, nseg = io.nseg;
-	PcgWork w;
-	w.d_misc = sc.alloc<int>(4);
-	std::vector<PcgSeg> hseg(2 * (size_t)nseg);
-	memset(hseg.data(), 0, sizeof(PcgSeg) * hseg.size());
-	for (int g = 0, row = 0; g < nseg; g++) { hseg[g].row0 = hseg[nseg + g].row0 = row; row += io.seg_rows[g]; }
-	w.seg = sc.alloc<PcgSeg>(hseg.size());
-	h2d(ctx, w.seg, hseg.data(), sizeof(PcgSeg) * hseg.size());
-	const size_t nscal = (size_t)M * 6;
+	const size_t nscal = (size_t)io.M * 6;
 	w.r = sc.alloc<double>(nscal); w.z = ctx->comm ? ctx->comm->alloc<double>(nscal) : sc.alloc<double>(nscal); w.p = sc.alloc<double>(nscal);
 	w.Ap = sc.alloc<double>(nscal); w.v = sc.alloc<double>(nscal);
-	const unsigned nbe = (unsigned)((nscal + 255) / 256);
-	hipLaunchKernelGGL(k_x_init, dim3(std::max(1u, nbe)), dim3(256), 0, s, M, io.x0, io.d_fixed, io.x_pose, w.Ap, w.d_misc);
+}
+static void pcg_alloc_records(lsfm_context* ctx, const SolveIO& io, PcgWork& w)
+{
+	w.seg = ctx->scratch.alloc<PcgSeg>(2 * (size_t)io.nseg);
+	w.d_misc = ctx->scratch.alloc<int>(4);
+}
+void pcg_start_with_assembly(lsfm_context* ctx, const SolveIO& io, PcgWork& w, SolveStart& start)
+{
+	pcg_alloc_vectors(ctx, io, w);
+	start.x0 = io.x0; start.x = io.x_pose; start.y = w.Ap;
+	const std::function<void()> before = start.zeroed;
+	start.zeroed = [ctx, &io, &w, before]() { pcg_alloc_records(ctx, io, w); if (before) before(); };
+	w.started = true;
+}
+
+PcgWork pcg_begin(lsfm_context* ctx, const SolveIO& io, const SchurSystem& sy, const CholDev& ch, PcgWork w)
+{
+	hipStream_t s = ctx->stream;
+	const int M = io.M;
+	if (!w.started)
+	{
+		ZeroSpan zs(ctx->scratch);
+		pcg_alloc_records(ctx, io, w);
+		zs.zero(s);
+		pcg_alloc_vectors(ctx, io, w);
+		const unsigned nbe = (unsigned)(((size_t)M * 6 + 255) / 256);
+		hipLaunchKernelGGL(k_x_init, dim3(std::max(1u, nbe)), dim3(256), 0, s, M, io.x0, io.d_fixed, io.x_pose, w.Ap);
+	}
 	launch_spmv(ctx, sy, io.x_pose, w.Ap, io.d_fixed, nullptr, nullptr, nullptr, 1);
-	hipLaunchKernelGGL(k_pcg_resid, dim3((M + 127) / 128), dim3(128), 0, s, M, sy.E, w.Ap, io.d_pose_seg, io.d_fixed, w.r, w.seg, 1);
 	static const bool no_fused_fwd = getenv("LSFM_NO_FUSED_FWD") != nullptr;
 	w.fused_fwd = !ctx->pcg.mixed && !no_fused_fwd && ch.M > 0;
+	w.pairs = (level_overlap(ctx) & 4) != 0 && w.fused_fwd && ch.M == M;
+	if (!w.pairs) hipLaunchKernelGGL(k_pcg_resid, dim3((M + 127) / 128), dim3(128), 0, s, M, sy.E, w.Ap, io.d_pose_seg, io.d_fixed, w.r, w.seg, 1);
 	return w;
+}
+void pcg_resid_perm_in(lsfm_context* ctx, const SolveIO& io, const SchurSystem& sy, const CholDev& ch, PcgWork& w)
+{
+	const int M = io.M;
+	if (M) hipLaunchKernelGGL(k_pcg_resid_perm, dim3((M + 127) / 128), dim3(128), 0, ctx->stream, M, sy.E, w.Ap, io.d_pose_seg, io.d_fixed, ch.perm, ch.dscale, w.r, w.v, w.seg);
 }
 
 PcgResult pcg_run(lsfm_context* ctx, const SolveIO& io, const SchurSystem& sy, const CholDev& ch, PcgWork& w, const PcgSteps& steps)
@@ -186,8 +241,12 @@
 	PcgSeg* seg = w.seg;
 	int* d_misc = w.d_misc;
 	const bool mixed = ctx->pcg.mixed;
-	chol_apply(ctx, ch, r, v, z, io.d_fixed, io.d_pose_seg, &seg[0].rz[0], SEG_STRIDE, w.fused_fwd);
-	hipLaunchKernelGGL(k_copy, dim3(nbe), dim3(256), 0, s, nscal, z, p);
+	if (w.pairs) chol_apply(ctx, ch, r, v, z, io.d_fixed, io.d_pose_seg, &seg[0].rz[0], SEG_STRIDE, w.fused_fwd, p, Ap);
+	else
+	{
+		chol_apply(ctx, ch, r, v, z, io.d_fixed, io.d_pose_seg, &seg[0].rz[0], SEG_STRIDE, w.fused_fwd);
+		hipLaunchKernelGGL(k_copy, dim3(nbe), dim3(256), 0, s, nscal, z, p);
+	}
 	const bool err_to_run = steps.deferred || (ctx->comm && ctx->d_run);
 	hipLaunchKernelGGL(k_pcg_start, dim3(nbs), dim3(128), 0, s, nseg, seg, io.d_seg_active, ctx->pcg.rel_tol, d_misc + 1, ch.d_err, err_to_run ? ctx->d_run : (RunStatsDev*)nullptr);
 
@@ -200,6 +259,9 @@
 	const int base_steps = hinted ? io.step_hint : (planned_run ? steps.its : maxit);
 	const int planned = (planned_run && !ask_after && base_steps >= (mixed ? 3 : 2)) ? std::min(base_steps + 1, maxit) : base_steps;
 	bool counting = planned_run;
+	static const bool dbg_conv = getenv("LSFM_DEBUG_CONV") != nullptr;
+	const bool stats_with_last = w.pairs && steps.deferred && planned_run && !ask_after && !ctx->comm && ctx->d_run && !dbg_conv;
+	bool stats_left = false;
 	int cap = maxit;
 	while ((counting ? its < planned : (ndone < nseg && its < cap)))
 	{
@@ -210,7 +272,9 @@
 		launch_spmv(ctx, sy, x, Ap, io.d_fixed, nullptr, nullptr, nullptr, 1);
 		if (!w.es_done) { LSFM_REC_T(w.es1, s); w.es_done = true; }
 		hipLaunchKernelGGL(k_pcg_resid, dim3(nbr), dim3(128), 0, s, M, sy.E, Ap, io.d_pose_seg, io.d_fixed, r, seg, 0);
-		hipLaunchKernelGGL(k_pcg_check, dim3(nbs), dim3(128), 0, s, nseg, seg, d_misc + 1);
+		const bool last = stats_with_last && its + 1 >= planned;
+		hipLaunchKernelGGL(k_pcg_check, dim3(nbs), dim3(128), 0, s, nseg, seg, d_misc + 1, last ? ctx->d_run : (RunStatsDev*)nullptr);
+		stats_left = stats_left || last;
 		its++;
 		if (counting)
 		{
@@ -243,7 +307,7 @@
 		hipLaunchKernelGGL(k_pcg_update2, dim3(nbr), dim3(128), 0, s, M, cur, z, io.d_pose_seg, p, Ap, seg, d_misc + 1);
 		hipLaunchKernelGGL(k_pcg_reset, dim3(nbs), dim3(128), 0, s, nseg, cur, seg);
 	}
-	return PcgResult{ its, planned_run };
+	return PcgResult{ its, planned_run, stats_left };
 }
 
 void pcg_final_residual(lsfm_context* ctx, const SolveIO& io, const SchurSystem& sy, PcgWork& w)
diff --git a/linearsfm_amd/csrc/lsfm_pcg.hpp b/linearsfm_amd/csrc/lsfm_pcg.hpp
--- a/linearsfm_amd/csrc/lsfm_pcg.hpp
+++ b/linearsfm_amd/csrc/lsfm_pcg.hpp
@@ -12,11 +12,15 @@
 	bool fused_fwd = false;
 	hipEvent_t es0 = nullptr, es1 = nullptr;
 	bool es_done = false;
+	bool started = false;
+	bool pairs = false;
 };
 struct PcgSteps { bool warm, deferred; int its; bool mixed; double rel_tol; };
-struct PcgResult { int its; bool planned; };
+struct PcgResult { int its; bool planned; bool stats_left; };
 
-PcgWork pcg_begin(lsfm_context* ctx, const SolveIO& io, const SchurSystem& sy, const CholDev& ch);
+void pcg_start_with_assembly(lsfm_context* ctx, const SolveIO& io, PcgWork& w, SolveStart& start);
+PcgWork pcg_begin(lsfm_context* ctx, const SolveIO& io, const SchurSystem& sy, const CholDev& ch, PcgWork w = PcgWork());
+void pcg_resid_perm_in(lsfm_context* ctx, const SolveIO& io, const SchurSystem& sy, const CholDev& ch, PcgWork& w);
 PcgResult pcg_run(lsfm_context* ctx, const SolveIO& io, const SchurSystem& sy, const CholDev& ch, PcgWork& w, const PcgSteps& steps);
 void pcg_final_residual(lsfm_context* ctx, const SolveIO& io, const SchurSystem& sy, PcgWork& w);
 __global__ void k_pcg_run_stats(int nseg, const PcgSeg* __restrict__ seg, RunStatsDev* run);
diff --git a/linearsfm_amd/csrc/lsfm_solve.hip b/linearsfm_amd/csrc/lsfm_solve.hip
--- a/linearsfm_amd/csrc/lsfm_solve.hip
+++ b/linearsfm_amd/csrc/lsfm_solve.hip
@@ -1,5 +1,6 @@
 #include <algorithm>
 #include <cmath>
+#include <cstdlib>
 
 #include "lsfm_device.hpp"
 #include "lsfm_internal.hpp"
@@ -73,12 +74,18 @@
 }
 __global__ void __launch_bounds__(256) k_schur_scale(int M, const int* __restrict__ rowptr, const double* __restrict__ S, int NF, int nymax,
                                                       const double* __restrict__ ymax, const unsigned char* __restrict__ fixed, int* __restrict__ sexp,
-                                                      const double* __restrict__ ea, double* __restrict__ E)
+                                                      const double* __restrict__ ea, double* __restrict__ E, const double* __restrict__ x0,
+                                                      double* __restrict__ x, double* __restrict__ y)
 {
 	const int i = blockIdx.x * blockDim.x + threadIdx.x;
 	if (i < 6 * M)
 	{
 		E[i] = ea[i];
+		if (x)
+		{
+			y[i] = 0.0;
+			x[i] = (x0 && !(fixed && fixed[i])) ? x0[i] : 0.0;
+		}
 		const int p = i / 6, r = i - 6 * p;
 		sexp[i] = (fixed && fixed[i]) ? 400 : half_exponent(S[(size_t)rowptr[p] * 36 + 7 * r]);
 	}
@@ -606,17 +613,36 @@
 	}
 }
 
-void schur_vinv(lsfm_context* ctx, const SolveIO& io, SchurSystem& sy)
+static void vinv_alloc(lsfm_context* ctx, const SolveIO& io, SchurSystem& sy)
 {
 	sy.IV = ctx->scratch.alloc<double>((size_t)io.NF * 9);
 	sy.LY = ctx->scratch.alloc<double>((size_t)io.NF * 9);
 	sy.ymax = ctx->scratch.alloc<double>((size_t)(io.NF + 255) / 256 + 1);
 	sy.uu = nullptr;
 	if (io.rhs) sy.uu = ctx->scratch.alloc<double>((size_t)io.NF * 6);
-	if (io.NF) hipLaunchKernelGGL(k_vinv, dim3((io.NF + 255) / 256), dim3(256), 0, ctx->stream, io.NF, io.V, io.eb, sy.IV, sy.LY, sy.ymax, io.rhs ? *io.rhs : RhsFused(), sy.uu);
-}
-
-void build_schur_values(lsfm_context* ctx, const SolveIO& io, SchurSystem& sy)
+}
+static void vinv_launch(hipStream_t s, const SolveIO& io, const SchurSystem& sy)
+{
+	if (io.NF) hipLaunchKernelGGL(k_vinv, dim3((io.NF + 255) / 256), dim3(256), 0, s, io.NF, io.V, io.eb, sy.IV, sy.LY, sy.ymax, io.rhs ? *io.rhs : RhsFused(), sy.uu);
+}
+void schur_vinv(lsfm_context* ctx, const SolveIO& io, SchurSystem& sy)
+{
+	vinv_alloc(ctx, io, sy);
+	vinv_launch(ctx->stream, io, sy);
+}
+
+int level_overlap(const lsfm_context* ctx)
+{
+	static const int bits = []() {
+		const char* e = getenv("LSFM_LEVEL_OVERLAP");
+		int b = e ? atoi(e) & 7 : 7;
+		if (getenv("LSFM_NO_SIDE_STREAM")) b &= ~1;
+		return b;
+	}();
+	return ctx->comm ? 0 : bits;
+}
+
+void build_schur_values(lsfm_context* ctx, const SolveIO& io, SchurSystem& sy, const SolveStart* start)
 {
 	hipStream_t s = ctx->stream;
 	Arena& sc = ctx->scratch;
@@ -626,30 +652,60 @@
 	const unsigned long long mask = sy.mask;
 	const int ntiles = (NF + SCHUR_TILE - 1) / SCHUR_TILE;
 	unsigned char* fb;
+	const bool vinv_here = start && start->vinv;
+	if (vinv_here) vinv_alloc(ctx, io, sy);
 	const size_t nacc = 1 + (size_t)cnt * 36 + (size_t)M * 12;
+	sy.sexp = sc.alloc<int>((size_t)M * 6 + 1);
+	if (!ctx->comm) sy.E = sc.alloc<double>((size_t)M * 6);
+	static_assert(LSFM_PM_TILE % SCHUR_TILE == 0, "a tile of the panel kernel must be whole tiles of the fallback kernel");
+	const bool fresh_lists = NF && !sy.k9.ns;
+	if (fresh_lists)
+	{
+		sy.k9.ns = sc.alloc<int>(ntiles + 1);
+		sy.k9.pose = sc.alloc<int>((size_t)ntiles * 64 + 1);
+		sy.k9.eslot = sc.alloc<unsigned char>((size_t)io.NW + 1);
+		sy.k9.wlist = sc.alloc<int>((size_t)3 * ntiles + 1);
+		sy.k9.wcnt = sc.alloc<int>(8);
+		sy.k9_tiles = ntiles; sy.k9_NW = io.NW;
+	}
+	ZeroSpan zs(sc);
 	if (ctx->comm)
 	{
 		ctx->comm->restart();
 		sy.acc = ctx->comm->alloc<long long>(nacc);
 		sy.E = ctx->comm->alloc<double>((size_t)M * 6);
 		fill_async(s, sy.acc, 0, nacc * sizeof(long long));
-		ZeroSpan zs(sc);
 		sy.S = sc.alloc<double>((size_t)cnt * 36);
 		fb = sc.alloc<unsigned char>(ntiles + 1);
-		zs.zero(s);
 	}
 	else
 	{
-		ZeroSpan zs(sc);
 		sy.S = sc.alloc<double>((size_t)cnt * 36);
 		fb = sc.alloc<unsigned char>(ntiles + 1);
 		sy.acc = sc.alloc<long long>(nacc);
-		zs.zero(s);
-		sy.E = sc.alloc<double>((size_t)M * 6);
-	}
-	sy.sexp = sc.alloc<int>((size_t)M * 6 + 1);
-	if (io.NU) hipLaunchKernelGGL(k_schur_u, dim3((io.NU + 255) / 256), dim3(256), 0, s, io.NU, io.U, io.Ui, io.Uj, tab, hval, mask, sy.S);
-	hipLaunchKernelGGL(k_schur_scale, dim3((6 * M + 255) / 256 + 1), dim3(256), 0, s, M, sy.rowptr, sy.S, NF, NF ? (NF + 255) / 256 : 0, sy.ymax, io.d_fixed, sy.sexp, io.ea, sy.E);
+	}
+	if (start && start->zeroed) start->zeroed();
+	zs.zero(s);
+	auto scatter_u = [&](hipStream_t su) {
+		if (io.NU) hipLaunchKernelGGL(k_schur_u, dim3((io.NU + 255) / 256), dim3(256), 0, su, io.NU, io.U, io.Ui, io.Uj, tab, hval, mask, sy.S);
+	};
+	if (vinv_here && (level_overlap(ctx) & 1))
+	{
+		Fork side(ctx, ctx->stream2, evS_fork);
+		if (fresh_lists) launch_schur_slots(ctx, NF, io.fptr, io.photo, fb, sy.k9);
+		else vinv_launch(ctx->stream, io, sy);
+		scatter_u(side.main);
+		if (fresh_lists) vinv_launch(side.main, io, sy);
+		side.join(evS_done);
+	}
+	else
+	{
+		if (vinv_here) vinv_launch(s, io, sy);
+		scatter_u(s);
+		if (fresh_lists) launch_schur_slots(ctx, NF, io.fptr, io.photo, fb, sy.k9);
+	}
+	hipLaunchKernelGGL(k_schur_scale, dim3((6 * M + 255) / 256 + 1), dim3(256), 0, s, M, sy.rowptr, sy.S, NF, NF ? (NF + 255) / 256 : 0, sy.ymax, io.d_fixed, sy.sexp, io.ea, sy.E,
+	                   start ? start->x0 : (const double*)nullptr, start ? start->x : (double*)nullptr, start ? start->y : (double*)nullptr);
 	K9Out ko;
 	ko.poison = sy.acc; ko.S = sy.acc + 1; ko.Ehi = ko.S + (size_t)cnt * 36; ko.Elo = ko.Ehi + (size_t)M * 6;
 	ko.sexp = sy.sexp; ko.ey = sy.sexp + (size_t)M * 6;
@@ -658,19 +714,6 @@
 	{
 		hipEvent_t e2 = nullptr, e3 = nullptr;
 		if (ctx->stats) { e2 = ctx->pool_event(); e3 = ctx->pool_event(); LSFM_REC_T(e2, s); }
-		static_assert(LSFM_PM_TILE % SCHUR_TILE == 0, "a tile of the panel kernel must be whole tiles of the fallback kernel");
-		bool fresh_lists = false;
-		if (!sy.k9.ns)
-		{
-			fresh_lists = true;
-			sy.k9.ns = sc.alloc<int>(ntiles + 1);
-			sy.k9.pose = sc.alloc<int>((size_t)ntiles * 64 + 1);
-			sy.k9.eslot = sc.alloc<unsigned char>((size_t)io.NW + 1);
-			sy.k9.wlist = sc.alloc<int>((size_t)3 * ntiles + 1);
-			sy.k9.wcnt = sc.alloc<int>(8);
-			sy.k9_tiles = ntiles; sy.k9_NW = io.NW;
-			launch_schur_slots(ctx, NF, io.fptr, io.photo, fb, sy.k9);
-		}
 		launch_schur_panel(ctx, NF, io.fptr, io.photo, io.W, sy.LY, tab, hval, mask, ko, fb, most_rows(io.seg_rows), sy.k9, fresh_lists);
 		hipLaunchKernelGGL(k_schur_w, dim3(ntiles), dim3(SCHUR_TILE), 0, s, NF, io.fptr, io.photo, io.W, sy.IV, io.eb, tab, hval, mask, ko, fb, sy.LY);
 		if (ctx->stats)
diff --git a/linearsfm_amd/csrc/lsfm_solve.hpp b/linearsfm_amd/csrc/lsfm_solve.hpp
--- a/linearsfm_amd/csrc/lsfm_solve.hpp
+++ b/linearsfm_amd/csrc/lsfm_solve.hpp
@@ -65,8 +65,15 @@
 void schur_pattern_check(lsfm_context* ctx, const SolveIO& io, const SchurSystem& sy, const char* what);
 void rowptr_from_keys(lsfm_context* ctx, int M, int cnt, const unsigned long long* sorted_upper, int* rowptr);
 
-void build_schur_values(lsfm_context* ctx, const SolveIO& io, SchurSystem& sy);
+struct SolveStart {
+	bool vinv = false;
+	const double* x0 = nullptr;
+	double *x = nullptr, *y = nullptr;
+	std::function<void()> zeroed;
+};
+void build_schur_values(lsfm_context* ctx, const SolveIO& io, SchurSystem& sy, const SolveStart* start = nullptr);
 void schur_vinv(lsfm_context* ctx, const SolveIO& io, SchurSystem& sy);
+int level_overlap(const lsfm_context* ctx);
 void build_spmv_index(lsfm_context* ctx, SchurSystem& sy, const unsigned long long* sorted_upper);
 void launch_spmv(lsfm_context* ctx, const SchurSystem& sy, const double* x, double* y, const unsigned char* fixed, const double* dotw,
                  const int* pose_seg, double* dot, int dot_stride);
```
